# facebookresearch/D3GA

Measured on AMD Instinct MI355X. Metric: fwd+bwd frames/sec @500k Gaussians 1920x1080, higher is better.
Workload: dtype f32

## Files before the change

### d3ga_amd/_lib.py

```python
import ctypes
import os

_HERE = os.path.dirname(os.path.abspath(__file__))
_PATH = os.environ.get("D3GA_LIB_PATH") or os.path.join(_HERE, "libd3ga_hip.so")
_lib = None
ACC_STRIDE = 16
replay_epoch = [0]
ABI_VERSION = 112
KNOBS = ("composite_variant", "merge_slots", "tile_assign", "bwd_split", "sort_merge", "ssim_impl", "wgrad_ws", "chain_abl", "chain_grid")
CAMERA_SLOT_WINDOWED = -1.0
LOSS_PARTIALS = 2048
BLUR_PARTIALS = 6144
CALIB_PARTIALS = 12288
FRAME_GAMMA, FRAME_BG_WHITE, FRAME_ERODE_MASK, FRAME_CLOSE_HOLES, FRAME_IMAGE_U8, FRAME_SEG_F32 = 1, 2, 4, 8, 16, 32
EVAL_BG_WHITE, EVAL_COMPOSED, EVAL_ALPHA3, EVAL_BOUNDARY_F32 = 1, 2, 4, 8
EVAL_MAX_PARTIALS = 2048
MESH_MAX_SIDE = 16384
MESH_CAM_FLOATS = 16
INTERP_MAX_D = 64
KNN_MAX_K = 16
POINTS_MAX_K = 8
LPIPS_PARTIALS = 1024
OPTIM_CHUNK = 8192
OPTIM_ALIGNED16 = 1


class D3GAError(RuntimeError):
    pass


def library_path():
    return _PATH


class RasterParams(ctypes.Structure):
    _fields_ = [("P", ctypes.c_int32), ("M", ctypes.c_int32), ("sh_degree", ctypes.c_int32),
                ("W", ctypes.c_int32), ("H", ctypes.c_int32),
                ("tanfovx", ctypes.c_float), ("tanfovy", ctypes.c_float), ("scale_modifier", ctypes.c_float),
                ("antialiasing", ctypes.c_int32), ("prefiltered", ctypes.c_int32), ("debug", ctypes.c_int32),
                ("opacity_activation", ctypes.c_int32), ("forward_only", ctypes.c_int32),
                ("acc_self_clearing", ctypes.c_int32), ("n_views", ctypes.c_int32), ("per_view_geometry", ctypes.c_int32),
                ("tile_cull", ctypes.c_int32),
                ("factor_rows", ctypes.c_int32), ("per_view_appearance", ctypes.c_int32), ("per_view_background", ctypes.c_int32)]


BODY_MAX_JOINTS = 64
BODY_MAX_SHAPE = 32
BODY_LD_ALIGN = 2048


def body_saved_floats(J):
    return 27 * J + 16


class BodyModel(ctypes.Structure):
    _fields_ = [("V", ctypes.c_int32), ("J", ctypes.c_int32), ("n_shape", ctypes.c_int32), ("n_expr", ctypes.c_int32),
                ("n_hand_pca", ctypes.c_int32), ("ld", ctypes.c_int32), ("n_levels", ctypes.c_int32), ("reserved", ctypes.c_int32)] + \
               [(n, ctypes.c_void_p) for n in ("v_template", "dirs", "w_ptr", "w_joint", "w_val", "wt_ptr", "wt_vert", "wt_val",
                                               "J0", "Jdirs", "parents", "level_ptr", "level_joint", "child_ptr", "child_joint",
                                               "hand_comps", "hand_mean")]


class LbsPoseGrad(ctypes.Structure):
    _fields_ = [("J", ctypes.c_int32), ("n_chunks", ctypes.c_int32), ("n_entries", ctypes.c_int64)] + \
               [(n, ctypes.c_void_p) for n in ("tmpl", "delta", "chunk_ptr", "chunk_range", "entries", "counter", "scratch", "g_joint_mats",
                                               "g_Rh", "g_Th")]


DEFORM_ROUTE_CORNERS, DEFORM_ROUTE_MERGE = 1, 2


class CageDeformIn(ctypes.Structure):
    _fields_ = [(n, ctypes.c_int32) for n in ("P", "V", "flags", "reserved")] + \
               [(n, ctypes.c_void_p) for n in ("tetpoints", "tetras", "tetra_id", "barys", "canon_grad", "scales", "rots", "delta_barys")]


class CageDeformGrads(ctypes.Structure):
    _fields_ = [(n, ctypes.c_void_p) for n in ("g_means", "g_cov6", "g_tetpoints", "g_barys", "g_scales", "g_rots")]


class CageDeformRoute(ctypes.Structure):
    _fields_ = [(n, ctypes.c_int32) for n in ("kind", "n_segments")] + \
               [(n, ctypes.c_void_p) for n in ("item_pos", "seg_begin", "seg_ptr", "vert_start", "vert_items", "records")]


class CageDeformSkin(ctypes.Structure):
    _fields_ = [(n, ctypes.c_int32) for n in ("K", "reserved")] + \
               [(n, ctypes.c_void_p) for n in ("joint_mats", "skin_idx", "skin_w", "Rh", "g_tetpoints_extra", "g_delta")]


SKEL_MAX_JOINTS = 512
SKEL_SAVED_FLOATS = 12


class Skeleton(ctypes.Structure):
    _fields_ = [("J", ctypes.c_int32), ("n_params", ctypes.c_int32), ("n_levels", ctypes.c_int32), ("n_children", ctypes.c_int32)] + \
               [(n, ctypes.c_void_p) for n in ("parents", "level_ptr", "level_joint", "child_ptr", "child_joint", "joint_offset",
                                               "joint_rotation", "transform_offsets", "csr_ptr", "csr_col", "csr_val", "csc_ptr",
                                               "csc_row", "csc_val")]


CODE_MAX_B, CODE_MAX_D = 16, 4096
ROW_CACHE_MAX_PAIRS = 16


class RowPair(ctypes.Structure):
    _fields_ = [("table", ctypes.c_void_p), ("stage", ctypes.c_void_p), ("width", ctypes.c_int32), ("n_rows", ctypes.c_int32)]


SCALE_ACT_NONE, SCALE_ACT_EXP = 0, 1
SCALE_ENERGY_GRID = 1536
OBJ_MAX_FRAMES, OBJ_SLOTS, OBJ_MAX_LEN, OBJ_TERMS = 16, 9, 4096, 9
OBJ_STATUS_NAN_SEEN, OBJ_STATUS_FIRST_BAD, OBJ_STATUS_STEPS, OBJ_STATUS_TERMS, OBJ_STATUS_WORDS = 0, 1, 2, 4, 16


POSE_MAX_D, POSE_FIT_CHUNK = 256, 256
POSE_STAGE_PROJECT, POSE_STAGE_CLIP, POSE_STAGE_RECONSTRUCT = 1, 2, 4


class ObjectiveEntry(ctypes.Structure):
    _fields_ = [("ptr", ctypes.c_void_p), ("len", ctypes.c_int32), ("goff", ctypes.c_int32)]


class ObjectiveDesc(ctypes.Structure):
    _fields_ = [("n_frames", ctypes.c_int32), ("reserved", ctypes.c_int32)] + \
               [(n, ctypes.c_float) for n in ("lambda_dssim", "rgb_weight", "sil_weight", "fme_weight", "blur_weight", "vgg_weight")] + \
               [("entry", ObjectiveEntry * (OBJ_MAX_FRAMES * OBJ_SLOTS))]


_vp, _i, _i64, _f = ctypes.c_void_p, ctypes.c_int, ctypes.c_int64, ctypes.c_float
_prm = ctypes.POINTER(RasterParams)
_bm = ctypes.POINTER(BodyModel)
_lpg = ctypes.POINTER(LbsPoseGrad)
_sk = ctypes.POINTER(Skeleton)

_deform_tail = [ctypes.POINTER(c) for c in (CageDeformIn, CageDeformGrads, CageDeformRoute)]

_SIGNATURES = {
    "d3ga_version": ([], _i),
    "d3ga_status_string": ([_i], ctypes.c_char_p),
    "d3ga_debug_set": ([ctypes.c_int32, ctypes.c_int32], _i),
    "d3ga_debug_defaults": ([ctypes.POINTER(ctypes.c_int32), ctypes.c_int32], _i),
    "d3ga_lbs_cage_fwd": ([_i, _i] + [_vp] * 8 + [_vp], _i),
    "d3ga_lbs_cage_bwd": ([_i, _i] + [_vp] * 6 + [_lpg, _vp], _i),
    "d3ga_lbs_pose_scratch_bytes": ([_i, ctypes.c_int32, ctypes.c_int32, ctypes.POINTER(_i64)], _i),
    "d3ga_cage_deform_fwd": ([ctypes.POINTER(CageDeformIn), _vp, _vp, _vp], _i),
    "d3ga_cage_deform_bwd": ([ctypes.POINTER(c) for c in (CageDeformIn, CageDeformGrads, CageDeformRoute, CageDeformSkin)] + [_lpg, _vp], _i),
    "d3ga_cage_deform_bwd_tail": ([ctypes.POINTER(c) for c in (CageDeformIn, CageDeformGrads, CageDeformRoute, CageDeformSkin)] + [_lpg, _vp], _i),
    "d3ga_fem_energy_fwd": ([_i] + [_vp] * 4 + [_vp], _i),
    "d3ga_fem_energy_bwd": ([_i, _i] + [_vp] * 5 + [_vp], _i),
    "d3ga_bary_interp_fwd": ([ctypes.c_int32] * 3 + [_vp] * 5 + [_vp], _i),
    "d3ga_bary_interp_bwd": ([ctypes.c_int32] * 4 + [_vp] * 9 + [_vp], _i),
    "d3ga_raster_scratch_bytes": ([ctypes.c_int32, ctypes.c_int32, ctypes.c_int32, _i64, ctypes.POINTER(_i64)], _i),
    "d3ga_raster_scratch_bytes_views": ([ctypes.c_int32] * 4 + [_i64, ctypes.c_int32, ctypes.POINTER(_i64)], _i),
    "d3ga_raster_scratch_bytes_window": ([ctypes.c_int32] * 4 + [_i64, ctypes.c_int32, ctypes.POINTER(_i64)], _i),
    "d3ga_raster_binning_layout_window": ([ctypes.c_int32] * 3 + [_i64, ctypes.POINTER(_i64)], _i),
    "d3ga_raster_binning_layout": ([ctypes.c_int32, ctypes.c_int32, _i64, ctypes.POINTER(_i64)], _i),
    "d3ga_raster_img_layout": ([ctypes.c_int32, ctypes.c_int32, ctypes.POINTER(_i64)], _i),
    "d3ga_raster_img_layout_blocks": ([ctypes.c_int32, ctypes.c_int32, ctypes.POINTER(_i64)], _i),
    "d3ga_raster_img_bytes": ([ctypes.c_int32, ctypes.c_int32, _i64, ctypes.c_int32], _i64),
    "d3ga_raster_preprocess": ([_prm] + [_vp] * 12 + [_i64, _vp, _vp], _i),
    "d3ga_raster_bin_sort": ([_prm, _vp, _vp, _i64, _vp], _i),
    "d3ga_raster_composite_fwd": ([_prm, _vp, _vp, _vp, _i64, _vp, _vp, _vp, _vp], _i),
    "d3ga_raster_composite_bwd": ([_prm, _vp, _vp, _vp, _i64, _vp, _vp, _vp, _vp], _i),
    "d3ga_raster_composite_bwd_depth": ([_prm, _vp, _vp, _vp, _i64, _vp, _vp, _vp, _vp, _vp], _i),
    "d3ga_raster_composite_fwd2": ([_prm, _vp, _vp, _vp, _vp, _vp, _i64, _vp, _vp, _vp, _vp, _vp], _i),
    "d3ga_raster_composite_bwd2": ([_prm, _vp, _vp, _vp, _vp, _vp, _i64, _vp, _vp, _vp, _vp, _vp], _i),
    "d3ga_raster_preprocess_bwd": ([_prm] + [_vp] * 18 + [_vp], _i),
    "d3ga_raster_preprocess_bwd_deform": ([_prm] + [_vp] * 18 + _deform_tail + [_vp], _i),
    "d3ga_raster_forward": ([_prm] + [_vp] * 14 + [_i64, _vp, _vp, _vp, _vp], _i),
    "d3ga_raster_backward": ([_prm] + [_vp] * 11 + [_i64] + [_vp] * 11 + [_vp], _i),
    "d3ga_raster_backward_deform": ([_prm] + [_vp] * 11 + [_i64] + [_vp] * 11 + _deform_tail + [_vp], _i),
    "d3ga_raster_composite_fwd_l1": ([_prm, _vp, _vp, _vp, _i64] + [_vp] * 7 + [_vp], _i),
    "d3ga_raster_composite_bwd_l1": ([_prm, _vp, _vp, _vp, _i64] + [_vp] * 7 + [_vp], _i),
    "d3ga_raster_backward_l1": ([_prm] + [_vp] * 11 + [_i64] + [_vp] * 15 + [_vp], _i),
    "d3ga_raster_backward_l1_deform": ([_prm] + [_vp] * 11 + [_i64] + [_vp] * 15 + _deform_tail + [_vp], _i),
    "d3ga_raster_recolor": ([_prm] + [_vp] * 6 + [_vp], _i),
    "d3ga_raster_mark_visible": ([ctypes.c_int32, _vp, _vp, _vp, _vp], _i),
    "d3ga_sh_grad_from_views": ([ctypes.c_int32] * 4 + [_vp, _vp, _i64, _vp, _i64, ctypes.c_float, _vp, _vp], _i),
    "d3ga_compute_bary": ([_i, _i] + [_vp] * 5 + [_vp], _i),
    "d3ga_selftest_row_scan": ([_i, _vp, _vp, _vp], _i),
    "d3ga_selftest_alpha": ([ctypes.c_int32, _vp, _i, _vp, _vp, _vp, _vp, _vp, _vp], _i),
    "d3ga_knn3_mean_dist2": ([_i, _vp, _vp, _vp], _i),
    "d3ga_compute_bary_grid": ([_i] + [_vp] * 9 + [_vp], _i),
    "d3ga_knn3_mean_dist2_grid": ([_i] + [_vp] * 6 + [_vp], _i),
    "d3ga_knn_points": ([_i] * 4 + [_vp] * 4 + [_vp], _i),
    "d3ga_knn_points_grid": ([_i] * 3 + [_vp] * 8 + [_vp], _i),
    "d3ga_interp_face_attrs": ([_i64, _i64, _i] + [_vp] * 4 + [_vp], _i),
    "d3ga_l1_mean_fwd": ([_i64, _vp, _vp, _vp, _vp], _i),
    "d3ga_l1_mean_fwd_ws": ([_i64, _vp, _vp, _vp, _vp, _vp], _i),
    "d3ga_l1_mean_bwd": ([_i64, _vp, _vp, _vp, _vp, _vp], _i),
    "d3ga_l1_mean_fwd_ws_cell": ([_i64, _vp, _vp, _vp, _vp, _vp], _i),
    "d3ga_l1_mean_bwd_cell": ([_i64, _vp, _vp, _vp, _vp, _vp], _i),
    "d3ga_mlp_panel_bytes": ([ctypes.c_int32, ctypes.c_int32], _i64),
    "d3ga_mlp_pack_weights": ([ctypes.c_int32, ctypes.c_int32, _vp, _i64, _i64, _vp, _vp], _i),
# ... 167 lines not shown
```

### d3ga_amd/csrc/build.py

```python
import os
import subprocess
import sys

HERE = os.path.dirname(os.path.abspath(__file__))
SOURCES = ["deform.hip", "raster_pre.hip", "raster_bin.hip", "raster_composite.hip", "raster_composite_scan.hip", "raster_api.hip", "bary.hip", "loss.hip", "image_tail.hip", "calib.hip", "frame_prep.hip", "eval.hip", "mesh_raster.hip", "point_raster.hip", "optim.hip", "mlp.hip", "encoding.hip", "body_model.hip", "skeleton.hip", "perceptual.hip", "lpips.hip", "knn.hip", "bary_interp.hip", "frame_state.hip", "objective.hip", "pose_prior.hip"]
LINK_MAP = os.path.join(HERE, "d3ga.map")
HEADERS = ["d3ga_math.h", "d3ga_internal.h", "raster_pre_body.h", "deform_tail.h", "composite_common.h", "body_model_math.h", "skeleton_math.h", "frame_prep_math.h", "eval_math.h", "mesh_raster_math.h", "point_raster_math.h", "perceptual_math.h", "lpips_math.h", "knn_math.h", "objective_math.h", "pose_prior_math.h", os.path.join("..", "..", "include", "d3ga.h")]
ABL = os.environ.get("D3GA_SCAN_ABL")
VARIANT = os.environ.get("D3GA_VARIANT")
DIAG = os.environ.get("D3GA_DIAG") or (("abl" + ABL) if ABL else None) or (("var" + VARIANT.split(":")[0]) if VARIANT else None)
DIAG_DIR = os.path.abspath(os.path.join(HERE, "..", "..", "tools", "_build"))
_DIAG_TAG = (VARIANT.split(":")[0] if (VARIANT and not os.environ.get("D3GA_DIAG") and not ABL) else
             "diag" if os.environ.get("D3GA_DIAG") in (None, "counters") else os.environ["D3GA_DIAG"])
if VARIANT:
    FLAGS_VARIANT = [f for f in VARIANT.split(":", 1)[1].split(",") if f]
else:
    FLAGS_VARIANT = []
OUT = (os.path.join(DIAG_DIR, f"libd3ga_hip_abl{ABL}.so" if ABL else f"libd3ga_hip_{_DIAG_TAG}.so") if DIAG
       else os.path.join(HERE, "..", "libd3ga_hip.so"))
FLAGS = ["--offload-arch=gfx950", "-O3", "-std=c++17", "-fPIC", "-fvisibility=hidden", "-munsafe-fp-atomics", "-fno-gpu-rdc",
         "-Wall", "-Wno-unused-function"] + FLAGS_VARIANT
EXTRA = {"raster_composite_scan.hip": ["-fno-slp-vectorize"],
         "raster_composite.hip": ["-fno-slp-vectorize"],
         "frame_prep.hip": ["-fhip-fp32-correctly-rounded-divide-sqrt"],
         "eval.hip": ["-fhip-fp32-correctly-rounded-divide-sqrt"]}
EXTRA["mesh_raster.hip"] = ["-fhip-fp32-correctly-rounded-divide-sqrt", "-ffp-contract=off"]
EXTRA["lpips.hip"] = ["-fhip-fp32-correctly-rounded-divide-sqrt"]
EXTRA["point_raster.hip"] = EXTRA["mesh_raster.hip"]
EXTRA["knn.hip"] = ["-ffp-contract=off"]
EXTRA["frame_state.hip"] = ["-fhip-fp32-correctly-rounded-divide-sqrt"]
EXTRA["objective.hip"] = ["-fhip-fp32-correctly-rounded-divide-sqrt", "-ffp-contract=off"]
EXTRA["pose_prior.hip"] = ["-ffp-contract=off"]
if os.environ.get("D3GA_CHAIN_WAVES"):
    FLAGS.append("-DD3GA_CHAIN_WAVES=" + os.environ["D3GA_CHAIN_WAVES"])
if os.environ.get("D3GA_CHAIN_CS"):
    FLAGS.append("-DD3GA_CHAIN_CS=" + os.environ["D3GA_CHAIN_CS"])
if os.environ.get("D3GA_ALL_NOSLP"):
    FLAGS.append("-fno-slp-vectorize")
if ABL:
    FLAGS.append("-DD3GA_SCAN_ABL=" + ABL.split("w")[0].split("p")[0].split("f")[0])
    if "w" in ABL:
        FLAGS.append("-DD3GA_TILE_WAVES=" + ABL.split("w")[1])
    if "f" in ABL:
        FLAGS.append("-DD3GA_FWD_WAVES=" + ABL.split("f")[1])
    if "p" in ABL:
        FLAGS.append("-DD3GA_TILE_PRIO=1")
if os.environ.get("D3GA_DIAG"):
    FLAGS += ["-DD3GA_DIAG", "-DD3GA_DIAG_TIMELINE"]
    if os.environ.get("D3GA_DIAG") == "counters":
        FLAGS.append("-DD3GA_DIAG_COUNTERS")


def _newer(target, deps):
    if not os.path.exists(target):
        return True
    t = os.path.getmtime(target)
    return any(os.path.getmtime(d) > t for d in deps)


def build(force=False, verbose=False):
    hipcc = os.environ.get("HIPCC", "/opt/rocm/bin/hipcc")
    objdir = os.path.join(DIAG_DIR, f"obj_abl{ABL}" if ABL else f"obj_{_DIAG_TAG}") if DIAG else os.path.join(HERE, "build")
    os.makedirs(objdir, exist_ok=True)
    hdrs = [os.path.join(HERE, h) for h in HEADERS]
    objs = []
    for src in SOURCES:
        s = os.path.join(HERE, src)
        o = os.path.join(objdir, src.replace(".hip", ".o"))
        if force or _newer(o, [s] + hdrs):
            cmd = [hipcc] + FLAGS + EXTRA.get(src, []) + ["-c", s, "-o", o]
            if verbose:
                print(" ".join(cmd))
            subprocess.check_call(cmd)
        objs.append(o)
    if force or _newer(OUT, objs + [LINK_MAP]):
        import torch
        tlib = os.path.join(os.path.dirname(torch.__file__), "lib")
        cmd = ["g++", "-shared", "-fPIC"] + objs + ["-L" + tlib, "-lamdhip64", "-Wl,-rpath," + tlib,
                                                    "-Wl,-rpath,/opt/rocm/lib", "-Wl,--version-script=" + LINK_MAP, "-o", OUT]
        if verbose:
            print(" ".join(cmd))
        subprocess.check_call(cmd)
    return os.path.abspath(OUT)


if __name__ == "__main__":
    print(build(force="--force" in sys.argv, verbose=True))
```

### d3ga_amd/csrc/d3ga_internal.h

```cpp
#pragma once
#include <hip/hip_runtime.h>
#include <stdint.h>

#include "../../include/d3ga.h"
#include "d3ga_math.h"

namespace d3ga {

constexpr int kBlock = 256;

int debug_knob(int key);

int deform_tail_check(const d3ga_cage_deform_in *in, const d3ga_cage_deform_grads *gr, const d3ga_cage_deform_route *route);

static inline int64_t align256(int64_t x) { return (x + 255) & ~int64_t(255); }

struct GeomBuf {
    float *depth;
    float4 *conic_o;
    float4 *rgb_invd;
    uint2 *rect;
    uint8_t *clamped;
    float *cov3D;
    float4 *xyh;
    float *dcol;
    int64_t dcol_stride;
};
static inline int64_t geom_bytes(int64_t P) {
    return align256(4 * P) + align256(16 * P) + align256(16 * P) + align256(8 * P) + align256(P) +
           align256(24 * P) + align256(16 * P) + align256(36 * P);
}
static inline GeomBuf carve_geom(void *base, int64_t P) {
    char *p = (char *)base;
    GeomBuf g;
    g.depth = (float *)p;     p += align256(4 * P);
    g.conic_o = (float4 *)p;  p += align256(16 * P);
    g.rgb_invd = (float4 *)p; p += align256(16 * P);
    g.rect = (uint2 *)p;      p += align256(8 * P);
    g.clamped = (uint8_t *)p; p += align256(P);
    g.cov3D = (float *)p;     p += align256(24 * P);
    g.xyh = (float4 *)p;      p += align256(16 * P);
    g.dcol = (float *)p;
    g.dcol_stride = P;
    return g;
}
__host__ __device__ static inline GeomBuf geom_view(const GeomBuf &g, int64_t P, int64_t v) {
    GeomBuf o = g;
    const int64_t d = v * P;
    o.depth += d; o.conic_o += d; o.rgb_invd += d; o.rect += d; o.clamped += d; o.cov3D += 6 * d; o.xyh += d; o.dcol += d;
    return o;
}

struct BinBuf {
    uint32_t *counters;
    uint32_t *tile_count;
    uint32_t *tile_count2;
    uint32_t *vis_part;
    uint32_t *tile_start;
    uint32_t *tile_cursor;
    uint64_t *keys;
    uint32_t *point_list;
    uint32_t *big_tiles;
    uint32_t *huge_tiles;
    uint32_t *mid_tiles;
    uint32_t *tile_order;
};
constexpr int kVisParts = 32, kVisStride = 32;
constexpr int kUnresvWord = 1;
static inline int64_t bin_bytes(int64_t tiles, int64_t dcap) {
    return 256 + 2 * align256(4 * tiles) + 4 * kVisParts * kVisStride + align256(4 * (tiles + 1)) + align256(4 * tiles) + align256(8 * dcap) +
           align256(4 * dcap) + 4 * align256(4 * tiles);
}
static inline BinBuf carve_bin(void *base, int64_t tiles, int64_t dcap) {
    char *p = (char *)base;
    BinBuf b;
    b.counters = (uint32_t *)p;    p += 256;
    b.tile_count = (uint32_t *)p;  p += align256(4 * tiles);
    b.tile_count2 = (uint32_t *)p; p += align256(4 * tiles);
    b.vis_part = (uint32_t *)p;    p += 4 * kVisParts * kVisStride;
    b.tile_start = (uint32_t *)p;  p += align256(4 * (tiles + 1));
    b.tile_cursor = (uint32_t *)p; p += align256(4 * tiles);
    b.keys = (uint64_t *)p;        p += align256(8 * dcap);
    b.point_list = (uint32_t *)p;  p += align256(4 * dcap);
    b.big_tiles = (uint32_t *)p;   p += align256(4 * tiles);
    b.huge_tiles = (uint32_t *)p;  p += align256(4 * tiles);
    b.mid_tiles = (uint32_t *)p;   p += align256(4 * tiles);
    b.tile_order = (uint32_t *)p;
    return b;
}

struct ImgBuf {
    float *final_T;
    uint32_t *n_contrib;
    uint32_t *blk_count;
    uint2 *blk_list;
};
static inline int64_t img_bytes(int64_t W, int64_t H, int64_t tiles, int64_t dcap, int64_t views = 1) {
    return 2 * align256(4 * W * H * views) + align256(64 * tiles) + align256(128 * dcap);
}
static inline ImgBuf carve_img(void *base, int64_t W, int64_t H, int64_t tiles, int64_t views = 1) {
    ImgBuf i;
    char *p = (char *)base;
    i.final_T = (float *)p;        p += align256(4 * W * H * views);
    i.n_contrib = (uint32_t *)p;   p += align256(4 * W * H * views);
    i.blk_count = (uint32_t *)p;   p += align256(64 * tiles);
    i.blk_list = (uint2 *)p;
    return i;
}

constexpr int kResvStride = 512;
constexpr int kResvHdr = 4;
constexpr int kResvTiles = kResvStride - kResvHdr;
constexpr int kResvSlots = (kResvTiles + 63) / 64;
static inline int64_t resv_waves(int64_t P) { return (kBlock / 64) * ((P + kBlock - 1) / kBlock); }
static inline int64_t resv_bytes(int64_t P, int64_t views) { return align256(4 * kResvStride * resv_waves(P) * views); }

struct TileWindow {
    int x0, y0, w, h;
    __device__ __forceinline__ bool empty() const { return w <= 0 || h <= 0; }
    __device__ __forceinline__ bool fits() const { return w <= kResvTiles && h <= kResvTiles && w * h <= kResvTiles; }
    __device__ __forceinline__ int area() const { return w * h; }
    __device__ __forceinline__ int tile_of(int k, int gx, float inv_w) const {
        const int r = (int)(((float)k + 0.5f) * inv_w);
        return (y0 + r) * gx + x0 + (k - r * w);
    }
};

#ifdef __HIPCC__
__device__ __forceinline__ TileWindow wave_tile_window(bool visible, int rx0, int ry0, int rx1, int ry1) {
    int bx0 = visible ? rx0 : 0x7fffffff, by0 = visible ? ry0 : 0x7fffffff, bx1 = visible ? rx1 : 0, by1 = visible ? ry1 : 0;
#pragma unroll
    for (int off = 1; off < 64; off <<= 1) {
        bx0 = min(bx0, __shfl_xor(bx0, off)); by0 = min(by0, __shfl_xor(by0, off));
        bx1 = max(bx1, __shfl_xor(bx1, off)); by1 = max(by1, __shfl_xor(by1, off));
    }
    TileWindow win;
    win.x0 = bx0; win.y0 = by0;
    win.w = bx1 > bx0 ? bx1 - bx0 : 0;
    win.h = by1 > by0 ? by1 - by0 : 0;
    if (win.w == 0 || win.h == 0) { win.x0 = 0; win.y0 = 0; win.w = 0; win.h = 0; }
    return win;
}
#endif

static inline int tiles_x(int W) { return (W + kTile - 1) / kTile; }
static inline int tiles_y(int H) { return (H + kTile - 1) / kTile; }
static inline int n_views_of(const d3ga_raster_params *prm) { return prm->n_views > 1 ? prm->n_views : 1; }
static inline bool is_windowed(const d3ga_raster_params *prm) { return prm->tanfovx == D3GA_CAMERA_SLOT_WINDOWED; }
static inline int grid_x(const d3ga_raster_params *prm) { return tiles_x(prm->W) + (is_windowed(prm) ? 1 : 0); }
static inline int grid_y(const d3ga_raster_params *prm) { return tiles_y(prm->H) + (is_windowed(prm) ? 1 : 0); }
static inline int4 *win_table(void *binning, int64_t tiles, int64_t dcap) { return (int4 *)((char *)binning + bin_bytes(tiles, dcap)); }
static inline int64_t win_table_bytes(int64_t views) { return align256(16 * views); }
static inline uint32_t *resv_records(void *binning, int64_t tiles, int64_t dcap, int64_t views, bool windowed) {
    return (uint32_t *)((char *)binning + bin_bytes(tiles, dcap) + (windowed ? win_table_bytes(views) : 0));
}

static inline int check_launch(hipStream_t s, int debug) {
    hipError_t e = hipGetLastError();
    if (e != hipSuccess) return (int)e;
    if (debug) {
        e = hipStreamSynchronize(s);
        if (e != hipSuccess) return (int)e;
    }
    return 0;
}

#define D3GA_TRY(expr)            \
    do {                          \
        int _st = (expr);         \
        if (_st != 0) return _st; \
    } while (0)
#define D3GA_HIP(expr)                          \
    do {                                        \
        hipError_t _e = (expr);                 \
        if (_e != hipSuccess) return (int)_e;   \
    } while (0)

#ifdef __HIPCC__
static __global__ void zero_words_kernel(uint32_t *__restrict__ p, size_t n) {
    for (size_t i = (size_t)blockIdx.x * blockDim.x + threadIdx.x; i < n; i += (size_t)gridDim.x * blockDim.x) p[i] = 0u;
}
static __global__ void zero_bytes_kernel(unsigned char *__restrict__ p, size_t n) {
    for (size_t i = (size_t)blockIdx.x * blockDim.x + threadIdx.x; i < n; i += (size_t)gridDim.x * blockDim.x) p[i] = 0;
}
static inline hipError_t zero_async(void *ptr, size_t bytes, hipStream_t s) {
    if (bytes == 0) return hipSuccess;
    if ((((uintptr_t)ptr | bytes) & 3) == 0) {
        const size_t n = bytes / 4;
        const size_t blocks = (n + 4 * kBlock - 1) / (4 * kBlock);
        hipLaunchKernelGGL(zero_words_kernel, dim3((unsigned)(blocks < 1 ? 1 : (blocks > 4096 ? 4096 : blocks))), dim3(kBlock), 0, s,
                           reinterpret_cast<uint32_t *>(ptr), n);
    } else {
        const size_t blocks = (bytes + kBlock - 1) / kBlock;
        hipLaunchKernelGGL(zero_bytes_kernel, dim3((unsigned)(blocks > 4096 ? 4096 : blocks)), dim3(kBlock), 0, s,
                           reinterpret_cast<unsigned char *>(ptr), bytes);
    }
    return hipGetLastError();
}
#endif

}
```

### d3ga_amd/csrc/raster_bin.hip

```cpp
#include <atomic>

#include "composite_common.h"

namespace d3ga {

constexpr int kScanBlock = 1024;

__device__ __forceinline__ void tile_scan_body(int tiles, const uint32_t *__restrict__ count, const uint32_t *__restrict__ count2,
                                               const uint32_t *__restrict__ vis_part, uint32_t *__restrict__ start, uint32_t *__restrict__ cursor,
                                               uint32_t *__restrict__ counters, uint64_t dcap,
                                               uint32_t *__restrict__ big_tiles, uint32_t *__restrict__ huge_tiles,
                                               uint32_t *__restrict__ mid_tiles, uint32_t n_small, uint32_t n_mid,
                                               uint32_t n_large) {
    constexpr int kPer = 8, kChunk = kPer * kScanBlock;
    __shared__ uint32_t s_wave[2][kScanBlock / 64];
    __shared__ uint32_t s_max;
    const int tid = threadIdx.x, lane = tid & 63, wave = tid >> 6;
    if (tid == 0) s_max = 0;
    const bool unresv = vis_part[kUnresvWord] != 0u;
    uint32_t visible = wave == 0 && lane < kVisParts ? vis_part[lane * kVisStride] : 0u;
    uint32_t carry = 0, mx = 0;
    int par = 0;
    for (int c0 = 0; c0 < tiles; c0 += kChunk, par ^= 1) {
        const int t0 = c0 + kPer * tid;
        uint32_t c[kPer], u[kPer];
        if (t0 + kPer <= tiles) {
            const uint4 lo = reinterpret_cast<const uint4 *>(count + t0)[0], hi = reinterpret_cast<const uint4 *>(count + t0)[1];
            uint4 lo2 = make_uint4(0u, 0u, 0u, 0u), hi2 = lo2;
            if (unresv) { lo2 = reinterpret_cast<const uint4 *>(count2 + t0)[0]; hi2 = reinterpret_cast<const uint4 *>(count2 + t0)[1]; }
            c[0] = lo.x; c[1] = lo.y; c[2] = lo.z; c[3] = lo.w; c[4] = hi.x; c[5] = hi.y; c[6] = hi.z; c[7] = hi.w;
            u[0] = lo2.x; u[1] = lo2.y; u[2] = lo2.z; u[3] = lo2.w; u[4] = hi2.x; u[5] = hi2.y; u[6] = hi2.z; u[7] = hi2.w;
        } else {
#pragma unroll
            for (int k = 0; k < kPer; ++k) { c[k] = t0 + k < tiles ? count[t0 + k] : 0u; u[k] = unresv && t0 + k < tiles ? count2[t0 + k] : 0u; }
        }
        uint32_t any2 = 0;
#pragma unroll
        for (int k = 0; k < kPer; ++k) { any2 |= u[k]; c[k] += u[k]; }
        uint32_t sum = 0;
#pragma unroll
        for (int k = 0; k < kPer; ++k) { sum += c[k]; mx = max(mx, c[k]); }
        uint32_t incl = sum;
#pragma unroll
        for (int off = 1; off < 64; off <<= 1) {
            const uint32_t v = __shfl_up(incl, off);
            if (lane >= off) incl += v;
        }
        if (lane == 63) s_wave[par][wave] = incl;
        __syncthreads();
        uint32_t wbase = 0, total = 0;
#pragma unroll
        for (int w = 0; w < kScanBlock / 64; ++w) {
            const uint32_t v = s_wave[par][w];
            wbase += w < wave ? v : 0u;
            total += v;
        }
        uint32_t run = carry + wbase + incl - sum;
        uint32_t e[kPer];
        int cls[kPer];
#pragma unroll
        for (int k = 0; k < kPer; ++k) {
            e[k] = run;
            run += c[k];
            cls[k] = c[k] > n_large ? 2 : (c[k] > n_mid ? 1 : (c[k] > n_small ? 0 : -1));
        }
#pragma unroll
        for (int q = 0; q < 3; ++q) {
            uint32_t nq = 0;
#pragma unroll
            for (int k = 0; k < kPer; ++k) nq += cls[k] == q ? 1u : 0u;
            if (__ballot(nq != 0u) == 0ull) continue;
            uint32_t inq = nq;
#pragma unroll
            for (int off = 1; off < 64; off <<= 1) {
                const uint32_t v = __shfl_up(inq, off);
                if (lane >= off) inq += v;
            }
            const uint32_t tot = (uint32_t)__shfl((int)inq, 63);
            uint32_t base = 0;
            if (lane == 0) base = atomicAdd(&counters[q == 0 ? D3GA_CNT_MID : (q == 1 ? D3GA_CNT_BIG : D3GA_CNT_HUGE)], tot);
            uint32_t pos = (uint32_t)__shfl((int)base, 0) + inq - nq;
            uint32_t *list = q == 0 ? mid_tiles : (q == 1 ? big_tiles : huge_tiles);
#pragma unroll
            for (int k = 0; k < kPer; ++k)
                if (cls[k] == q) list[pos++] = (uint32_t)(t0 + k);
        }
        if (t0 + kPer <= tiles) {
            const uint4 lo = make_uint4(e[0], e[1], e[2], e[3]), hi = make_uint4(e[4], e[5], e[6], e[7]);
            reinterpret_cast<uint4 *>(start + t0)[0] = lo; reinterpret_cast<uint4 *>(start + t0)[1] = hi;
        } else {
#pragma unroll
            for (int k = 0; k < kPer; ++k)
                if (t0 + k < tiles) start[t0 + k] = e[k];
        }
        if (any2) {
#pragma unroll
            for (int k = 0; k < kPer; ++k)
                if (t0 + k < tiles && u[k]) cursor[t0 + k] = e[k] + (c[k] - u[k]);
        }
        carry += total;
    }
#pragma unroll
    for (int off = 1; off < 64; off <<= 1) {
        mx = max(mx, (uint32_t)__shfl_xor((int)mx, off));
        visible += (uint32_t)__shfl_xor((int)visible, off);
    }
    if (lane == 0) atomicMax(&s_max, mx);
    __syncthreads();
    if (tid == 0) {
        start[tiles] = carry;
        counters[D3GA_CNT_D] = carry;
        counters[D3GA_CNT_OVERFLOW] = (uint64_t)carry > dcap ? 1u : 0u;
        counters[D3GA_CNT_MAXTILE] = s_max;
        counters[D3GA_CNT_VISIBLE] = visible;
    }
}

__device__ __forceinline__ void tile_order_body(int tiles, const uint32_t *__restrict__ count, const uint32_t *__restrict__ count2,
                                                const uint32_t *__restrict__ vis_part, uint32_t *__restrict__ order, uint32_t *__restrict__ counters) {
    __shared__ uint32_t s_hist[256];
    __shared__ uint32_t s_zero;
    const int tid = threadIdx.x, lane = tid & 63;
    constexpr int kPer = 8;
    const bool unresv = vis_part[kUnresvWord] != 0u;
    if (tid < 256) s_hist[tid] = 0;
    if (tid == 0) s_zero = 0;
    __syncthreads();
    auto bucket = [](uint32_t c) { return 254u - min(c >> 4, 254u); };
    for (int c0 = 0; c0 < tiles; c0 += kPer * kScanBlock) {
        uint32_t c[kPer];
#pragma unroll
        for (int k = 0; k < kPer; ++k) {
            const int t = c0 + k * kScanBlock + tid;
            c[k] = t < tiles ? count[t] + (unresv ? count2[t] : 0u) : 0xffffffffu;
        }
#pragma unroll
        for (int k = 0; k < kPer; ++k) {
            const bool zero = c[k] == 0u;
            const unsigned long long zm = __ballot(zero);
            if (lane == 0 && zm) atomicAdd(&s_zero, (uint32_t)__popcll(zm));
            if (c[k] != 0u && c[k] != 0xffffffffu) atomicAdd(&s_hist[bucket(c[k])], 1u);
        }
        if (c0 + kPer * kScanBlock < tiles) continue;
        __syncthreads();
        if (tid < 64) {
            uint32_t v[4], sum = 0;
#pragma unroll
            for (int k = 0; k < 4; ++k) { v[k] = (4 * tid + k < 255) ? s_hist[4 * tid + k] : 0u; sum += v[k]; }
            uint32_t incl = sum;
#pragma unroll
            for (int off = 1; off < 64; off <<= 1) {
                const uint32_t u = __shfl_up(incl, off);
                if (tid >= off) incl += u;
            }
            uint32_t run = incl - sum;
#pragma unroll
            for (int k = 0; k < 4; ++k) { s_hist[4 * tid + k] = run; run += v[k]; }
        }
        __syncthreads();
        if (tid == 0) {
            s_zero = s_hist[255];
            counters[D3GA_CNT_HEAVY] = s_hist[255] <= 4096u ? (s_hist[255] + 9u) / 10u : 0u;
        }
        __syncthreads();
        for (int c1 = 0; c1 < tiles; c1 += kPer * kScanBlock) {
            if (c0 != 0) {
#pragma unroll
                for (int k = 0; k < kPer; ++k) {
                    const int t = c1 + k * kScanBlock + tid;
                    c[k] = t < tiles ? count[t] + (unresv ? count2[t] : 0u) : 0xffffffffu;
                }
            }
#pragma unroll
            for (int k = 0; k < kPer; ++k) {
                const int t = c1 + k * kScanBlock + tid;
                const bool zero = c[k] == 0u;
                const unsigned long long zm = __ballot(zero);
                uint32_t zbase = 0;
                if (lane == 0 && zm) zbase = atomicAdd(&s_zero, (uint32_t)__popcll(zm));
                zbase = (uint32_t)__shfl((int)zbase, 0);
                if (zero) order[zbase + (uint32_t)__popcll(zm & ((1ull << lane) - 1ull))] = (uint32_t)t;
                if (c[k] != 0u && c[k] != 0xffffffffu) order[atomicAdd(&s_hist[bucket(c[k])], 1u)] = (uint32_t)t;
            }
        }
    }
}

__global__ __launch_bounds__(kScanBlock) void tile_scan_order_kernel(int tiles, const uint32_t *__restrict__ count,
                                                                     const uint32_t *__restrict__ count2,
                                                                     const uint32_t *__restrict__ vis_part,
                                                                     uint32_t *__restrict__ start,
                                                                     uint32_t *__restrict__ cursor,
                                                                     uint32_t *__restrict__ counters, uint64_t dcap,
                                                                     uint32_t *__restrict__ big_tiles,
                                                                     uint32_t *__restrict__ huge_tiles,
                                                                     uint32_t *__restrict__ mid_tiles, uint32_t n_small,
                                                                     uint32_t n_mid, uint32_t n_large,
                                                                     uint32_t *__restrict__ order) {
    if (blockIdx.x == 0) tile_scan_body(tiles, count, count2, vis_part, start, cursor, counters, dcap, big_tiles, huge_tiles, mid_tiles, n_small, n_mid, n_large);
    else tile_order_body(tiles, count, count2, vis_part, order, counters);
}

__global__ __launch_bounds__(kBlock) void tile_scatter_kernel(int P, int gx, const uint2 *__restrict__ rect,
                                                              const float *__restrict__ depth,
                                                              const uint32_t *__restrict__ start,
                                                              const uint32_t *__restrict__ resv,
                                                              uint32_t *__restrict__ cursor, uint64_t *__restrict__ keys,
                                                              uint64_t dcap) {
    __shared__ uint32_t s_cur[kBlock / 64][kResvTiles];
    const int tid = threadIdx.x, lane = tid & 63, wave = tid >> 6;
    const int i = blockIdx.x * kBlock + tid;
    if (i - lane >= P) return;
    const size_t j = (size_t)blockIdx.y * P + i;
    const uint32_t *rec = resv + ((size_t)blockIdx.y * gridDim.x * (kBlock / 64) + blockIdx.x * (kBlock / 64) + wave) * kResvStride;
    const uint2 box = *reinterpret_cast<const uint2 *>(rec);
    uint32_t base[kResvSlots];
    base[0] = rec[kResvHdr + lane];
    int x0 = 0, y0 = 0, x1 = 0, y1 = 0;
    uint64_t key = 0;
    if (i < P) {
        const uint2 rc = rect[j];
        x0 = rc.x & 0xffffu; y0 = rc.x >> 16; x1 = rc.y & 0xffffu; y1 = rc.y >> 16;
        key = ((uint64_t)__float_as_uint(depth[j]) << 32) | (uint32_t)j;
    }
    const bool visible = x1 > x0 && y1 > y0;
    TileWindow win;
    win.x0 = (int)(box.x & 0xffffu); win.y0 = (int)(box.x >> 16); win.w = (int)(box.y & 0xffffu); win.h = (int)(box.y >> 16);
    if (win.empty()) return;
    if (win.fits()) {
        const int area = win.area();
        uint32_t *cur = s_cur[wave];
        const float inv_w = 1.0f / (float)win.w;
#pragma unroll
        for (int q = 1; q < kResvSlots; ++q) base[q] = lane + 64 * q < area ? rec[kResvHdr + lane + 64 * q] : 0u;
#pragma unroll
        for (int q = 0; q < kResvSlots; ++q) {
            const int k = lane + 64 * q;
            if (k < area) cur[k] = start[win.tile_of(k, gx, inv_w)] + base[q];
        }
        __builtin_amdgcn_wave_barrier();
        if (visible)
            for (int ty = y0; ty < y1; ++ty)
                for (int tx = x0; tx < x1; ++tx) {
                    const int l = (ty - win.y0) * win.w + (tx - win.x0);
                    if ((unsigned)l >= (unsigned)area) continue;
                    const uint32_t pos = atomicAdd(&cur[l], 1u);
                    if (pos < dcap) keys[pos] = key;
                }
    } else if (visible) {
        for (int ty = y0; ty < y1; ++ty)
            for (int tx = x0; tx < x1; ++tx) {
                const uint32_t pos = atomicAdd(&cursor[ty * gx + tx], 1u);
                if (pos < dcap) keys[pos] = key;
            }
    }
}

template <typename KeyPtr>
__device__ __forceinline__ void bitonic_sort(KeyPtr k, int n, int tid, int nthreads) {
    int n2 = 1;
    while (n2 < n) n2 <<= 1;
    const int half = n2 >> 1;
    for (int size = 2, lsz = 1; size <= n2; size <<= 1, ++lsz) {
        const int hs = size >> 1;
        for (int i = tid; i < half; i += nthreads) {
            const int blk = i >> (lsz - 1), off = i & (hs - 1);
            const int lo = (blk << lsz) + off, hi = (blk << lsz) + size - 1 - off;
            if (hi < n) {
                const uint64_t a = k[lo], b = k[hi];
                if (b < a) { k[lo] = b; k[hi] = a; }
            }
        }
        __syncthreads();
        for (int j = hs >> 1, lj = lsz - 2; j >= 1; j >>= 1, --lj) {
            for (int i = tid; i < half; i += nthreads) {
                const int blk = i >> lj, off = i & (j - 1);
                const int lo = (blk << (lj + 1)) + off, hi = lo + j;
                if (hi < n) {
                    const uint64_t a = k[lo], b = k[hi];
                    if (b < a) { k[lo] = b; k[hi] = a; }
                }
            }
            __syncthreads();
        }
    }
}

template <int BLOCK, int CAP>
__device__ __forceinline__ void sort_one_tile_bucket(uint64_t *s_key, uint32_t *s_bin, uint32_t *s_red, int tile,
                                                     const uint32_t *__restrict__ start, const uint64_t *__restrict__ keys,
                                                     uint32_t *__restrict__ point_list, uint64_t dcap) {
    static_assert(CAP == 8 * BLOCK, "eight keys / eight counters per thread");
    constexpr int NW = BLOCK / 64;
    const uint64_t b64 = min((uint64_t)start[tile], dcap), e64 = min((uint64_t)start[tile + 1], dcap);
    const int n = min((int)(e64 - b64), CAP);
    const int tid = threadIdx.x, lane = tid & 63, wave = tid >> 6;
    uint64_t r[8];
    uint32_t lo = 0xffffffffu, hi = 0u;
#pragma unroll
    for (int k = 0; k < 8; ++k) {
        const int i = tid + k * BLOCK;
        r[k] = i < n ? keys[b64 + i] : ~0ull;
    }
#pragma unroll
    for (int k = 0; k < 8; ++k) {
        const int i = tid + k * BLOCK;
        if (i < n) { const uint32_t d = (uint32_t)(r[k] >> 32); lo = min(lo, d); hi = max(hi, d); }
    }
#pragma unroll
    for (int off = 1; off < 64; off <<= 1) {
        lo = min(lo, (uint32_t)__shfl_xor((int)lo, off));
        hi = max(hi, (uint32_t)__shfl_xor((int)hi, off));
    }
    if (lane == 0) { s_red[wave] = lo; s_red[NW + wave] = hi; }
#pragma unroll
    for (int k = 0; k < 8; ++k) s_bin[tid + k * BLOCK] = 0u;
    __syncthreads();
#pragma unroll
    for (int w = 0; w < NW; ++w) { lo = min(lo, s_red[w]); hi = max(hi, s_red[NW + w]); }
    const uint32_t range = hi - lo;
    int sh = 32 - __clz((int)(range | 1u)) - (31 - __clz(CAP));
    if (range & 0x80000000u) sh = 32 - (31 - __clz(CAP));
    sh = max(sh, 0);
    uint32_t bucket[8], slot[8];
#pragma unroll
    for (int k = 0; k < 8; ++k) {
        const int i = tid + k * BLOCK;
        bucket[k] = ((uint32_t)(r[k] >> 32) - lo) >> sh;
        slot[k] = 0u;
        if (i < n) slot[k] = atomicAdd(&s_bin[bucket[k]], 1u);
    }
    __syncthreads();
    {
        uint32_t c[8], sum = 0;
#pragma unroll
        for (int k = 0; k < 8; ++k) { c[k] = s_bin[8 * tid + k]; sum += c[k]; }
        uint32_t incl = sum;
#pragma unroll
        for (int off = 1; off < 64; off <<= 1) {
            const uint32_t u = (uint32_t)__shfl_up((int)incl, off);
            if (lane >= off) incl += u;
        }
        if (lane == 63) s_red[wave] = incl;
        __syncthreads();
        uint32_t run = incl - sum;
#pragma unroll
        for (int w = 0; w < NW; ++w) if (w < wave) run += s_red[w];
#pragma unroll
        for (int k = 0; k < 8; ++k) { s_bin[8 * tid + k] = run; run += c[k]; }
        if (tid == BLOCK - 1) s_bin[CAP] = run;
    }
    __syncthreads();
#pragma unroll
    for (int k = 0; k < 8; ++k) {
        const int i = tid + k * BLOCK;
        if (i < n) s_key[s_bin[bucket[k]] + slot[k]] = r[k];
    }
    __syncthreads();
#pragma unroll
    for (int k = 0; k < 8; ++k) {
        const int i = tid + k * BLOCK;
        if (i < n) {
            const uint32_t b0 = s_bin[bucket[k]], b1 = s_bin[bucket[k] + 1];
            uint32_t less = 0;
            for (uint32_t p = b0; p < b1; ++p) less += s_key[p] < r[k] ? 1u : 0u;
            point_list[b64 + b0 + less] = (uint32_t)r[k];
        }
    }
}

template <int BLOCK, int CAP>
__device__ __forceinline__ bool sort_huge_tile_bucket(uint64_t *s_key, uint32_t *s_bin, uint32_t *s_cur, uint32_t *s_red, int tile,
                                                      const uint32_t *__restrict__ start, const uint64_t *__restrict__ keys,
                                                      uint32_t *__restrict__ point_list, uint64_t dcap) {
    static_assert(CAP == 8 * BLOCK, "eight counters per thread");
    constexpr int NW = BLOCK / 64;
    const uint64_t b64 = min((uint64_t)start[tile], dcap), e64 = min((uint64_t)start[tile + 1], dcap);
    const int n = (int)(e64 - b64);
    const int tid = threadIdx.x, lane = tid & 63, wave = tid >> 6;
    uint32_t lo = 0xffffffffu, hi = 0u;
    for (int i = tid; i < n; i += BLOCK) { const uint32_t d = (uint32_t)(keys[b64 + i] >> 32); lo = min(lo, d); hi = max(hi, d); }
#pragma unroll
    for (int off = 1; off < 64; off <<= 1) {
        lo = min(lo, (uint32_t)__shfl_xor((int)lo, off));
        hi = max(hi, (uint32_t)__shfl_xor((int)hi, off));
    }
    __syncthreads();
    if (lane == 0) { s_red[wave] = lo; s_red[NW + wave] = hi; }
#pragma unroll
    for (int k = 0; k < 8; ++k) s_bin[tid + k * BLOCK] = 0u;
    __syncthreads();
#pragma unroll
    for (int w = 0; w < NW; ++w) { lo = min(lo, s_red[w]); hi = max(hi, s_red[NW + w]); }
    const uint32_t range = hi - lo;
    const int sh = max(32 - __clz((int)(range | 1u)) - (31 - __clz(CAP)), 0);
    for (int i = tid; i < n; i += BLOCK) atomicAdd(&s_bin[((uint32_t)(keys[b64 + i] >> 32) - lo) >> sh], 1u);
    __syncthreads();
    uint32_t cmax = 0;
    {
        uint32_t c[8], sum = 0;
#pragma unroll
        for (int k = 0; k < 8; ++k) { c[k] = s_bin[8 * tid + k]; sum += c[k]; cmax = max(cmax, c[k]); }
        uint32_t incl = sum;
#pragma unroll
        for (int off = 1; off < 64; off <<= 1) {
            const uint32_t u = (uint32_t)__shfl_up((int)incl, off);
            if (lane >= off) incl += u;
            cmax = max(cmax, (uint32_t)__shfl_xor((int)cmax, off));
        }
        __syncthreads();
        if (lane == 63) { s_red[wave] = incl; s_red[NW + wave] = cmax; }
        __syncthreads();
        uint32_t run = incl - sum;
#pragma unroll
        for (int w = 0; w < NW; ++w) { if (w < wave) run += s_red[w]; cmax = max(cmax, s_red[NW + w]); }
#pragma unroll
        for (int k = 0; k < 8; ++k) { s_bin[8 * tid + k] = run; run += c[k]; }
        if (tid == BLOCK - 1) s_bin[CAP] = run;
    }
    __syncthreads();
    if (cmax > (uint32_t)CAP) return false;
    for (int segA = 0; segA < CAP;) {
        if (tid == 0) {
            const uint32_t limit = s_bin[segA] + (uint32_t)CAP;
            int a = segA + 1, b = CAP;
            while (a < b) { const int m = (a + b + 1) >> 1; if (s_bin[m] <= limit) a = m; else b = m - 1; }
            s_red[0] = (uint32_t)a;
        }
#pragma unroll
        for (int k = 0; k < 8; ++k) s_cur[tid + k * BLOCK] = 0u;
        __syncthreads();
        const int segB = (int)s_red[0];
        const uint32_t baseA = s_bin[segA], m = s_bin[segB] - baseA;
        if (m) {
            for (int i = tid; i < n; i += BLOCK) {
                const uint64_t key = keys[b64 + i];
                const uint32_t b = ((uint32_t)(key >> 32) - lo) >> sh;
                if (b >= (uint32_t)segA && b < (uint32_t)segB) s_key[s_bin[b] - baseA + atomicAdd(&s_cur[b], 1u)] = key;
            }
            __syncthreads();
            for (uint32_t i = tid; i < m; i += BLOCK) {
                const uint64_t key = s_key[i];
                const uint32_t b = ((uint32_t)(key >> 32) - lo) >> sh;
                const uint32_t b0 = s_bin[b] - baseA, b1 = s_bin[b + 1] - baseA;
                uint32_t less = 0;
                for (uint32_t p = b0; p < b1; ++p) less += s_key[p] < key ? 1u : 0u;
                point_list[b64 + baseA + b0 + less] = (uint32_t)key;
            }
        }
        __syncthreads();
        segA = segB;
    }
    return true;
}

template <int BLOCK, int CAP>
__global__ __launch_bounds__(BLOCK) void tile_sort_lds_kernel(const uint32_t *__restrict__ start,
                                                              const uint64_t *__restrict__ keys,
                                                              uint32_t *__restrict__ point_list, uint64_t dcap,
                                                              const uint32_t *__restrict__ order, int tiles) {
    __shared__ uint64_t s_key[CAP];
    __shared__ __attribute__((aligned(8))) uint32_t s_bin[CAP + 1];
    __shared__ uint32_t s_red[2 * (BLOCK / 64)];
    for (int rank = blockIdx.x; rank < tiles; rank += gridDim.x) {
        const int tile = (int)order[rank];
        const uint32_t n = start[tile + 1] - start[tile];
        if (n == 0) return;
        if (n <= (uint32_t)CAP) sort_one_tile_bucket<BLOCK, CAP>(s_key, s_bin, s_red, tile, start, keys, point_list, dcap);
        __syncthreads();
    }
}

template <int BLOCK, int CAP>
__global__ __launch_bounds__(BLOCK) void tile_sort_lds_list_kernel(const uint32_t *__restrict__ start,
                                                                   const uint64_t *__restrict__ keys,
                                                                   uint32_t *__restrict__ point_list, uint64_t dcap,
                                                                   const uint32_t *__restrict__ list,
                                                                   const uint32_t *__restrict__ list_count,
                                                                   uint64_t *__restrict__ keys_rw,
                                                                   const uint32_t *__restrict__ huge_list,
                                                                   const uint32_t *__restrict__ huge_count,
                                                                   const uint32_t *__restrict__ list2,
                                                                   const uint32_t *__restrict__ list2_count) {
    extern __shared__ __attribute__((aligned(16))) uint64_t s_key_dyn[];
    uint32_t *s_bin = reinterpret_cast<uint32_t *>(s_key_dyn + CAP);
    uint32_t *s_red = s_bin + CAP + 1;
    uint32_t *s_cur = s_red + 2 * (BLOCK / 64) + 2;
    const uint32_t count = *list_count;
    for (uint32_t v = blockIdx.x; v < count; v += gridDim.x) {
        __syncthreads();
        sort_one_tile_bucket<BLOCK, CAP>(s_key_dyn, s_bin, s_red, (int)list[v], start, keys, point_list, dcap);
    }
    if (list2) {
        const uint32_t count2 = *list2_count;
        for (uint32_t v = gridDim.x - 1u - blockIdx.x; v < count2; v += gridDim.x) {
            __syncthreads();
            sort_one_tile_bucket<BLOCK, CAP>(s_key_dyn, s_bin, s_red, (int)list2[v], start, keys, point_list, dcap);
        }
    }
    if (huge_list) {
        const uint32_t hcount = *huge_count;
        const int tid = threadIdx.x;
        for (uint32_t k = blockIdx.x; k < hcount; k += gridDim.x) {
            const int tile = (int)huge_list[k];
            const uint64_t b64 = min((uint64_t)start[tile], dcap), e64 = min((uint64_t)start[tile + 1], dcap);
            const int n = (int)(e64 - b64);
            __syncthreads();
            if (!sort_huge_tile_bucket<BLOCK, CAP>(s_key_dyn, s_bin, s_cur, s_red, tile, start, keys, point_list, dcap)) {
                bitonic_sort(keys_rw + b64, n, tid, BLOCK);
                for (int i = tid; i < n; i += BLOCK) point_list[b64 + i] = (uint32_t)keys_rw[b64 + i];
            }
        }
    }
}

}

using namespace d3ga;

constexpr int kSortSmall = 2048;
constexpr int kSortMid = 4096;
constexpr int kSortLarge = 8192;
static inline size_t sort_lds_bytes(int cap, int block, bool huge = false) {
    return (size_t)cap * 8 + ((size_t)cap + 1 + 2 * (block / 64) + 2 + (huge ? cap : 0)) * 4 + 16;
}


extern "C" int d3ga_raster_bin_sort(const d3ga_raster_params *prm, void *geom, void *binning, int64_t d_capacity,
                                    d3ga_stream_t stream) {
    if (!prm || !geom || !binning) return D3GA_E_NULL;
    if (prm->P < 0 || prm->W <= 0 || prm->H <= 0 || d_capacity < 0) return D3GA_E_SIZE;
    hipStream_t s = (hipStream_t)stream;
    const int views = n_views_of(prm);
    const int gx = grid_x(prm);
    const int tiles = gx * grid_y(prm) * views;
    const int64_t P = (int64_t)prm->P * views;
    BinBuf bin = carve_bin(binning, tiles, d_capacity);
    GeomBuf g = carve_geom(geom, P);
    hipLaunchKernelGGL(tile_scan_order_kernel, dim3(2), dim3(kScanBlock), 0, s, tiles, bin.tile_count, bin.tile_count2, bin.vis_part, bin.tile_start,
                       bin.tile_cursor, bin.counters, (uint64_t)d_capacity, bin.big_tiles, bin.huge_tiles, bin.mid_tiles,
                       (uint32_t)kSortSmall, (uint32_t)kSortMid, (uint32_t)kSortLarge, bin.tile_order);
    D3GA_TRY(check_launch(s, prm->debug));
    if (P == 0 || d_capacity == 0) return D3GA_OK;
    hipLaunchKernelGGL(tile_scatter_kernel, dim3((unsigned)((prm->P + kBlock - 1) / kBlock), (unsigned)views), dim3(kBlock), 0, s, prm->P,
                       gx, g.rect, g.depth, bin.tile_start, resv_records(binning, tiles, d_capacity, views, is_windowed(prm)),
                       bin.tile_cursor, bin.keys, (uint64_t)d_capacity);
    D3GA_TRY(check_launch(s, prm->debug));
    {
        static std::atomic<int> resident[64] = {};
        int dev = 0;
        D3GA_HIP(hipGetDevice(&dev));
        int want = (dev >= 0 && dev < 64) ? resident[dev].load(std::memory_order_relaxed) : 0;
        if (want == 0) {
            int per_cu = 0, cus = 0;
            if (hipOccupancyMaxActiveBlocksPerMultiprocessor(&per_cu, (const void *)tile_sort_lds_kernel<256, kSortSmall>, 256, 0) != hipSuccess || per_cu < 1) per_cu = 4;
            if (hipDeviceGetAttribute(&cus, hipDeviceAttributeMultiprocessorCount, dev) != hipSuccess || cus < 1) cus = 256;
            want = per_cu * cus;
            if (dev >= 0 && dev < 64) resident[dev].store(want, std::memory_order_relaxed);
        }
        hipLaunchKernelGGL((tile_sort_lds_kernel<256, kSortSmall>), dim3(tiles < want ? tiles : want), dim3(256), 0, s, bin.tile_start,
                           bin.keys, bin.point_list, (uint64_t)d_capacity, (const uint32_t *)bin.tile_order, tiles);
    }
    D3GA_TRY(check_launch(s, prm->debug));
    {
        static std::atomic<bool> attr_set[64] = {};
        int dev = 0;
        D3GA_HIP(hipGetDevice(&dev));
        if (dev >= 0 && dev < 64 && !attr_set[dev].load(std::memory_order_relaxed)) {
            D3GA_HIP(hipFuncSetAttribute((const void *)tile_sort_lds_list_kernel<1024, kSortLarge>,
                                         hipFuncAttributeMaxDynamicSharedMemorySize, (int)sort_lds_bytes(kSortLarge, 1024, true)));
            attr_set[dev].store(true, std::memory_order_relaxed);
        }
    }
    const int lgrid = tiles < 256 ? tiles : 256, mgrid = tiles < 768 ? tiles : 768;
    const int merge_knob = debug_knob(D3GA_KNOB_SORT_MERGE);
    const bool merged = merge_knob >= 0 ? merge_knob != 0 : d_capacity / (tiles > 0 ? tiles : 1) < 320;
#define D3GA_LAUNCH_LIST_SORT(BLOCKV, CAPV, GRID, HUGE, LIST, CNT, KEYS_RW, HLIST, HCNT, LIST2, CNT2)                              \
    hipLaunchKernelGGL((tile_sort_lds_list_kernel<BLOCKV, CAPV>), dim3(GRID), dim3(BLOCKV), sort_lds_bytes(CAPV, BLOCKV, HUGE), s, \
                       bin.tile_start, bin.keys, bin.point_list, (uint64_t)d_capacity, LIST, CNT, KEYS_RW, HLIST, HCNT, LIST2, CNT2)
    const uint32_t *const nil = nullptr;
    if (!merged) {
        D3GA_LAUNCH_LIST_SORT(512, kSortMid, mgrid, false, bin.mid_tiles, bin.counters + D3GA_CNT_MID, (uint64_t *)nullptr, nil, nil, nil, nil);
        D3GA_TRY(check_launch(s, prm->debug));
    }
    const uint32_t *l2 = merged ? (const uint32_t *)bin.mid_tiles : nil, *c2 = merged ? (const uint32_t *)(bin.counters + D3GA_CNT_MID) : nil;
    D3GA_LAUNCH_LIST_SORT(1024, kSortLarge, lgrid, true, bin.big_tiles, bin.counters + D3GA_CNT_BIG, bin.keys,
                          (const uint32_t *)bin.huge_tiles, (const uint32_t *)(bin.counters + D3GA_CNT_HUGE), l2, c2);
#undef D3GA_LAUNCH_LIST_SORT
    return check_launch(s, prm->debug);
}
```

### d3ga_amd/csrc/raster_pre.hip

```cpp
#include <type_traits>

#include "composite_common.h"
#include "raster_pre_body.h"
#include "deform_tail.h"

namespace d3ga {

constexpr int kShRow = 52;
constexpr int kShSlab = 64 * kShRow;
constexpr size_t kShLdsBytes = (size_t)(kBlock / 64) * kShSlab * sizeof(float);

__host__ __device__ __forceinline__ bool sh_staged(int M) { return M > 0 && (3 * M) % 4 == 0 && 3 * M <= 48; }

__device__ __forceinline__ void sh_slab_load(float *slab, const float *__restrict__ src, int rows, int M3, int lane) {
    const int nvec = rows * M3 / 4;
    for (int v = lane; v < nvec; v += 64) {
        const float4 x = reinterpret_cast<const float4 *>(src)[v];
        const int e = 4 * v, r = e / M3, c = e - r * M3;
        *reinterpret_cast<float4 *>(slab + r * kShRow + c) = x;
    }
}
__device__ __forceinline__ void sh_slab_store(const float *slab, float *__restrict__ dst, int rows, int M3, int lane) {
    const int nvec = rows * M3 / 4;
    for (int v = lane; v < nvec; v += 64) {
// ... 69 lines not shown
    float *slab = s_sh + wave * kShHalfSlab;
    const int row0 = blockIdx.x * kBlock + wave * 64;
    const int rows = min(64, prm.P - row0);
    const int nb = (prm.sh_degree + 1) * (prm.sh_degree + 1);
    float B[16];
    float dx = 0.f, dy = 0.f, dz = 1.f;
    auto eval = [&](const float *row) __attribute__((always_inline)) {
        if (WANT_J) cj = sh_accumulate_jacobian(B, dx, dy, dz, row, nb, cj);
        else sh_accumulate(B, row, 0, 16, nb, acc);
    };
    if (M3 == 48 && rows == 64) {
        if (WANT_J) {
            sh_two_pass48(slab, shs + (size_t)48 * row0, lane, [&]() __attribute__((always_inline)) {
                sh_view_dir(mean, campos, dx, dy, dz);
                sh_basis(prm.sh_degree, dx, dy, dz, B);
            }, eval);
            return;
        }
        const float *src = shs + (size_t)48 * row0;
        const ShRegs<kShPassRows> h0 = sh_rows48_load<kShPassRows>(src, lane);
        const ShRegs<kShPassRows> h1 = sh_rows48_load<kShPassRows>(src + 48 * kShPassRows, lane);
        sh_view_basis(prm, mean, campos, B);
        __builtin_amdgcn_wave_barrier();
        sh_rows48_to_slab<kShPassRows>(slab, h0, lane);
        __builtin_amdgcn_wave_barrier();
        if (lane / kShPassRows == 0) eval(slab + (lane % kShPassRows) * kShRow);
        __builtin_amdgcn_wave_barrier();
        sh_rows48_to_slab<kShPassRows>(slab, h1, lane);
        __builtin_amdgcn_wave_barrier();
        if (lane / kShPassRows == 1) eval(slab + (lane % kShPassRows) * kShRow);
        return;
    }
    if (WANT_J && i < prm.P) sh_view_dir(mean, campos, dx, dy, dz);
    if (i < prm.P) sh_view_basis(prm, mean, campos, B);
    for (int h = 0; h < 2; ++h) {
        const int r = min(kShPassRows, rows - kShPassRows * h);
        __builtin_amdgcn_wave_barrier();
        if (r > 0) sh_slab_load(slab, shs + (size_t)M3 * (row0 + kShPassRows * h), r, M3, lane);
        __builtin_amdgcn_wave_barrier();
        if (i < prm.P && lane / kShPassRows == h) eval(slab + (lane % kShPassRows) * kShRow);
    }
}

struct TileRect { bool visible; int r0, r1, r2, r3; };
__device__ __forceinline__ TileRect view_tile_rect(const PreOut &o, int tile_row0) {
    const Splat &sp = o.sp;
    return TileRect{sp.visible, sp.rect[0], sp.rect[1] + tile_row0, sp.rect[2], sp.rect[3] + tile_row0};
}
__device__ __forceinline__ void tile_tighten(PreOut &o) {
    Splat &sp = o.sp;
    if (!sp.visible) return;
    const SplatCull sc = splat_cull(sp.conic[0], sp.conic[1], sp.conic[2], o.opacity);
    tile_rect_tight(sp.rect, sp.px, sp.py, sc.hx, sc.hy, sp.rect);
}
__device__ __forceinline__ float write_geom_records_splat(const GeomBuf &geom, int i, const PreOut &o, bool keep_cov, int tile_row0,
                                                          int32_t *__restrict__ radii) {
    const Splat &sp = o.sp;
    if (keep_cov) {
#pragma unroll
        for (int k = 0; k < 6; ++k) geom.cov3D[6 * (size_t)i + k] = o.c6[k];
    }
    radii[i] = sp.radius;
    geom.depth[i] = sp.depth;
    geom.rect[i] = sp.visible ? make_uint2((uint32_t)sp.rect[0] | ((uint32_t)(sp.rect[1] + tile_row0) << 16),
                                           (uint32_t)sp.rect[2] | ((uint32_t)(sp.rect[3] + tile_row0) << 16))
                              : make_uint2(0u, 0u);
    geom.conic_o[i] = make_float4(sp.conic[0], sp.conic[1], sp.conic[2], o.opacity);
    {
        const SplatCull sc = splat_cull(sp.conic[0], sp.conic[1], sp.conic[2], o.opacity);
        geom.xyh[i] = make_float4(sp.px, sp.py, sp.visible ? sc.hx : -1.0f, sc.hy);
    }
    return sp.visible ? 1.0f / sp.depth : 0.f;
}
__device__ __forceinline__ void write_geom_records_colour(const GeomBuf &geom, int i, float r, float g, float b, float invd,
                                                           uint8_t clampmask, bool want_j, const ShColJ &cj) {
    geom.rgb_invd[i] = make_float4(r, g, b, invd);
    geom.clamped[i] = clampmask;
    if (want_j) dcol_store(geom.dcol, geom.dcol_stride, i, cj);
}
__device__ __forceinline__ void write_geom_records(const GeomBuf &geom, int i, const PreOut &o, bool keep_cov, int tile_row0,
                                                   int32_t *__restrict__ radii, bool want_j, const ShColJ &cj) {
    const float invd = write_geom_records_splat(geom, i, o, keep_cov, tile_row0, radii);
    write_geom_records_colour(geom, i, o.rgb[0], o.rgb[1], o.rgb[2], invd, o.clampmask, want_j, cj);
}

__device__ __forceinline__ PreOut window_clip(PreOut o, int x0, int y0, int gx, int gy) {
    Splat &sp = o.sp;
    const int r0 = max(sp.rect[0], x0) - x0, r1 = max(sp.rect[1], y0) - y0;
    const int r2 = min(sp.rect[2], x0 + gx) - x0, r3 = min(sp.rect[3], y0 + gy) - y0;
    if (sp.visible && r2 > r0 && r3 > r1) { sp.rect[0] = r0; sp.rect[1] = r1; sp.rect[2] = r2; sp.rect[3] = r3; }
    else { sp.visible = false; sp.rect[0] = sp.rect[1] = sp.rect[2] = sp.rect[3] = 0; }
    return o;
}
__global__ void window_table_kernel(d3ga_raster_params prm, const float *__restrict__ campos, int views, int4 *__restrict__ table) {
    const int v = blockIdx.x * blockDim.x + threadIdx.x;
    if (v >= views) return;
    const ViewCam c = view_cam(prm, nullptr, nullptr, campos + (size_t)D3GA_CAMERA_SLOT_WINDOWED_FLOATS * v, true);
    table[v] = make_int4(c.ox, c.oy, c.W, c.H);
}

struct TileResv { TileWindow win; uint32_t base[kResvSlots]; };
template <bool SCALAR_WIN = false >
__device__ __forceinline__ TileResv tile_reserve_issue(uint32_t *s_win, const TileRect &t, int gx, uint32_t *__restrict__ tile_count,
                                                       uint32_t *__restrict__ tile_count2, uint32_t *__restrict__ vis_part) {
    const int lane = threadIdx.x & 63;
    TileResv r;
    r.win = wave_tile_window(t.visible, t.r0, t.r1, t.r2, t.r3);
    if constexpr (SCALAR_WIN) {
    r.win.x0 = __builtin_amdgcn_readfirstlane(r.win.x0); r.win.y0 = __builtin_amdgcn_readfirstlane(r.win.y0);
    r.win.w = __builtin_amdgcn_readfirstlane(r.win.w); r.win.h = __builtin_amdgcn_readfirstlane(r.win.h);
    }
#pragma unroll
    for (int j = 0; j < kResvSlots; ++j) r.base[j] = 0u;
    const unsigned long long vis = __ballot(t.visible);
    if (lane == 0 && vis) atomicAdd(&vis_part[((blockIdx.x * (kBlock / 64) + (threadIdx.x >> 6)) % kVisParts) * kVisStride], (uint32_t)__popcll(vis));
    if (r.win.empty()) return r;
    if (r.win.fits()) {
        const int area = r.win.area();
        __builtin_amdgcn_wave_barrier();
#pragma unroll
        for (int j = 0; j < kResvSlots; ++j)
            if (lane + 64 * j < area) s_win[lane + 64 * j] = 0u;
        __builtin_amdgcn_wave_barrier();
        if (t.visible)
            for (int ty = t.r1; ty < t.r3; ++ty)
                for (int tx = t.r0; tx < t.r2; ++tx) atomicAdd(&s_win[(ty - r.win.y0) * r.win.w + (tx - r.win.x0)], 1u);
        __builtin_amdgcn_wave_barrier();
        const float inv_w = 1.0f / (float)r.win.w;
#pragma unroll
        for (int j = 0; j < kResvSlots; ++j) {
            const int k = lane + 64 * j;
            const uint32_t c = k < area ? s_win[k] : 0u;
            if (c) r.base[j] = atomicAdd(&tile_count[r.win.tile_of(k, gx, inv_w)], c);
        }
    } else {
        if (lane == 0) atomicOr(&vis_part[kUnresvWord], 1u);
        if (t.visible)
            for (int ty = t.r1; ty < t.r3; ++ty)
                for (int tx = t.r0; tx < t.r2; ++tx) atomicAdd(&tile_count2[ty * gx + tx], 1u);
    }
    return r;
}
__device__ __forceinline__ void tile_reserve_store(const TileResv &r, uint32_t *__restrict__ rec) {
    const int lane = threadIdx.x & 63;
    if (lane == 0)
        *reinterpret_cast<uint4 *>(rec) = make_uint4((uint32_t)r.win.x0 | ((uint32_t)r.win.y0 << 16), (uint32_t)r.win.w | ((uint32_t)r.win.h << 16), 0u, 0u);
    if (r.win.empty() || !r.win.fits()) return;
    const int area = r.win.area();
#pragma unroll
    for (int j = 0; j < kResvSlots; ++j)
        if (lane + 64 * j < area) rec[kResvHdr + lane + 64 * j] = r.base[j];
}

template <bool WIN, bool TC = false>
__device__ __forceinline__ PreOut preprocess_view(const d3ga_raster_params &prm, const ViewCam &cam, int i, V3 mean,
                                                    const float *sh_row, bool staged, const ShColJ &cj, bool pre, const float (&pc6)[6],
                                                    float pop, const float *colors_precomp, const float *opacities, const float *scales,
                                                    const float *rotations, const float *cov3D_precomp, int gx, int gy) {
    PreLoaded pl;
    pl.has_sh = staged; pl.has_c6 = pre;
    pl.sh[0] = cj.a0; pl.sh[1] = cj.a1; pl.sh[2] = cj.a2;
#pragma unroll
    for (int k = 0; k < 6; ++k) pl.c6[k] = pc6[k];
    pl.op = pop;
    pl.has_mean = true; pl.mean = mean;
    PreOut o = preprocess_one(prm, cam, i, nullptr, sh_row, colors_precomp, opacities, scales, rotations, cov3D_precomp, pl);
    if constexpr (TC) tile_tighten(o);
    if constexpr (WIN) o = window_clip(o, cam.ox / kTile, cam.oy / kTile, gx, gy);
    return o;
}

template <bool WIN, bool TC = false>
__device__ __forceinline__ void preprocess_full_wavefront(
    const d3ga_raster_params &prm, const ViewCam &cam, const float *__restrict__ means3D, const float *__restrict__ shs,
    const float *__restrict__ opacities, const float *__restrict__ cov3D_precomp, const float *__restrict__ campos, const GeomBuf &geom,
    uint32_t *__restrict__ tile_count,
    uint32_t *__restrict__ tile_count2, uint32_t *__restrict__ vis_part, uint32_t *__restrict__ rec, int32_t *__restrict__ radii,
    int tile_row0, int gx, int gy, float *slab) {
    const int tid = threadIdx.x, lane = tid & 63;
    const int i = blockIdx.x * kBlock + tid;
    const int row0 = i - lane;
    PreLoaded pl;
    pl.has_sh = true; pl.has_c6 = true; pl.has_mean = true;
    pl.mean = ld3(means3D, i);
    pl.op = opacities[i];
#pragma unroll
    for (int k = 0; k < 6; ++k) pl.c6[k] = cov3D_precomp[6 * (size_t)i + k];
    const int nb = (prm.sh_degree + 1) * (prm.sh_degree + 1);
    float B[16];
    float dx, dy, dz, invd;
    bool visible = false;
    TileResv rs;
    ShColJ cj = {0.f, 0.f, 0.f, 0.f, 0.f, 0.f, 0.f, 0.f, 0.f, 0.f, 0.f, 0.f};
    sh_two_pass48(slab, shs + (size_t)48 * row0, lane, [&]() __attribute__((always_inline)) {
        PreOut o = preprocess_geom(prm, cam, i, pl.mean, opacities, nullptr, nullptr, cov3D_precomp, pl);
        if constexpr (WIN) visible = o.sp.visible;
        if constexpr (TC) tile_tighten(o);
        if constexpr (WIN) o = window_clip(o, cam.ox / kTile, cam.oy / kTile, gx, gy);
        rs = tile_reserve_issue<true>(reinterpret_cast<uint32_t *>(slab), view_tile_rect(o, tile_row0), gx, tile_count, tile_count2, vis_part);
        invd = write_geom_records_splat(geom, i, o, false, tile_row0, radii);
        sh_view_dir(pl.mean, campos, dx, dy, dz);
        sh_basis(prm.sh_degree, dx, dy, dz, B);
    }, [&](const float *row) __attribute__((always_inline)) {
        cj = sh_accumulate_jacobian(B, dx, dy, dz, row, nb, cj);
    });
    pl.sh[0] = cj.a0; pl.sh[1] = cj.a1; pl.sh[2] = cj.a2;
    float rgb[3] = {0.f, 0.f, 0.f};
    uint8_t clampmask = 0;
    if constexpr (!WIN) visible = invd != 0.f;
    preprocess_colour(prm, cam, i, pl.mean, nullptr, nullptr, pl, visible, rgb, clampmask);
    write_geom_records_colour(geom, i, rgb[0], rgb[1], rgb[2], invd, clampmask, true, cj);
    tile_reserve_store(rs, rec);
}

template <bool WANT_J, bool WIN, bool TC = false>
__global__ __launch_bounds__(kBlock) void preprocess_kernel(
    d3ga_raster_params prm, const float *__restrict__ means3D, const float *__restrict__ shs,
    const float *__restrict__ colors_precomp, const float *__restrict__ opacities, const float *__restrict__ scales,
    const float *__restrict__ rotations, const float *__restrict__ cov3D_precomp, const float *__restrict__ viewmatrix,
    const float *__restrict__ projmatrix, const float *__restrict__ campos, GeomBuf geom,
    uint32_t *__restrict__ tile_count, uint32_t *__restrict__ tile_count2, uint32_t *__restrict__ vis_part,
    uint32_t *__restrict__ resv , int32_t *__restrict__ radii,
    int tile_row0 ) {
    const ViewCam cam = view_cam(prm, viewmatrix, projmatrix, campos, WIN);
    const int gx = (prm.W + kTile - 1) / kTile + (WIN ? 1 : 0), gy = (prm.H + kTile - 1) / kTile + 1;
    extern __shared__ __attribute__((aligned(16))) char smem[];
    float *s_sh = reinterpret_cast<float *>(smem);
    const int tid = threadIdx.x, wave = tid >> 6;
    const int i = blockIdx.x * kBlock + tid;
    const int M3 = 3 * prm.M;
    const bool staged = shs != nullptr && sh_staged(prm.M);
    uint32_t *s_win = reinterpret_cast<uint32_t *>(smem) + wave * (staged ? kShHalfSlab : kResvStride);
    uint32_t *const rec = resv + (size_t)(blockIdx.x * (kBlock / 64) + wave) * kResvStride;
    const int row0 = blockIdx.x * kBlock + wave * 64;
    if (WANT_J && staged && cov3D_precomp && M3 == 48 && prm.P - row0 >= 64) {
        preprocess_full_wavefront<WIN, TC>(prm, cam, means3D, shs, opacities, cov3D_precomp, campos, geom, tile_count, tile_count2, vis_part, rec,
                                           radii, tile_row0, gx, gy, s_sh + wave * kShHalfSlab);
        return;
    }
    V3 mean = v3(0.f, 0.f, 0.f);
    float pc6[6] = {0.f, 0.f, 0.f, 0.f, 0.f, 0.f}, pop = 0.f;
    const bool pre = staged && cov3D_precomp != nullptr;
    if (i < prm.P) {
        mean = ld3(means3D, i);
        if (pre) {
#pragma unroll
            for (int k = 0; k < 6; ++k) pc6[k] = cov3D_precomp[6 * (size_t)i + k];
            pop = opacities[i];
        }
    }
    ShColJ cj = {0.f, 0.f, 0.f, 0.f, 0.f, 0.f, 0.f, 0.f, 0.f, 0.f, 0.f, 0.f};
    float acc[3] = {0.f, 0.f, 0.f};
    if (staged) {
        staged_sh_colour<WANT_J>(prm, mean, shs, campos, s_sh, acc, cj);
        if (!WANT_J) { cj.a0 = acc[0]; cj.a1 = acc[1]; cj.a2 = acc[2]; }
    }
    TileRect tr = {false, 0, 0, 0, 0};
    PreOut o = {};
    if (i < prm.P) {
        o = staged ? preprocess_view<WIN, TC>(prm, cam, i, mean, nullptr, true, cj, pre, pc6, pop, colors_precomp, opacities, scales,
                                              rotations, cov3D_precomp, gx, gy)
                   : preprocess_view<WIN, TC>(prm, cam, i, mean, shs ? shs + (size_t)M3 * i : nullptr, false, cj, false, pc6, pop,
                                              colors_precomp, opacities, scales, rotations, cov3D_precomp, gx, gy);
        tr = view_tile_rect(o, tile_row0);
    }
    const TileResv rs = tile_reserve_issue(s_win, tr, gx, tile_count, tile_count2, vis_part);
    if (i < prm.P) write_geom_records(geom, i, o, !cov3D_precomp, tile_row0, radii, WANT_J, cj);
    tile_reserve_store(rs, rec);
}

template <bool WANT_J, int KV>
__device__ __forceinline__ void staged_sh_colour_views(const d3ga_raster_params &prm, const float *__restrict__ means3D, size_t pv,
                                                       const float *__restrict__ shs, const ViewCams<KV> &cams, float *s_sh,
                                                       ShColJ (&cj)[KV]) {
    const int tid = threadIdx.x, lane = tid & 63, wave = tid >> 6;
    const int i = blockIdx.x * kBlock + tid;
    const int M3 = 3 * prm.M;
    float *slab = s_sh + wave * kShHalfSlab;
    const int row0 = blockIdx.x * kBlock + wave * 64;
    const int rows = min(64, prm.P - row0);
    const int nb = (prm.sh_degree + 1) * (prm.sh_degree + 1);
    auto eval = [&](const float *row) __attribute__((always_inline)) {
#pragma unroll
        for (int v = 0; v < KV; ++v) {
            float B[16];
            const float *mv = means3D + 3 * pv * v;
            if (WANT_J) {
                float dx, dy, dz;
                sh_view_dir(mv, i, cams.cp[v], dx, dy, dz);
                sh_basis(prm.sh_degree, dx, dy, dz, B);
                cj[v] = sh_accumulate_jacobian(B, dx, dy, dz, row, nb, cj[v]);
            } else {
                sh_view_basis(prm, mv, i, cams.cp[v], B);
                float acc[3] = {cj[v].a0, cj[v].a1, cj[v].a2};
                sh_accumulate(B, row, 0, 16, nb, acc);
                cj[v].a0 = acc[0]; cj[v].a1 = acc[1]; cj[v].a2 = acc[2];
            }
        }
    };
    if (M3 == 48 && rows == 64) {
        const float *src = shs + (size_t)48 * row0;
        const ShRegs<kShPassRows> h0 = sh_rows48_load<kShPassRows>(src, lane);
        const ShRegs<kShPassRows> h1 = sh_rows48_load<kShPassRows>(src + 48 * kShPassRows, lane);
        __builtin_amdgcn_wave_barrier();
        sh_rows48_to_slab<kShPassRows>(slab, h0, lane);
        __builtin_amdgcn_wave_barrier();
        if (lane / kShPassRows == 0) eval(slab + (lane % kShPassRows) * kShRow);
        __builtin_amdgcn_wave_barrier();
        sh_rows48_to_slab<kShPassRows>(slab, h1, lane);
        __builtin_amdgcn_wave_barrier();
        if (lane / kShPassRows == 1) eval(slab + (lane % kShPassRows) * kShRow);
        return;
    }
    for (int h = 0; h < 2; ++h) {
        const int r = min(kShPassRows, rows - kShPassRows * h);
        __builtin_amdgcn_wave_barrier();
        if (r > 0) sh_slab_load(slab, shs + (size_t)M3 * (row0 + kShPassRows * h), r, M3, lane);
        __builtin_amdgcn_wave_barrier();
        if (i < prm.P && lane / kShPassRows == h) eval(slab + (lane % kShPassRows) * kShRow);
    }
}

template <bool WANT_J, int KV, bool TC = false>
__global__ __launch_bounds__(kBlock) void preprocess_views_kernel(
    d3ga_raster_params prm, const float *__restrict__ means3D, const float *__restrict__ shs,
    const float *__restrict__ colors_precomp, const float *__restrict__ opacities, const float *__restrict__ scales,
    const float *__restrict__ rotations, const float *__restrict__ cov3D_precomp, ViewCams<KV> cams, GeomBuf geom ,
    uint32_t *__restrict__ tile_count, uint32_t *__restrict__ tile_count2, uint32_t *__restrict__ vis_part,
    uint32_t *__restrict__ resv , int32_t *__restrict__ radii ,
    int tile_row0, int gyv, size_t pv ) {
    extern __shared__ __attribute__((aligned(16))) char smem[];
    float *s_sh = reinterpret_cast<float *>(smem);
    const int tid = threadIdx.x, wave = tid >> 6;
    const int i = blockIdx.x * kBlock + tid;
    uint32_t *s_win = reinterpret_cast<uint32_t *>(smem) + wave * kShHalfSlab;
    const size_t wpv = (size_t)gridDim.x * (kBlock / 64);
    float pc6[6] = {0.f, 0.f, 0.f, 0.f, 0.f, 0.f}, pop = 0.f;
    const bool pre = cov3D_precomp != nullptr && pv == 0;
    if (pre && i < prm.P) {
#pragma unroll
        for (int k = 0; k < 6; ++k) pc6[k] = cov3D_precomp[6 * (size_t)i + k];
        pop = opacities[i];
    }
    ShColJ cj[KV];
#pragma unroll
    for (int v = 0; v < KV; ++v) cj[v] = ShColJ{0.f, 0.f, 0.f, 0.f, 0.f, 0.f, 0.f, 0.f, 0.f, 0.f, 0.f, 0.f};
    staged_sh_colour_views<WANT_J, KV>(prm, means3D, pv, shs, cams, s_sh, cj);
    const int gx = (prm.W + kTile - 1) / kTile;
#pragma unroll
    for (int v = 0; v < KV; ++v) {
        TileRect tr = {false, 0, 0, 0, 0};
        PreOut o = {};
        if (i < prm.P) {
            const size_t og = pv * v;
            o = preprocess_view<false, TC>(prm, view_cam(prm, cams.vm[v], cams.pm[v], cams.cp[v], false), i, ld3(means3D + 3 * og, i), nullptr, true,
                                           cj[v], pre, pc6, pop, colors_precomp, opacities, scales ? scales + 3 * og : nullptr,
                                           rotations ? rotations + 4 * og : nullptr, cov3D_precomp ? cov3D_precomp + 6 * og : nullptr, gx, 0);
            tr = view_tile_rect(o, tile_row0 + v * gyv);
        }
        const TileResv rs = tile_reserve_issue(s_win, tr, gx, tile_count, tile_count2, vis_part);
        if (i < prm.P)
            write_geom_records(geom_view(geom, prm.P, v), i, o, !cov3D_precomp, tile_row0 + v * gyv, radii + (size_t)prm.P * v, WANT_J, cj[v]);
        tile_reserve_store(rs, resv + (wpv * v + blockIdx.x * (kBlock / 64) + wave) * kResvStride);
    }
}

template <bool WANT_J>
__global__ __launch_bounds__(kBlock) void recolor_kernel(d3ga_raster_params prm, const float *__restrict__ means3D,
                                                         const float *__restrict__ shs,
                                                         const float *__restrict__ colors_precomp,
                                                         const float *__restrict__ campos, GeomBuf src, GeomBuf dst) {
    extern __shared__ __attribute__((aligned(16))) char smem[];
    float *s_sh = reinterpret_cast<float *>(smem);
    const int i = blockIdx.x * kBlock + threadIdx.x;
    const int M3 = 3 * prm.M;
    const bool staged = shs != nullptr && sh_staged(prm.M);
    ShColJ cj = {0.f, 0.f, 0.f, 0.f, 0.f, 0.f, 0.f, 0.f, 0.f, 0.f, 0.f, 0.f};
    float acc[3] = {0.f, 0.f, 0.f};
    if (staged) staged_sh_colour<WANT_J>(prm, i < prm.P ? ld3(means3D, i) : v3(0.f, 0.f, 0.f), shs, campos, s_sh, acc, cj);
    if (i >= prm.P) return;
    if (WANT_J) {
        acc[0] = cj.a0; acc[1] = cj.a1; acc[2] = cj.a2;
        dcol_store(dst.dcol, dst.dcol_stride, i, cj);
    }
    const uint2 rc = src.rect[i];
    const bool visible = rect_visible(rc.x, rc.y);
    const float depth = src.depth[i];
    dst.depth[i] = depth;
    dst.conic_o[i] = src.conic_o[i];
    dst.xyh[i] = src.xyh[i];
    dst.rect[i] = rc;
#pragma unroll
    for (int k = 0; k < 6; ++k) dst.cov3D[6 * (size_t)i + k] = src.cov3D[6 * (size_t)i + k];
    float rgb[3] = {0.f, 0.f, 0.f};
    uint8_t mask = 0;
    if (visible) {
        if (colors_precomp) {
            rgb[0] = colors_precomp[3 * (size_t)i]; rgb[1] = colors_precomp[3 * (size_t)i + 1];
            rgb[2] = colors_precomp[3 * (size_t)i + 2];
        } else {
            if (!staged) {
                float B[16];
                sh_view_basis(prm, means3D, i, campos, B);
                sh_accumulate(B, shs + (size_t)M3 * i, 0, 16, (prm.sh_degree + 1) * (prm.sh_degree + 1), acc);
            }
#pragma unroll
            for (int c = 0; c < 3; ++c) {
                const float v = acc[c] + 0.5f;
                if (v < 0.f) mask |= (uint8_t)(1u << c);
                rgb[c] = fmaxf(v, 0.f);
            }
        }
    }
    dst.rgb_invd[i] = make_float4(rgb[0], rgb[1], rgb[2], visible ? 1.0f / depth : 0.f);
    dst.clamped[i] = mask;
}

__device__ __forceinline__ ViewRecs view_recs(const GeomBuf &g, const float *acc) {
    return ViewRecs{reinterpret_cast<const uint32_t *>(g.rect), acc, g.clamped, reinterpret_cast<const float *>(g.conic_o), g.dcol,
                    g.dcol_stride};
}
// ... 89 lines not shown
                for (int k = 0; k < 3; ++k) g9[k] = dL_dmeans3D[3 * (size_t)i + k];
#pragma unroll
                for (int k = 0; k < 6; ++k) g9[3 + k] = dL_dcov3D[6 * (size_t)i + k];
            } else {
                const size_t u = (size_t)i;
                float *const m2d = dL_dmeans2D ? dL_dmeans2D + 3 * u : nullptr, *const dop = dL_dopacity ? dL_dopacity + u : nullptr;
                float *const dcl = dL_dcolors ? dL_dcolors + 3 * u : nullptr;
                if (staged)
                    preprocess_bwd_one(prm, cam, 0, visible, means3D + 3 * u, slab + lane * kShRow, nullptr, nullptr, c6, clampmask, ar.a,
                                       g9, m2d, dop, dL_dsh ? slab + lane * kShRow : nullptr, dcl, g9 + 3, nullptr, nullptr, act_opacity,
                                       have_j, jd, 0);
                else
                    preprocess_bwd_one(prm, cam, 0, visible, means3D + 3 * u, shs ? shs + (size_t)M3 * i : nullptr, nullptr, nullptr, c6,
                                       clampmask, ar.a, g9, m2d, dop, dL_dsh ? dL_dsh + (size_t)M3 * i : nullptr, dcl, g9 + 3, nullptr,
                                       nullptr, act_opacity, false, ShColJ(), 0);
            }
        } else if (staged)
            preprocess_bwd_one(prm, cam, i, visible, means3D, slab + lane * kShRow, scales, rotations, c6, clampmask, ar.a, dL_dmeans3D,
                               dL_dmeans2D, dL_dopacity, dL_dsh ? slab + lane * kShRow : nullptr, dL_dcolors, dL_dcov3D, dL_dscales,
                               dL_drots, act_opacity, have_j, jd, accum);
        else
            preprocess_bwd_one(prm, cam, i, visible, means3D, shs ? shs + (size_t)M3 * i : nullptr, scales, rotations, c6, clampmask,
                               ar.a, dL_dmeans3D, dL_dmeans2D, dL_dopacity, dL_dsh ? dL_dsh + (size_t)M3 * i : nullptr, dL_dcolors,
                               dL_dcov3D, dL_dscales, dL_drots, act_opacity, false, ShColJ(), accum);
    }
    if (staged && dL_dsh) {
        __builtin_amdgcn_wave_barrier();
        if (full48) sh_rows48_store<64>(slab, dL_dsh + (size_t)48 * row0, lane);
        else if (rows > 0) sh_slab_store(slab, dL_dsh + (size_t)M3 * row0, rows, M3, lane);
    }
    if constexpr (DEFORM) {
        const auto &dt = first_of(tail...);
        DeformGrad o;
        if (i < prm.P) {
            load_deform_streams(i, tet, dt.barys, dt.canon_grad, dt.scales, dt.rots, dt.delta_barys, dt.flags, din);
            deform_bwd(din, g9, g9 + 3, o);
            store_deform_grads(i, dt.flags, din, o, dt.g_barys, dt.g_scales, dt.g_rots);
        }
        if (dt.mg.item_pos) {
            __syncthreads();
            deform_merge_epilogue(*reinterpret_cast<float (*)[3][kMergeItems]>(smem), dt.mg, prm.P, i, i < prm.P, o);
        } else if (dt.corner_grads && i < prm.P) {
            store_corner_records(dt.corner_grads, i, o);
        }
    }
}

constexpr int kMaxGroup = 8;
template <bool WIN>
__global__ __launch_bounds__(kBlock) void preprocess_bwd_views_kernel(
    d3ga_raster_params prm, int kv, const float *__restrict__ means3D, bool sh_path, const float *__restrict__ scales,
    const float *__restrict__ rotations, const float *__restrict__ cov3D_precomp, ViewCams<kMaxGroup> cams, GeomBuf geom ,
    const float *__restrict__ acc , float *__restrict__ dL_dmeans3D, float *__restrict__ dL_dmeans2D ,
    float *__restrict__ dL_dopacity, float *__restrict__ dL_dsh, float *__restrict__ dL_dcolors, float *__restrict__ dL_dcov3D,
    float *__restrict__ dL_dscales, float *__restrict__ dL_drots, bool accum,
    size_t pv ,
    bool pva ) {
    extern __shared__ __attribute__((aligned(16))) char smem[];
    float *s_sh = reinterpret_cast<float *>(smem);
    const int tid = threadIdx.x, lane = tid & 63, wave = tid >> 6;
    const int i = blockIdx.x * kBlock + tid;
    const int M3 = 3 * prm.M;
    const int row0 = blockIdx.x * kBlock + wave * 64;
    const int rows = min(64, prm.P - row0);
    float *slab = s_sh + wave * kShSlab;
    if (i < prm.P)
        preprocess_bwd_views_one(prm, i, kv, WIN, cams, view_recs(geom, acc), means3D, cov3D_precomp ? cov3D_precomp : geom.cov3D,
                                 scales, rotations, sh_path, pv, pva, accum, dL_dmeans3D, dL_dmeans2D, dL_dopacity, dL_dcolors,
                                 dL_dcov3D, dL_dscales, dL_drots, sh_path && dL_dsh ? slab + lane * kShRow : nullptr);
    if (sh_path && dL_dsh) {
        __builtin_amdgcn_wave_barrier();
        if (accum) {
            const int nvec = rows > 0 ? rows * M3 / 4 : 0;
            float4 *dst = reinterpret_cast<float4 *>(dL_dsh + (size_t)M3 * row0);
            for (int v = lane; v < nvec; v += 64) {
                const int e = 4 * v, r = e / M3, c = e - r * M3;
                const float4 x = *reinterpret_cast<const float4 *>(slab + r * kShRow + c);
                float4 y = dst[v];
                y.x += x.x; y.y += x.y; y.z += x.z; y.w += x.w;
                dst[v] = y;
            }
        } else if (M3 == 48 && rows == 64) sh_rows48_store<64>(slab, dL_dsh + (size_t)48 * row0, lane);
        else if (rows > 0) sh_slab_store(slab, dL_dsh + (size_t)M3 * row0, rows, M3, lane);
    }
}

__global__ __launch_bounds__(kBlock) void sh_grad_from_views_kernel(
    int P, int M, int sh_degree, int n_views, const float *__restrict__ means3D, int64_t means_stride ,
    const float *__restrict__ g_views, int64_t g_stride, const float *__restrict__ campos_views, int64_t campos_stride, float scale,
    float *__restrict__ dL_dsh) {
    extern __shared__ __attribute__((aligned(16))) char smem[];
    float *s_sh = reinterpret_cast<float *>(smem);
    const int tid = threadIdx.x, lane = tid & 63, wave = tid >> 6;
    const int i = blockIdx.x * kBlock + tid;
    const int M3 = 3 * M;
    const bool staged = sh_staged(M);
    const int row0 = blockIdx.x * kBlock + wave * 64;
    const int rows = min(64, P - row0);
    float *slab = s_sh + wave * kShSlab;
    if (i < P) {
        float out[48];
#pragma unroll
        for (int k = 0; k < 48; ++k) out[k] = 0.f;
        const int nb = (sh_degree + 1) * (sh_degree + 1);
        for (int v = 0; v < n_views; ++v) {
            const float *g = g_views + v * g_stride + 3 * (size_t)i;
            const float g0 = g[0], g1 = g[1], g2 = g[2];
            if (g0 == 0.f && g1 == 0.f && g2 == 0.f) continue;
            const V3 mean = ld3(means3D + v * means_stride, i);
            const float *cp = campos_views + v * campos_stride;
            const V3 d0 = mean - v3(cp[0], cp[1], cp[2]);
            const float inv = 1.0f / sqrtf(dot(d0, d0));
            float B[16];
            sh_basis(sh_degree, d0.x * inv, d0.y * inv, d0.z * inv, B);
#pragma unroll
            for (int k = 0; k < 16; ++k)
                if (k < nb) {
                    out[3 * k] += B[k] * g0; out[3 * k + 1] += B[k] * g1; out[3 * k + 2] += B[k] * g2;
                }
        }
        float *row = staged ? slab + lane * kShRow : nullptr;
#pragma unroll
        for (int k = 0; k < 48; ++k)
            if (k < M3) {
                if (staged) row[k] = out[k] * scale;
                else dL_dsh[(size_t)M3 * i + k] = out[k] * scale;
            }
    }
    if (staged) {
        __syncthreads();
        if (rows > 0) sh_slab_store(slab, dL_dsh + (size_t)M3 * row0, rows, M3, lane);
    }
}

__global__ __launch_bounds__(kBlock) void mark_visible_kernel(int P, const float *__restrict__ means3D,
                                                              const float *__restrict__ viewmatrix,
                                                              uint8_t *__restrict__ visible) {
    const int i = blockIdx.x * kBlock + threadIdx.x;
    if (i >= P) return;
    visible[i] = xform_point(viewmatrix, ld3(means3D, i)).z > kNear ? 1 : 0;
}

}

using namespace d3ga;

static int validate(const d3ga_raster_params *prm) {
    if (!prm) return D3GA_E_NULL;
    if (prm->P < 0 || prm->W <= 0 || prm->H <= 0 || prm->M < 0 || prm->M > 16) return D3GA_E_SIZE;
    if (prm->sh_degree < 0 || prm->sh_degree > 3) return D3GA_E_CONFIG;
    if (prm->n_views < 0) return D3GA_E_SIZE;
    if (grid_x(prm) > 65535 || (int64_t)grid_y(prm) * n_views_of(prm) > 65535) return D3GA_E_SIZE;
    if ((int64_t)prm->P * n_views_of(prm) >= (1ll << 31)) return D3GA_E_SIZE;
    return D3GA_OK;
}

static bool staged(const d3ga_raster_params *prm, const float *shs) { return shs != nullptr && sh_staged(prm->M); }
static bool leaves_dcol(const d3ga_raster_params *prm, const float *shs) { return staged(prm, shs) && !prm->forward_only; }
static size_t lds_bytes(bool staged, size_t slabs, size_t floor = 0) { return staged && slabs > floor ? slabs : floor; }
static int cam_stride(const d3ga_raster_params *prm) {
    return prm->tanfovx > 0.f ? 3 : (is_windowed(prm) ? D3GA_CAMERA_SLOT_WINDOWED_FLOATS : 5);
}
template <int K>
static ViewCams<K> view_cams(const float *vm, const float *pm, const float *cp, int stride, int v0, int kv) {
    ViewCams<K> c;
    for (int q = 0; q < K; ++q) {
        const int v = v0 + (q < kv ? q : 0);
        c.vm[q] = vm + 16 * (size_t)v; c.pm[q] = pm + 16 * (size_t)v; c.cp[q] = cp + (size_t)stride * v;
    }
    return c;
}
template <class T>
static T *at(T *p, size_t n, size_t r) { return p ? p + n * r : nullptr; }

extern "C" int d3ga_raster_preprocess(const d3ga_raster_params *prm, const float *means3D, const float *shs,
                                      const float *colors_precomp, const float *opacities, const float *scales,
                                      const float *rotations, const float *cov3D_precomp, const float *viewmatrix,
                                      const float *projmatrix, const float *campos, void *geom, void *binning,
                                      int64_t d_capacity, int32_t *radii, d3ga_stream_t stream) {
    D3GA_TRY(validate(prm));
    if (!geom || !binning || !viewmatrix || !projmatrix || !campos) return D3GA_E_NULL;
    if (d_capacity < 0) return D3GA_E_SIZE;
    hipStream_t s = (hipStream_t)stream;
    const int views = n_views_of(prm), gyv = grid_y(prm);
    const int64_t tiles = (int64_t)grid_x(prm) * gyv * views;
    const bool wnd = is_windowed(prm);
    BinBuf bin = carve_bin(binning, tiles, d_capacity);
    D3GA_HIP(zero_async(bin.counters, 256 + 2 * align256(4 * tiles) + 4 * kVisParts * kVisStride, s));
    if (wnd) hipLaunchKernelGGL(window_table_kernel, dim3((views + 63) / 64), dim3(64), 0, s, *prm, campos, views, win_table(binning, tiles, d_capacity));
    if (prm->P == 0) return D3GA_OK;
    if ((shs != nullptr) == (colors_precomp != nullptr)) return D3GA_E_CONFIG;
    const bool pva = views > 1 && prm->per_view_appearance;
    if (pva && shs) return D3GA_E_CONFIG;
    const bool sr = scales != nullptr && rotations != nullptr;
    if (sr == (cov3D_precomp != nullptr)) return D3GA_E_CONFIG;
    if (shs && (prm->sh_degree + 1) * (prm->sh_degree + 1) > prm->M) return D3GA_E_CONFIG;
    if (!means3D || !opacities || !radii) return D3GA_E_NULL;
    const GeomBuf g = carve_geom(geom, (int64_t)prm->P * views);
    const size_t lds = lds_bytes(staged(prm, shs), kShHalfLdsBytes, (size_t)(kBlock / 64) * kResvStride * 4);
    uint32_t *const resv = resv_records(binning, tiles, d_capacity, views, wnd);
    const size_t resv_view = (size_t)resv_waves(prm->P) * kResvStride;
    const bool want_j = leaves_dcol(prm, shs);
    const bool tc = prm->tile_cull != 0;
    const int cs = cam_stride(prm);
    const size_t pv = (views > 1 && prm->per_view_geometry) ? (size_t)prm->P : 0;
    const size_t pa = pva ? (size_t)prm->P : 0;
    const dim3 grid((prm->P + kBlock - 1) / kBlock), block(kBlock);
    int v0 = 0;
    const bool grouped = views > 1 && !pva && !wnd && staged(prm, shs);
    auto launch_group = [&](auto kv) {
        constexpr int KV = decltype(kv)::value;
        const size_t og = pv * v0;
        const auto kernel = tc ? (want_j ? preprocess_views_kernel<true, KV, true> : preprocess_views_kernel<false, KV, true>)
                               : (want_j ? preprocess_views_kernel<true, KV> : preprocess_views_kernel<false, KV>);
        hipLaunchKernelGGL(kernel, grid, block, lds, s, *prm,
                           at(means3D, 3, og), shs, colors_precomp, opacities, at(scales, 3, og), at(rotations, 4, og),
                           at(cov3D_precomp, 6, og), view_cams<KV>(viewmatrix, projmatrix, campos, cs, v0, KV), geom_view(g, prm->P, v0),
                           bin.tile_count, bin.tile_count2, bin.vis_part, resv + resv_view * v0, radii + (size_t)prm->P * v0, v0 * gyv,
                           gyv, pv);
        v0 += KV;
    };
    while (grouped && views - v0 >= 2) {
        const int left = views - v0;
        if (left >= 4 && left != 5) launch_group(std::integral_constant<int, 4>());
        else if (left == 3 || left == 5) launch_group(std::integral_constant<int, 3>());
        else launch_group(std::integral_constant<int, 2>());
    }
    const auto kernel = tc ? (want_j ? (wnd ? preprocess_kernel<true, true, true> : preprocess_kernel<true, false, true>)
                                      : (wnd ? preprocess_kernel<false, true, true> : preprocess_kernel<false, false, true>))
                            : (want_j ? (wnd ? preprocess_kernel<true, true> : preprocess_kernel<true, false>)
                                      : (wnd ? preprocess_kernel<false, true> : preprocess_kernel<false, false>));
    for (int v = v0; v < views; ++v) {
        const ViewCams<1> c = view_cams<1>(viewmatrix, projmatrix, campos, cs, v, 1);
        const size_t og = pv * v, oa = pa * v;
        hipLaunchKernelGGL(kernel, grid, block, lds, s, *prm, at(means3D, 3, og), shs, at(colors_precomp, 3, oa), opacities + oa,
                           at(scales, 3, og), at(rotations, 4, og), at(cov3D_precomp, 6, og), c.vm[0], c.pm[0], c.cp[0],
                           geom_view(g, prm->P, v), bin.tile_count, bin.tile_count2, bin.vis_part, resv + resv_view * v,
                           radii + (size_t)prm->P * v, v * gyv);
    }
    return check_launch(s, prm->debug & 0xff);
}

extern "C" int d3ga_raster_recolor(const d3ga_raster_params *prm, const float *means3D, const float *shs,
                                   const float *colors_precomp, const float *campos, const void *geom_src,
                                   void *geom_dst, d3ga_stream_t stream) {
    D3GA_TRY(validate(prm));
    if (n_views_of(prm) > 1 || is_windowed(prm)) return D3GA_E_CONFIG;
    if (prm->P == 0) return D3GA_OK;
    if (!geom_src || !geom_dst || geom_src == geom_dst) return D3GA_E_NULL;
    if ((shs != nullptr) == (colors_precomp != nullptr)) return D3GA_E_CONFIG;
    if (shs && (!means3D || !campos)) return D3GA_E_NULL;
    if (shs && (prm->sh_degree + 1) * (prm->sh_degree + 1) > prm->M) return D3GA_E_CONFIG;
    hipStream_t s = (hipStream_t)stream;
    const GeomBuf src = carve_geom(const_cast<void *>(geom_src), prm->P), dst = carve_geom(geom_dst, prm->P);
    hipLaunchKernelGGL(leaves_dcol(prm, shs) ? recolor_kernel<true> : recolor_kernel<false>, dim3((prm->P + kBlock - 1) / kBlock),
                       dim3(kBlock), lds_bytes(staged(prm, shs), kShHalfLdsBytes), s, *prm, means3D, shs, colors_precomp, campos, src, dst);
    return check_launch(s, prm->debug & 0xff);
}

extern "C" int d3ga_raster_preprocess_bwd_deform(const d3ga_raster_params *prm, const float *means3D, const float *shs,
                                                 const float *scales, const float *rotations, const float *cov3D_precomp,
                                                 const float *viewmatrix, const float *projmatrix, const float *campos,
                                                 const void *geom, const float *acc, float *dL_dmeans3D, float *dL_dmeans2D,
                                                 float *dL_dopacity, float *dL_dsh, float *dL_dcolors, float *dL_dcov3D,
                                                 float *dL_dscales, float *dL_drots, const d3ga_cage_deform_in *din,
                                                 const d3ga_cage_deform_grads *dgr, const d3ga_cage_deform_route *route,
                                                 d3ga_stream_t stream) {
    D3GA_TRY(validate(prm));
    D3GA_TRY(deform_tail_check(din, dgr, route));
    if (n_views_of(prm) > 1 || is_windowed(prm) || scales || rotations || dL_dscales || dL_drots || din->P != prm->P) return D3GA_E_CONFIG;
    if ((dL_dmeans3D != nullptr) != (dL_dcov3D != nullptr)) return D3GA_E_CONFIG;
    if (prm->P == 0) return D3GA_OK;
    if (!means3D || !viewmatrix || !projmatrix || !campos || !geom || !acc || !cov3D_precomp) return D3GA_E_NULL;
    if (dL_dsh && !shs) return D3GA_E_NULL;
    if (shs && !dL_dsh && !dL_dcolors) return D3GA_E_NULL;
    hipStream_t s = (hipStream_t)stream;
    const GeomBuf g = carve_geom(const_cast<void *>(geom), prm->P);
    const bool merge = route && route->kind == D3GA_DEFORM_ROUTE_MERGE;
    const size_t lds = lds_bytes(staged(prm, shs), kShLdsBytes, merge ? sizeof(float) * 3 * kMergeItems : 0);
    const ViewCams<1> c = view_cams<1>(viewmatrix, projmatrix, campos, cam_stride(prm), 0, 1);
    auto launch = [&](auto dt) {
        using Tail = decltype(dt);
        dt = Tail{din->tetpoints, din->tetras, din->tetra_id, din->barys, din->canon_grad, din->scales, din->rots, din->delta_barys,
                  (int)din->flags, dgr->g_barys, dgr->g_scales, dgr->g_rots, (route && !merge) ? route->records : nullptr,
                  merge ? DeformMerge{route->item_pos, route->seg_ptr, route->seg_begin, route->records}
                        : DeformMerge{nullptr, nullptr, nullptr, nullptr}};
        hipLaunchKernelGGL((preprocess_bwd_kernel<false, true, Tail>), dim3((prm->P + kBlock - 1) / kBlock), dim3(kBlock), lds, s, *prm,
                           means3D, shs, (const float *)nullptr, (const float *)nullptr, c.vm[0], c.pm[0], c.cp[0], g, acc, dL_dmeans3D,
                           dL_dmeans2D, dL_dopacity, dL_dsh, dL_dcolors, dL_dcov3D, (float *)nullptr, (float *)nullptr, cov3D_precomp, 0, dt);
    };
    if (dL_dmeans3D) launch(DeformTailGeo{});
    else launch(DeformTail{});
    return check_launch(s, prm->debug);
}

extern "C" int d3ga_raster_preprocess_bwd(const d3ga_raster_params *prm, const float *means3D, const float *shs,
                                          const float *scales, const float *rotations, const float *cov3D_precomp,
                                          const float *viewmatrix, const float *projmatrix, const float *campos,
                                          const void *geom, const float *acc, float *dL_dmeans3D, float *dL_dmeans2D,
                                          float *dL_dopacity, float *dL_dsh, float *dL_dcolors, float *dL_dcov3D,
                                          float *dL_dscales, float *dL_drots, d3ga_stream_t stream) {
    D3GA_TRY(validate(prm));
    if (prm->P == 0) return D3GA_OK;
    if (!means3D || !viewmatrix || !projmatrix || !campos || !geom || !acc || !dL_dmeans3D) return D3GA_E_NULL;
    if (dL_dsh && !shs) return D3GA_E_NULL;
    if (shs && !dL_dsh && !dL_dcolors) return D3GA_E_NULL;
    if ((dL_dscales != nullptr) != (dL_drots != nullptr)) return D3GA_E_CONFIG;
    if (dL_dscales && (!scales || !rotations)) return D3GA_E_NULL;
    if (!cov3D_precomp && !(scales && rotations)) return D3GA_E_NULL;
    hipStream_t s = (hipStream_t)stream;
    const int views = n_views_of(prm);
    const bool pva = views > 1 && prm->per_view_appearance;
    if (pva && shs) return D3GA_E_CONFIG;
    const GeomBuf g = carve_geom(const_cast<void *>(geom), (int64_t)prm->P * views);
    const size_t lds = lds_bytes(staged(prm, shs), kShLdsBytes);
    const bool win = is_windowed(prm);
    const int cs = cam_stride(prm);
    const dim3 grid((prm->P + kBlock - 1) / kBlock), block(kBlock);
    const size_t pv = prm->per_view_geometry ? (size_t)prm->P : 0;
    auto launch_view = [&](int v, float *dsh, float *dcol, int accum) {
        const ViewCams<1> c = view_cams<1>(viewmatrix, projmatrix, campos, cs, v, 1);
        const size_t o = (size_t)prm->P * v, og = pv * v;
        hipLaunchKernelGGL(win ? preprocess_bwd_kernel<true> : preprocess_bwd_kernel<false>, grid, block, lds, s, *prm, at(means3D, 3, og),
                           shs, at(scales, 3, og), at(rotations, 4, og), c.vm[0], c.pm[0], c.cp[0], geom_view(g, prm->P, v),
                           acc + D3GA_ACC_STRIDE * o, dL_dmeans3D + 3 * og, at(dL_dmeans2D, 3, o), dL_dopacity, dsh, dcol,
                           at(dL_dcov3D, 6, og), at(dL_dscales, 3, og), at(dL_drots, 4, og), at(cov3D_precomp, 6, og), accum);
    };
    if (views == 1) {
        launch_view(0, dL_dsh, dL_dcolors, 0);
        return check_launch(s, prm->debug);
    }
    if (shs ? (dL_dsh != nullptr && leaves_dcol(prm, shs)) : true) {
        for (int v0 = 0; v0 < views; v0 += kMaxGroup) {
            const int kv = views - v0 < kMaxGroup ? views - v0 : kMaxGroup;
            const size_t o = (size_t)prm->P * v0, og = pv * v0, oa = pva ? o : 0;
            hipLaunchKernelGGL(win ? preprocess_bwd_views_kernel<true> : preprocess_bwd_views_kernel<false>, grid, block, lds, s, *prm, kv,
                               at(means3D, 3, og), shs != nullptr, at(scales, 3, og), at(rotations, 4, og), at(cov3D_precomp, 6, og),
                               view_cams<kMaxGroup>(viewmatrix, projmatrix, campos, cs, v0, kv), geom_view(g, prm->P, v0),
                               acc + D3GA_ACC_STRIDE * o, dL_dmeans3D + 3 * og, at(dL_dmeans2D, 3, o), at(dL_dopacity, 1, oa), dL_dsh,
                               at(dL_dcolors, 3, oa), at(dL_dcov3D, 6, og), at(dL_dscales, 3, og), at(dL_drots, 4, og), v0 > 0, pv, pva);
        }
        return check_launch(s, prm->debug);
    }
    if (pva) return D3GA_E_CONFIG;
    if (shs && !dL_dcolors) return D3GA_E_NULL;
    if (prm->factor_rows != 0 && prm->factor_rows < prm->P) return D3GA_E_SIZE;
    const size_t fr = prm->factor_rows > 0 ? (size_t)prm->factor_rows : (size_t)prm->P;
    for (int v = 0; v < views; ++v) launch_view(v, nullptr, shs ? dL_dcolors + 3 * fr * v : dL_dcolors, v > 0 ? (pv ? 1 : 3) : 0);
    D3GA_TRY(check_launch(s, prm->debug));
    if (shs && dL_dsh) {
        hipLaunchKernelGGL(sh_grad_from_views_kernel, grid, block, lds_bytes(sh_staged(prm->M), kShLdsBytes), s, prm->P, prm->M,
                           prm->sh_degree, views, means3D, (int64_t)(3 * pv), dL_dcolors, (int64_t)(3 * fr), campos, (int64_t)cs, 1.0f, dL_dsh);
        return check_launch(s, prm->debug);
    }
    return D3GA_OK;
}

extern "C" int d3ga_sh_grad_from_views(int32_t P, int32_t M, int32_t sh_degree, int32_t n_views, const float *means3D,
                                       const float *g_views, int64_t g_stride, const float *campos_views,
                                       int64_t campos_stride, float scale, float *dL_dsh, d3ga_stream_t stream) {
    if (P < 0 || M < 1 || M > 16 || n_views < 0) return D3GA_E_SIZE;
    if (sh_degree < 0 || sh_degree > 3 || (sh_degree + 1) * (sh_degree + 1) > M) return D3GA_E_CONFIG;
    if (P == 0) return D3GA_OK;
    if (!means3D || !dL_dsh || (n_views > 0 && (!g_views || !campos_views))) return D3GA_E_NULL;
    hipStream_t s = (hipStream_t)stream;
    hipLaunchKernelGGL(sh_grad_from_views_kernel, dim3((P + kBlock - 1) / kBlock), dim3(kBlock), lds_bytes(sh_staged(M), kShLdsBytes), s, P, M, sh_degree,
                       n_views, means3D, (int64_t)0, g_views, g_stride, campos_views, campos_stride, scale, dL_dsh);
    return check_launch(s, 0);
}

extern "C" int d3ga_raster_mark_visible(int32_t P, const float *means3D, const float *viewmatrix, uint8_t *visible,
                                        d3ga_stream_t stream) {
    if (P < 0) return D3GA_E_SIZE;
    if (P == 0) return D3GA_OK;
    if (!means3D || !viewmatrix || !visible) return D3GA_E_NULL;
    hipLaunchKernelGGL(mark_visible_kernel, dim3((P + kBlock - 1) / kBlock), dim3(kBlock), 0, (hipStream_t)stream, P,
                       means3D, viewmatrix, visible);
    return check_launch((hipStream_t)stream, 0);
}
```

### d3ga_amd/rasterizer.py

```python
import ctypes
import os
from typing import NamedTuple, Optional

import torch
from torch import nn

from . import _lib
from ._lib import RasterParams, check, dptr, require_cuda, stream_handle


class GaussianRasterizationSettings(NamedTuple):
    image_height: int
    image_width: int
    tanfovx: float
    tanfovy: float
    bg: torch.Tensor
    scale_modifier: float
    viewmatrix: torch.Tensor
    projmatrix: torch.Tensor
    sh_degree: int
    campos: torch.Tensor
    prefiltered: bool
    debug: bool
    antialiasing: bool = False
    tile_cull: bool = False


_policy = {"mode": "auto", "static": 0}
_hwm = {}
_last = {}
_last_img = {}
_capture_log = None


def set_capacity_policy(mode, capacity=0):
    if mode not in ("auto", "static"):
        raise ValueError(mode)
    _policy["mode"] = mode
    _policy["static"] = int(capacity)


def _record_forward(dev, binning, cap):
    _last[dev.index] = (binning, cap)
    if _capture_log is not None:
        _capture_log.append((binning, cap))


def _forward_with_capacity(P, k, dev, launch):
    static = _policy["mode"] == "static"
    cap = _policy["static"] if static else k * max(_hwm.get(dev.index, 0), 4 * P + 1024)
    while True:
        geom, binning, img = launch(cap)
        _record_forward(dev, binning, cap)
        if static:
            break
        cnt = binning[:32].view(torch.int32)[:2].cpu().tolist()
        D = cnt[0] & 0xFFFFFFFF
        _hwm[dev.index] = max(_hwm.get(dev.index, 0), int(D * 1.25 / k) + 1024)
        if not cnt[1]:
            break
        cap = k * _hwm[dev.index]
    return cap, geom, binning, img


_acc_policy = {"persistent": False}
_acc_cache = {}


def set_accumulator_policy(mode):
    if mode not in ("fresh", "persistent"):
        raise ValueError(mode)
    _acc_policy["persistent"] = mode == "persistent"
    if mode == "fresh":
        _acc_cache.clear()


_tile_cull = {"override": None}


def set_tile_cull(mode):
    if mode not in (None, True, False):
        raise ValueError(mode)
    _tile_cull["override"] = mode


def _tile_cull_of(requested):
    o = _tile_cull["override"]
    return bool(requested) if o is None else o


_l1_policy = {"fused_value": os.environ.get("D3GA_L1_VALUE", "fused") != "separate"}


def l1_mean_forward(image, target, cell, out, dev):
    L = _lib.lib()
    ws = torch.empty(_lib.LOSS_PARTIALS, dtype=torch.float32, device=dev)
    if cell is None:
        check(L.d3ga_l1_mean_fwd_ws(image.numel(), dptr(image), dptr(target), dptr(out), dptr(ws), stream_handle()), "d3ga_l1_mean_fwd_ws")
    else:
        check(L.d3ga_l1_mean_fwd_ws_cell(image.numel(), dptr(image), dptr(cell), dptr(out), dptr(ws), stream_handle()),
              "d3ga_l1_mean_fwd_ws_cell")


def _accumulator(P, dev):
    if not _acc_policy["persistent"] or P == 0:
        return torch.empty((P, _lib.ACC_STRIDE), dtype=torch.float32, device=dev), False
    key = (dev.index, P)
    buf = _acc_cache.get(key)
    if buf is None:
        if len(_acc_cache) > 8:
            _acc_cache.clear()
        buf = _acc_cache[key] = torch.zeros((P, _lib.ACC_STRIDE), dtype=torch.float32, device=dev)
    return buf, True


def last_counters(device=None):
    dev = torch.cuda.current_device() if device is None else torch.device(device).index
    c = _last[dev][0][:32].view(torch.int32)[:4].cpu().tolist()
    return {"D": c[0] & 0xFFFFFFFF, "overflow": bool(c[1]), "max_tile": c[2] & 0xFFFFFFFF, "visible": c[3]}


class StageTimer:

    def __init__(self):
        self.enabled = False
        self.records = []
        self.burst = {}

    def reset(self):
        self.records = []

    def stage(self, name, fn):
        if not self.enabled:
            return fn()
        reps = int(self.burst.get(name, 1))
        a, b = torch.cuda.Event(enable_timing=True), torch.cuda.Event(enable_timing=True)
        a.record()
        r = fn()
        for _ in range(reps - 1):
            fn()
        b.record()
        self.records.append((name, a, b, reps))
        return r

    def summary(self):
        per = {}
        for name, a, b, reps in self.records:
            per.setdefault(name, []).append((a.elapsed_time(b) / reps, reps))
        out = {}
        for name, ts in per.items():
            med = sorted(t for t, _ in ts)[len(ts) // 2]
            kept = [(t, r) for t, r in ts if t <= 5.0 * med] or ts
            out[name] = (sum(r for _, r in kept), sum(t for t, _ in kept) / len(kept))
        return out


stage_timer = StageTimer()


_scratch_sizes = {}
_prm_cache = {}


def _scratch(P, W, H, k, cap, device, forward_only, windowed, binning=True):
    key = (P, W, H, k, cap, bool(forward_only), bool(windowed))
    sz = _scratch_sizes.get(key)
    if sz is None:
        sizes = (ctypes.c_int64 * 3)()
        name = "d3ga_raster_scratch_bytes_window" if windowed else "d3ga_raster_scratch_bytes_views"
        check(getattr(_lib.lib(), name)(P, W, H, k, cap, int(bool(forward_only)), sizes), name)
        if len(_scratch_sizes) > 64:
            _scratch_sizes.clear()
        sz = _scratch_sizes[key] = tuple(int(n) for n in sizes)
    new = lambda n: torch.empty(n, dtype=torch.uint8, device=device)
    return [new(sz[0]), new(sz[1]) if binning else None, new(sz[2])]


def _params(P, M, sh_degree, W, H, tanfovx, tanfovy, scale_modifier, antialiasing, prefiltered, debug, opacity_activation,
            forward_only, n_views=0, per_view_geometry=False, per_view_appearance=False, per_view_background=False, tile_cull=False):
    key = (P, M, sh_degree, W, H, tanfovx, tanfovy, scale_modifier, antialiasing, prefiltered, debug, opacity_activation,
           forward_only, n_views, per_view_geometry, per_view_appearance, per_view_background, tile_cull)
    prm = _prm_cache.get(key)
    if prm is None:
        if len(_prm_cache) > 64:
            _prm_cache.clear()
        prm = _prm_cache[key] = RasterParams(
            P=P, M=M, sh_degree=sh_degree, W=W, H=H, tanfovx=tanfovx, tanfovy=tanfovy, scale_modifier=scale_modifier,
            antialiasing=int(antialiasing), prefiltered=int(prefiltered), debug=int(debug),
            opacity_activation=_ACTIVATIONS[opacity_activation], forward_only=int(forward_only), n_views=n_views,
            per_view_geometry=int(per_view_geometry), per_view_appearance=int(per_view_appearance),
            per_view_background=int(per_view_background), tile_cull=int(tile_cull))
        prm.cache_key = key
    return prm


def _prm_variant(prm, **fields):
    key = (prm.cache_key, tuple(fields.items()))
    p2 = _prm_cache.get(key)
    if p2 is None:
        if len(_prm_cache) > 64:
            _prm_cache.clear()
        p2 = _prm_cache[key] = RasterParams(**{f: getattr(prm, f) for f, _ in RasterParams._fields_})
        for f, value in fields.items():
            setattr(p2, f, value)
        p2.cache_key = key
    return p2


def _f32(t, device):
    if t is None:
        return None
    if t.dtype != torch.float32 or t.device != device:
        t = t.to(device=device, dtype=torch.float32)
    return t if t.is_contiguous() else t.contiguous()


def _views_of(prm):
    return max(prm.n_views, 1)


def _composite_forward(prm, cap, windowed, bg, geom, binning, img, color, invdepth, pair, l1):
    L, st, pp = _lib.lib(), stream_handle(), ctypes.byref(prm)
    if pair is not None:
        colors2, bg2, color2 = pair
        stage_timer.stage("composite_fwd", lambda: check(L.d3ga_raster_composite_fwd2(
            pp, dptr(bg), dptr(bg2), dptr(geom), dptr(colors2), dptr(binning), cap, dptr(img), dptr(color), dptr(color2),
            dptr(invdepth), st), "d3ga_raster_composite_fwd2"))
    elif l1 is not None:
        target, cell, loss = l1
        ws = torch.empty(4 * _views_of(prm) * ((prm.W + 15) // 16 + windowed) * ((prm.H + 15) // 16 + windowed),
                         dtype=torch.float32, device=color.device)
        stage_timer.stage("composite_fwd", lambda: check(L.d3ga_raster_composite_fwd_l1(
            pp, dptr(bg), dptr(geom), dptr(binning), cap, dptr(img), dptr(color), dptr(invdepth),
            dptr(None if cell is not None else target), dptr(cell), dptr(loss), dptr(ws), st), "d3ga_raster_composite_fwd_l1"))
    else:
        stage_timer.stage("composite_fwd", lambda: check(L.d3ga_raster_composite_fwd(
            pp, dptr(bg), dptr(geom), dptr(binning), cap, dptr(img), dptr(color), dptr(invdepth), st), "d3ga_raster_composite_fwd"))


def _launch_forward(prm, cap, windowed, gauss, cam, bg, color, radii, invdepth, pair=None, l1=None):
    means3D, sh, colors_precomp, opacities, scales, rotations, cov3Ds_precomp = gauss
    view, proj, campos = cam
    k = _views_of(prm)
    geom, binning, img = _scratch(prm.P, prm.W, prm.H, k, cap, color.device, prm.forward_only, windowed)
    L = _lib.lib()
    if stage_timer.enabled or k > 1 or pair is not None or l1 is not None:
        st, pp = stream_handle(), ctypes.byref(prm)
        stage_timer.stage("preprocess", lambda: check(L.d3ga_raster_preprocess(
            pp, dptr(means3D), dptr(sh), dptr(colors_precomp), dptr(opacities), dptr(scales), dptr(rotations),
            dptr(cov3Ds_precomp), dptr(view), dptr(proj), dptr(campos), dptr(geom), dptr(binning), cap,
            dptr(radii), st), "d3ga_raster_preprocess"))
        stage_timer.stage("bin_sort", lambda: check(L.d3ga_raster_bin_sort(
            pp, dptr(geom), dptr(binning), cap, st), "d3ga_raster_bin_sort"))
        _composite_forward(prm, cap, windowed, bg, geom, binning, img, color, invdepth, pair, l1)
    else:
        check(L.d3ga_raster_forward(ctypes.byref(prm), dptr(means3D), dptr(sh), dptr(colors_precomp),
                                    dptr(opacities), dptr(scales), dptr(rotations), dptr(cov3Ds_precomp),
                                    dptr(view), dptr(proj), dptr(campos), dptr(bg), dptr(geom), dptr(binning),
                                    dptr(img), cap, dptr(color), dptr(radii), dptr(invdepth), stream_handle()),
              "d3ga_raster_forward")
    return geom, binning, img


def _grad_buffers(prm, has_sh, from_sr, dev, exchanged, geo, opac, col, lead, geometry=True):
    new = lambda *shape: torch.empty(shape, dtype=torch.float32, device=dev)
    P, cut = prm.P, None
    if not exchanged:
        g_means3D, g_opac = new(*geo, 3) if geometry else None, new(*opac)
        g_sh = new(P, prm.M, 3) if has_sh else None
        g_col = None if col is None else new(*col)
        g_cov = None if (from_sr or not geometry) else new(*geo, 6)
        g_scales = new(*geo, 3) if from_sr else None
        g_rots = new(*geo, 4) if from_sr else None
    else:
        widths = [3, 1] + ([3, 4] if from_sr else [6]) + ([] if has_sh else [3])
        flat = new(P * sum(widths))
        parts, off = [], 0
        for w in widths:
            parts.append(flat[off:off + P * w].view(P, w))
            off += P * w
        g_means3D, g_opac = parts[0], parts[1]
        g_scales, g_rots = (parts[2], parts[3]) if from_sr else (None, None)
        g_cov = None if from_sr else parts[2]
        g_sh = factor = None
        by_name = {"means3D": g_means3D, "opacities": g_opac}
        by_name.update({"scales": g_scales, "rotations": g_rots} if from_sr else {"cov3D_precomp": g_cov})
        if not has_sh:
            g_col = by_name["colors_precomp"] = parts[-1]
        else:
            g_col = factor = new(*lead, P + 1, 3)
            if _views_of(prm) > 1:
                prm = _prm_variant(prm, factor_rows=P + 1)
        cut = (flat, factor, by_name)
    return g_means3D, g_opac, g_sh, g_col, g_cov, g_scales, g_rots, cut, prm


def _launch_backward(prm, cap, gauss, cam, bg, geom, binning, img, grad_color, grads, pair=None, g_invd=None, l1=None, deform=None):
    means3D, sh, scales, rotations, cov3Ds_precomp = gauss
    view, proj, campos = cam
    g_means3D, g_means2D, g_opac, g_sh, g_col, g_cov, g_scales, g_rots = grads
    k = _views_of(prm)
    acc, self_clearing = _accumulator(k * prm.P, means3D.device)
    if self_clearing != bool(prm.acc_self_clearing):
        prm = _prm_variant(prm, acc_self_clearing=int(self_clearing))
    L = _lib.lib()
    tail = () if deform is None else tuple(None if x is None else ctypes.byref(x) for x in deform)
    sfx = "" if deform is None else "_deform"
    if stage_timer.enabled or k > 1 or pair is not None or g_invd is not None:
        st, pp = stream_handle(), ctypes.byref(prm)
        if not self_clearing:
            acc.zero_()
        if pair is not None:
            colors2, bg2, grad_color2 = pair
            stage_timer.stage("composite_bwd", lambda: check(L.d3ga_raster_composite_bwd2(
                pp, dptr(bg), dptr(bg2), dptr(geom), dptr(colors2), dptr(binning), cap, dptr(img), dptr(grad_color),
                dptr(grad_color2), dptr(acc), st), "d3ga_raster_composite_bwd2"))
        elif g_invd is not None:
            stage_timer.stage("composite_bwd", lambda: check(L.d3ga_raster_composite_bwd_depth(
                pp, dptr(bg), dptr(geom), dptr(binning), cap, dptr(img), dptr(grad_color), dptr(g_invd), dptr(acc), st),
                "d3ga_raster_composite_bwd_depth"))
        elif l1 is not None:
            image, target, cell, g_loss = l1
            stage_timer.stage("composite_bwd", lambda: check(L.d3ga_raster_composite_bwd_l1(
                pp, dptr(bg), dptr(geom), dptr(binning), cap, dptr(img), dptr(image), dptr(target), dptr(cell),
                dptr(g_loss), dptr(grad_color), dptr(acc), st), "d3ga_raster_composite_bwd_l1"))
        else:
            stage_timer.stage("composite_bwd", lambda: check(L.d3ga_raster_composite_bwd(
                pp, dptr(bg), dptr(geom), dptr(binning), cap, dptr(img), dptr(grad_color), dptr(acc), st),
                "d3ga_raster_composite_bwd"))
        stage_timer.stage("preprocess_bwd", lambda: check(getattr(L, "d3ga_raster_preprocess_bwd" + sfx)(
            pp, dptr(means3D), dptr(sh), dptr(scales), dptr(rotations), dptr(cov3Ds_precomp), dptr(view), dptr(proj),
            dptr(campos), dptr(geom), dptr(acc), dptr(g_means3D), dptr(g_means2D), dptr(g_opac), dptr(g_sh),
            dptr(g_col), dptr(g_cov), dptr(g_scales), dptr(g_rots), *tail, st), "d3ga_raster_preprocess_bwd" + sfx))
    elif l1 is not None:
        image, target, cell, g_loss = l1
        check(getattr(L, "d3ga_raster_backward_l1" + sfx)(
            ctypes.byref(prm), dptr(means3D), dptr(sh), dptr(scales), dptr(rotations), dptr(cov3Ds_precomp),
            dptr(view), dptr(proj), dptr(campos), dptr(bg), dptr(geom), dptr(binning), cap, dptr(img),
            dptr(image), dptr(target), dptr(cell), dptr(g_loss), dptr(grad_color), dptr(acc), dptr(g_means3D),
            dptr(g_means2D), dptr(g_opac), dptr(g_sh), dptr(g_col), dptr(g_cov), dptr(g_scales), dptr(g_rots), *tail,
            stream_handle()), "d3ga_raster_backward_l1" + sfx)
    else:
        check(getattr(L, "d3ga_raster_backward" + sfx)(
            ctypes.byref(prm), dptr(means3D), dptr(sh), dptr(scales), dptr(rotations), dptr(cov3Ds_precomp),
            dptr(view), dptr(proj), dptr(campos), dptr(bg), dptr(geom), dptr(binning), cap, dptr(img),
            dptr(grad_color), dptr(acc), dptr(g_means3D), dptr(g_means2D), dptr(g_opac), dptr(g_sh), dptr(g_col),
            dptr(g_cov), dptr(g_scales), dptr(g_rots), *tail, stream_handle()), "d3ga_raster_backward" + sfx)


def _sh_grad_from_factors(gathered, P, M, sh_degree, means3D, scale):
    g_sh = torch.empty((P, M, 3), dtype=torch.float32, device=means3D.device)
    g = gathered.view(-1, P + 1, 3)
    check(_lib.lib().d3ga_sh_grad_from_views(P, M, sh_degree, g.shape[0], dptr(means3D), dptr(g), 3 * (P + 1), dptr(g[0, P]),
                                             3 * (P + 1), scale, dptr(g_sh), stream_handle()), "d3ga_sh_grad_from_views")
    return g_sh


def _exchange_gradients(sync, prm, cut, campos, means3D):
    P = prm.P
    flat, factor, by_name = cut
    if factor is not None:
        factor.view(-1, P + 1, 3)[:, P].copy_(campos.reshape(_views_of(prm), -1)[:, :3])
    if getattr(sync, "deferred", False):
        sync.park(flat, factor, by_name,
                  None if factor is None else {"P": P, "M": prm.M, "sh_degree": prm.sh_degree, "means3D": means3D})
        return True, None
    gathered = sync.exchange(flat, factor)
    return False, None if factor is None else _sh_grad_from_factors(gathered, P, prm.M, prm.sh_degree, means3D, sync.scale)


_reuse = {"enabled": False}
_geom_cache = {}


def set_geometry_reuse(enabled):
    _reuse["enabled"] = bool(enabled)
    if not enabled:
        _geom_cache.clear()


def clear_geometry_cache():
    _geom_cache.clear()


class geometry_reuse:

    def __enter__(self):
        self._was = _reuse["enabled"]
        _reuse["enabled"] = True
        return self

    def __exit__(self, *exc):
        _reuse["enabled"] = self._was
        _geom_cache.clear()
        return False


def _tkey(t):
    return None if t is None else (t.data_ptr(), t._version, tuple(t.shape))


def _geometry_key(prm, cap_mode, tensors):
    return (prm.P, prm.W, prm.H, prm.tanfovx, prm.tanfovy, prm.scale_modifier, prm.prefiltered, prm.opacity_activation, prm.antialiasing, prm.tile_cull, cap_mode) + tuple(
        _tkey(t) for t in tensors)


def _empty_to_none(t):
    return None if (t is None or t.numel() == 0) else t


def _check_exactly_one(shs, colors_precomp, scales, rotations, cov3D_precomp):
    if (shs is None) == (colors_precomp is None):
        raise Exception("Please provide excatly one of either SHs or precomputed colors!")
    if ((scales is None or rotations is None) and cov3D_precomp is None) or (
            (scales is not None or rotations is not None) and cov3D_precomp is not None):
        raise Exception("Please provide exactly one of either scale/rotation pair or precomputed 3D covariance!")


def _admit_grad_sync(grad_sync, P):
    if grad_sync is None or P == 0 or not (grad_sync.world > 1 or getattr(grad_sync, "always", False)):
        return None
    return grad_sync


def _verify_sync_inputs(sync, means3D, opacities, colors_precomp, sh, cov3Ds_precomp, scales, rotations):
    if sync is not None and hasattr(sync, "verify_inputs"):
        sync.verify_inputs({"means3D": means3D, "opacities": opacities, "colors_precomp": colors_precomp,
                            "shs": sh, "cov3D_precomp": cov3Ds_precomp, "scales": scales, "rotations": rotations})


class _RasterizeGaussians(torch.autograd.Function):
    @staticmethod
    def forward(ctx, means3D, means2D, sh, colors_precomp, opacities, scales, rotations, cov3Ds_precomp,
                raster_settings, grad_sync=None, colors2=None, bg2=None, opacity_activation=None, l1_target=None,
                want_invdepth=True, deform_node=None):
        s = raster_settings
        require_cuda(means3D)
        dev = means3D.device
        if means3D.shape[0] > 0:
            sh, colors_precomp, scales, rotations, cov3Ds_precomp = map(
                _empty_to_none, (sh, colors_precomp, scales, rotations, cov3Ds_precomp))
        means3D, sh, colors_precomp, opacities, scales, rotations, cov3Ds_precomp = (
            _f32(t, dev) for t in (means3D, sh, colors_precomp, opacities, scales, rotations, cov3Ds_precomp))
        view, proj, campos, bg = (_f32(t, dev) for t in (s.viewmatrix, s.projmatrix, s.campos, s.bg))
        P = means3D.shape[0]
        dual = colors2 is not None and P > 0
        empty_pair = colors2 is not None and P == 0
        if colors2 is not None:
            colors2, bg2 = _f32(colors2.detach(), dev), _f32(bg2, dev)
        H, W = int(s.image_height), int(s.image_width)
        M = sh.shape[1] if sh is not None else 0
        tfx, tfy = float(s.tanfovx), float(s.tanfovy)
        windowed = tfx == _lib.CAMERA_SLOT_WINDOWED and tfy == _lib.CAMERA_SLOT_WINDOWED and campos.numel() >= 9
        if not (tfx > 0.0 and tfy > 0.0) and not windowed:
            if not (tfx == 0.0 and tfy == 0.0 and campos.numel() >= 5):
                raise ValueError(f"GaussianRasterizationSettings: tanfovx / tanfovy must be positive (got {tfx}, {tfy}); only a "
                                 "camera slot (tanfovx = tanfovy = 0 with a 5-float campos: cameras.CameraSlot) reads them from the device")
        fwd_only = not any(ctx.needs_input_grad[:8])
        prm = _params(P, M, int(s.sh_degree), W, H, tfx, tfy, float(s.scale_modifier), bool(s.antialiasing), bool(s.prefiltered),
                      bool(s.debug), opacity_activation, fwd_only, tile_cull=_tile_cull_of(getattr(s, "tile_cull", False)))
        color = torch.empty((3, H, W), dtype=torch.float32, device=dev)
        l1_t = l1_cell = loss = None
        if l1_target is not None:
            from .graph import TensorSlot
            l1_t = l1_target.current if isinstance(l1_target, TensorSlot) else _f32(l1_target, dev)
            l1_cell = l1_target.cell if isinstance(l1_target, TensorSlot) else None
            if tuple(l1_t.shape) != (3, H, W):
                raise ValueError(f"rasterize_gaussians_l1: the target must be (3, {H}, {W}), got {tuple(l1_t.shape)}")
            loss = torch.empty((), dtype=torch.float32, device=dev)
        l1 = (l1_t, l1_cell, loss) if (l1_target is not None and P > 0 and colors2 is None and _l1_policy["fused_value"]) else None
        invdepth = torch.empty((1, H, W), dtype=torch.float32, device=dev) if want_invdepth else None
        radii = torch.empty((P,), dtype=torch.int32, device=dev)
        gauss = (means3D, sh, colors_precomp, opacities, scales, rotations, cov3Ds_precomp)
        cam = (view, proj, campos)
        geo_inputs = (means3D, opacities, scales, rotations, cov3Ds_precomp, view, proj)
        color2 = torch.empty((3, H, W), dtype=torch.float32, device=dev) if dual else None
        pair = (colors2, bg2, color2) if dual else None
        use_cache = _reuse["enabled"] and P > 0 and not dual and not windowed and not torch.cuda.is_current_stream_capturing()
        key = hit = None
        if use_cache:
            key = _geometry_key(prm, ("static", _policy["static"]) if _policy["mode"] == "static" else "auto", geo_inputs)
            hit = _geom_cache.get(dev.index)
        if hit is not None and hit["key"] == key:
            cap, binning, radii = hit["cap"], hit["binning"], hit["radii"]
            geom, _unused, img = _scratch(P, W, H, 1, cap, dev, fwd_only, False, binning=False)
            L, st, pp = _lib.lib(), stream_handle(), ctypes.byref(prm)
            stage_timer.stage("recolor", lambda: check(L.d3ga_raster_recolor(
                pp, dptr(means3D), dptr(sh), dptr(colors_precomp), dptr(campos), dptr(hit["geom"]), dptr(geom), st),
                "d3ga_raster_recolor"))
            _composite_forward(prm, cap, windowed, bg, geom, binning, img, color, invdepth, None, l1)
            _record_forward(dev, binning, cap)
        else:
            cap, geom, binning, img = _forward_with_capacity(P, 1, dev, lambda cap: _launch_forward(
                prm, cap, windowed, gauss, cam, bg, color, radii, invdepth, pair, l1))
            if use_cache:
                _geom_cache[dev.index] = {"key": key, "geom": geom, "binning": binning, "cap": cap, "radii": radii,
                                          "pins": tuple(None if t is None else t.detach() for t in geo_inputs)}
        ctx.prm = prm
        ctx.cap = cap
        ctx.has_means2D = means2D is not None
        ctx.grad_sync = _admit_grad_sync(grad_sync, P)
        _verify_sync_inputs(ctx.grad_sync, means3D, opacities, colors_precomp, sh, cov3Ds_precomp, scales, rotations)
        ctx.dual = dual
        ctx.l1 = l1_target is not None and P > 0 and not dual
        if deform_node is not None and (windowed or ctx.grad_sync is not None or P == 0 or cov3Ds_precomp is None or fwd_only):
            from .cage_deform import release_claim
            release_claim(*deform_node)
            deform_node = None
        ctx.deform_node = deform_node
        if l1_target is not None and l1 is None:
            l1_mean_forward(color, l1_t, l1_cell, loss, dev)
        _last_img[dev.index] = (img, W, H, geom, P)
        ctx.save_for_backward(means3D, sh, scales, rotations, cov3Ds_precomp, view, proj, campos, bg, geom, binning, img,
                              colors2, bg2, color if ctx.l1 else None, l1_t if ctx.l1 else None, l1_cell if ctx.l1 else None)
        ctx.mark_non_differentiable(radii)
        ctx.set_materialize_grads(False)
        if l1_target is not None:
            return color, radii, invdepth, loss
        if dual:
            return color, radii, invdepth, color2
        if empty_pair:
            return color, radii, invdepth, bg2.reshape(3, 1, 1).expand(3, H, W).contiguous()
        return color, radii, invdepth

    @staticmethod
    def backward(ctx, grad_color, _grad_radii, _grad_invdepth, grad_color2=None):
        (means3D, sh, scales, rotations, cov3Ds_precomp, view, proj, campos, bg, geom, binning, img, colors2,
         bg2, image, l1_t, l1_cell) = ctx.saved_tensors
        prm, dev, P = ctx.prm, means3D.device, means3D.shape[0]
        dual = ctx.dual
        g_loss = None
        if ctx.l1:
            g_loss, grad_color2 = grad_color2, None
            if g_loss is not None:
                g_loss = _f32(g_loss, dev).reshape(1)
        g_invd = None
        if _grad_invdepth is not None:
            if dual or ctx.l1:
                raise NotImplementedError("a gradient of the inverse-depth image is implemented for the single-image rasterizer call only "
                                          "(not for rasterize_gaussians_pair / rasterize_gaussians_l1)")
            g_invd = _f32(_grad_invdepth, dev).reshape(prm.H, prm.W)
        if grad_color is None and g_loss is None and g_invd is None:
            grad_color = torch.zeros((3, prm.H, prm.W), dtype=torch.float32, device=dev)
        grad_color = _f32(grad_color, dev)
        if dual:
            grad_color2 = (torch.zeros_like(grad_color) if grad_color2 is None else _f32(grad_color2, dev))
        has_sh, from_sr, sync = sh is not None, cov3Ds_precomp is None, ctx.grad_sync
        deform = deposit = node = None
        if ctx.deform_node is not None:
            from .cage_deform import deposit_on, fused_tail_structs, holds_claim
            node = ctx.deform_node[0] if holds_claim(*ctx.deform_node) else None
        g_means3D, g_opac, g_sh, g_col, g_cov, g_scales, g_rots, cut, prm = _grad_buffers(
            prm, has_sh, from_sr, dev, exchanged=sync is not None, geo=(P,), opac=(P, 1), col=None if has_sh else (P, 3), lead=(),
            geometry=node is None)
        g_means2D = torch.empty((P, 3), dtype=torch.float32, device=dev)
        if node is not None:
            *deform, deposit = fused_tail_structs(node)
        _launch_backward(prm, ctx.cap, (means3D, sh, scales, rotations, cov3Ds_precomp), (view, proj, campos), bg, geom, binning, img,
                         grad_color, (g_means3D, g_means2D, g_opac, g_sh, g_col, g_cov, g_scales, g_rots),
                         (colors2, bg2, grad_color2) if dual else None, g_invd,
                         (image, l1_t, l1_cell, g_loss) if g_loss is not None else None, deform)
        if deposit is not None:
            deposit_on(node, deposit)
        if sync is not None:
            parked, g_sh = _exchange_gradients(sync, prm, cut, campos, means3D)
            if parked:
                return (None, g_means2D if ctx.has_means2D else None) + (None,) * 14
            if has_sh:
                g_col = None
        return (g_means3D, g_means2D if ctx.has_means2D else None, g_sh, g_col, g_opac, g_scales, g_rots, g_cov, None,
                None, None, None, None, None, None, None)


_ACTIVATIONS = {None: 0, "none": 0, "sigmoid": 1}


def rasterize_gaussians(means3D, means2D, sh, colors_precomp, opacities, scales, rotations, cov3Ds_precomp,
                        raster_settings, grad_sync=None, opacity_activation=None, want_invdepth=True, deform_node=None):
    return _RasterizeGaussians.apply(means3D, means2D, sh, colors_precomp, opacities, scales, rotations,
                                     cov3Ds_precomp, raster_settings, grad_sync, None, None, opacity_activation, None, want_invdepth,
                                     deform_node)


def rasterize_gaussians_l1(means3D, means2D, sh, colors_precomp, opacities, scales, rotations, cov3Ds_precomp,
                           raster_settings, target, grad_sync=None, opacity_activation=None, want_invdepth=True, deform_node=None):
    return _RasterizeGaussians.apply(means3D, means2D, sh, colors_precomp, opacities, scales, rotations,
                                     cov3Ds_precomp, raster_settings, grad_sync, None, None, opacity_activation, target, want_invdepth,
                                     deform_node)


def rasterize_gaussians_pair(means3D, means2D, sh, colors_precomp, opacities, scales, rotations, cov3Ds_precomp,
                             raster_settings, colors2, bg2, grad_sync=None, opacity_activation=None, want_invdepth=True,
                             deform_node=None):
    return _RasterizeGaussians.apply(means3D, means2D, sh, colors_precomp, opacities, scales, rotations,
                                     cov3Ds_precomp, raster_settings, grad_sync, colors2, bg2, opacity_activation, None, want_invdepth,
                                     deform_node)


class GaussianRasterizer(nn.Module):

    def __init__(self, raster_settings, grad_sync=None, opacity_activation=None):
        super().__init__()
        self.raster_settings = raster_settings
        self.grad_sync = grad_sync
        self.opacity_activation = opacity_activation
        self.want_invdepth = True

    def markVisible(self, positions):
        require_cuda(positions)
        with torch.no_grad():
            p = _f32(positions, positions.device)
            view = _f32(self.raster_settings.viewmatrix, positions.device)
            vis = torch.empty((p.shape[0],), dtype=torch.uint8, device=p.device)
            check(_lib.lib().d3ga_raster_mark_visible(p.shape[0], dptr(p), dptr(view), dptr(vis), stream_handle()),
                  "d3ga_raster_mark_visible")
        return vis.bool()

    def forward(self, means3D, means2D, opacities, shs: Optional[torch.Tensor] = None,
                colors_precomp: Optional[torch.Tensor] = None, scales: Optional[torch.Tensor] = None,
                rotations: Optional[torch.Tensor] = None, cov3D_precomp: Optional[torch.Tensor] = None):
        _check_exactly_one(shs, colors_precomp, scales, rotations, cov3D_precomp)
        return rasterize_gaussians(means3D, means2D, shs, colors_precomp, opacities, scales, rotations, cov3D_precomp,
                                   self.raster_settings, self.grad_sync, self.opacity_activation, self.want_invdepth)


def last_tile_lists(W, H, device=None):
    dev = torch.cuda.current_device() if device is None else torch.device(device).index
    binning, cap = _last[dev]
    return tile_lists(binning, W, H, cap)


def last_termination(device=None):
    dev = torch.cuda.current_device() if device is None else torch.device(device).index
    img, W, H = _last_img[dev][:3]
    off = (ctypes.c_int64 * 2)()
    check(_lib.lib().d3ga_raster_img_layout(W, H, off), "d3ga_raster_img_layout")
    n = 4 * W * H
    return (img[off[0]:off[0] + n].view(torch.float32).view(H, W), img[off[1]:off[1] + n].view(torch.int32).view(H, W))


def last_block_lists(device=None):
    dev = torch.cuda.current_device() if device is None else torch.device(device).index
    img, W, H = _last_img[dev][:3]
    off = (ctypes.c_int64 * 2)()
    check(_lib.lib().d3ga_raster_img_layout_blocks(W, H, off), "d3ga_raster_img_layout_blocks")
    tiles = ((W + 15) // 16) * ((H + 15) // 16)
    if img.numel() <= off[1]:
        raise RuntimeError("the last forward was a forward_only render: it has no block lists")
    cnt = img[off[0]:off[0] + 64 * tiles].view(torch.int32).view(tiles, 16).long()
    n = (img.numel() - off[1]) // 8
# ... 27 lines not shown
```

### d3ga_amd/renderer.py

```python
import torch

from .cameras import CAMERA_SLOT_WINDOWED, batch_to_camera, crop_window, is_cropped, window_camera
from .rasterizer import GaussianRasterizationSettings, rasterize_gaussians, rasterize_gaussians_l1, rasterize_gaussians_pair

bg_colors = {"white": (1.0, 1.0, 1.0), "black": (0.0, 0.0, 0.0)}


_zeros = {}


def _zero_leaf(like):
    key = (like.device, tuple(like.shape))
    z = _zeros.get(key)
    if z is None:
        if len(_zeros) > 16:
            _zeros.clear()
        z = _zeros[key] = torch.zeros(like.shape, dtype=torch.float32, device=like.device)
    return z.detach().requires_grad_(True)


def paste(img, crop):
    left_w, right_w, top_h, bottom_h, W, H = crop[0], crop[1], crop[2], crop[3], int(crop[4]), int(crop[5])
    if W < img.shape[2]:
        img = img[:, :, :W] if left_w > right_w else img[:, :, -W:]
    if H < img.shape[1]:
        img = img[:, :H, :] if top_h > bottom_h else img[:, -H:, :]
    return img


def render_pair(batch, pkg, bg_color, colors2, bg_color2, grad_sync=None, crop_window=False):
    out = render(batch, pkg, bg_color, grad_sync=grad_sync, _pair=(colors2, bg_color2), crop_window=crop_window)
    return out


def render_l1(batch, pkg, bg_color, target, grad_sync=None, crop_window=False):
    windowed = crop_window or _windowed_slot(batch)
    if is_cropped(batch) and not windowed:
        from .losses import l1_loss
        img = render(batch, pkg, bg_color, grad_sync=grad_sync)["render"]
        return {"render": img, "l1": l1_loss(img, target)}
    return render(batch, pkg, bg_color, grad_sync=grad_sync, _l1=target, crop_window=crop_window)


def _windowed_slot(batch):
    slot = batch.get("camera_slot")
    return slot is not None and getattr(slot, "windowed", False)


def render_views(batches, pkg, bg_color, targets=None, cameras=None, colors2=None, bg_color2=None, grad_sync=None, tile_cull=False):
    from .raster_views import CameraBatch, rasterize_gaussians_views
    frames = pkg if isinstance(pkg, (list, tuple)) else None
    if frames is not None:
        first = frames[0]
        for f in frames[1:]:
            if f.get("shs") is not first.get("shs"):
                raise ValueError("render_views: the frames of a batch share their SH coefficients; `shs` differs between the packages")
            if f.get("sh_degree", 0) != first.get("sh_degree", 0):
                raise ValueError(f"render_views: `sh_degree` differs between the packages ({first.get('sh_degree', 0)} and {f.get('sh_degree', 0)})")
            for key in ("opacities", "opacity_logits", "rgb"):
                if (f.get(key) is None) != (first.get(key) is None):
                    raise ValueError(f"render_views: `{key}` is given in some packages of the batch and not in others")
        stack = lambda key: None if first.get(key) is None else torch.stack([f[key] for f in frames])
        same = lambda key: all(f.get(key) is first.get(key) for f in frames)
        look = {key: first.get(key) if same(key) else stack(key) for key in ("opacities", "opacity_logits", "rgb")}
        pkg = dict(first, means3D=stack("means3D"), cov3D_precomp=stack("cov3D_precomp"), scales=stack("scales"), rotations=stack("rotations"),
                   **look)
    means3D = pkg["means3D"]
    if cameras is None:
        sizes = {(int(b["width"]), int(b["height"])) for b in batches}
        if len(sizes) == 1 and not any(is_cropped(b) for b in batches):
            cameras = CameraBatch(len(batches), int(batches[0]["width"]), int(batches[0]["height"]), device=means3D.device).set(batches)
        else:
            W, H = crop_window(batches[0])[4:]
            for v, b in enumerate(batches):
                if crop_window(b)[4:] != (W, H):
                    raise ValueError(f"render_views: view {v}'s crop pastes to {crop_window(b)[4]}x{crop_window(b)[5]}, view 0's to {W}x{H} "
                                     "-- the views of a batch share one pasted image size")
            cameras = CameraBatch(len(batches), W, H, device=means3D.device, windowed=True).set(batches)
    opacities, act = pkg.get("opacities"), None
    if opacities is None and pkg.get("opacity_logits") is not None:
        opacities, act = pkg["opacity_logits"], "sigmoid"
    shs = pkg["shs"]
    out = rasterize_gaussians_views(means3D, shs, None if shs is not None else pkg["rgb"], opacities, pkg.get("scales"),
                                    pkg.get("rotations"), pkg.get("cov3D_precomp"), cameras, bg_color,
                                    sh_degree=pkg["sh_degree"] if "sh_degree" in pkg else 0, opacity_activation=act, l1_targets=targets,
                                    colors2=colors2, bg2=bg_color2, grad_sync=grad_sync, tile_cull=tile_cull)
    if colors2 is not None:
        return {"render": out[0], "render2": out[2]}
    return {"render": out[0], "l1": out[2]} if targets is not None else {"render": out[0]}


def render(batch, pkg, bg_color, colors_precomp=None, measure_time=False, solid_bg=True, fast=False, detach=[],
           grad_sync=None, _pair=None, _l1=None, crop_window=False):
    means3D = pkg["means3D"]
    slot = batch.get("camera_slot")
    crop = batch["crop"]
    windowed = (slot is not None and getattr(slot, "windowed", False)) or (crop_window and slot is None and is_cropped(batch))
    if windowed and grad_sync is not None:
        raise ValueError("render: grad_sync is not available with crop-window rendering")
    if windowed and slot is None:
        W, H = int(crop[4]), int(crop[5])
        mats, row = window_camera(batch, device=means3D.device)
        view, full, campos, tfx = mats[0:16].view(4, 4), mats[32:48].view(4, 4), row, CAMERA_SLOT_WINDOWED
    else:
        cam = slot or batch_to_camera(batch, device=means3D.device)
        W, H = (slot.image_width, slot.image_height) if windowed else (int(batch["width"]), int(batch["height"]))
        view, full, campos, tfx = cam.world_view_transform, cam.full_proj_transform, cam.camera_center, cam.tanfovx
    if windowed:
        crop = None

    settings = GaussianRasterizationSettings(
        image_height=H,
        image_width=W,
        tanfovx=tfx,
        tanfovy=tfx if windowed else cam.tanfovy,
        bg=bg_color,
        scale_modifier=1.0,
        viewmatrix=view,
        projmatrix=full,
        sh_degree=pkg["sh_degree"] if "sh_degree" in pkg else 0,
        campos=campos,
        prefiltered=False,
        debug=False,
        antialiasing=False,
        tile_cull=True,
    )

    geo = {k: pkg.get(k) for k in ("cov3D_precomp", "scales", "rotations", "opacities")}
    act = None
    if geo["opacities"] is None and pkg.get("opacity_logits") is not None:
        geo["opacities"], act = pkg["opacity_logits"], "sigmoid"
    cut = {"position": "means3D", "covariance": "cov3D_precomp", "opacity": "opacities"}
    geo["means3D"] = means3D
    for name in detach:
        if name in cut:
            geo[cut[name]] = geo[cut[name]].detach()
    means3D, cov3D_precomp, scales, rotations, opacities = (geo[k] for k in ("means3D", "cov3D_precomp", "scales", "rotations", "opacities"))
    shs = pkg["shs"] if colors_precomp is None else None
    if colors_precomp is None and shs is None:
        colors_precomp = pkg["rgb"]

    means2D = _zero_leaf(means3D)
    node = None
    if grad_sync is None and not windowed and scales is None and rotations is None:
        from .cage_deform import claim_for_render
        node = claim_for_render(means3D, cov3D_precomp)
        node = node if node[0] is not None else None
    try:
        means2D.retain_grad()
    except Exception:
        pass

    if _pair is not None:
        img, _radii, _invd, img2 = rasterize_gaussians_pair(means3D, means2D, shs, colors_precomp, opacities, scales, rotations,
                                                            cov3D_precomp, settings, _pair[0], _pair[1], grad_sync, act,
                                                            want_invdepth=False, deform_node=node)
        if crop is None:
            return {"render": img, "render2": img2}
        return {"render": paste(img, crop), "render2": paste(img2, crop)}
    if _l1 is not None:
        img, _radii, _invd, loss = rasterize_gaussians_l1(means3D, means2D, shs, colors_precomp, opacities, scales, rotations,
                                                          cov3D_precomp, settings, _l1, grad_sync, act, want_invdepth=False,
                                                          deform_node=node)
        return {"render": img, "l1": loss}
    if measure_time:
        torch.cuda.synchronize()
    rendered = rasterize_gaussians(means3D, means2D, shs, colors_precomp, opacities, scales, rotations, cov3D_precomp, settings,
                                   grad_sync, act, want_invdepth=False, deform_node=node)[0]
    if measure_time:
        torch.cuda.synchronize()
    return {"render": rendered if crop is None else paste(rendered, crop)}
```

### include/d3ga.h

```cpp
#ifndef D3GA_H
#define D3GA_H

#include <stddef.h>
#include <stdint.h>

#ifdef __cplusplus
extern "C" {
#endif

#if defined(__GNUC__)
#pragma GCC visibility push(default)
#endif

#define D3GA_VERSION 112

#define D3GA_OK 0
#define D3GA_E_NULL (-1)
#define D3GA_E_SIZE (-2)
#define D3GA_E_CONFIG (-3)
#define D3GA_E_CAPACITY (-4)

typedef void *d3ga_stream_t;

int d3ga_version(void);
const char *d3ga_status_string(int status);
#define D3GA_KNOB_COMPOSITE_VARIANT 0
#define D3GA_KNOB_MERGE_SLOTS 1
#define D3GA_KNOB_TILE_ASSIGN 2
#define D3GA_KNOB_BWD_SPLIT 3
#define D3GA_KNOB_SORT_MERGE 4
#define D3GA_KNOB_SSIM_IMPL 5
#define D3GA_KNOB_WGRAD_WS 6
#define D3GA_KNOB_CHAIN_ABL 7
#define D3GA_KNOB_CHAIN_GRID 8
#define D3GA_KNOB_COUNT 9
#define D3GA_KNOB_DEFAULT (-2147483647 - 1)
int d3ga_debug_set(int32_t key, int32_t value);
int d3ga_debug_defaults(int32_t *out, int32_t n);

typedef struct d3ga_lbs_pose_grad {
    int32_t J;
    int32_t n_chunks;
    int64_t n_entries;
    const float *tmpl;
    const float *delta;
    const int32_t *chunk_ptr;
    const int32_t *chunk_range;
    const int32_t *entries;
    uint32_t *counter;
    void *scratch;
    float *g_joint_mats;
    float *g_Rh;
    float *g_Th;
} d3ga_lbs_pose_grad;
int d3ga_lbs_pose_scratch_bytes(int V, int32_t n_chunks, int32_t fused, int64_t *bytes);
int d3ga_lbs_cage_fwd(int V, int K, const float *tmpl, const float *delta, const float *joint_mats,
                      const int32_t *skin_idx, const float *skin_w, const float *Rh, const float *Th, float *out,
                      d3ga_stream_t stream);
int d3ga_lbs_cage_bwd(int V, int K, const float *joint_mats, const int32_t *skin_idx, const float *skin_w,
                      const float *Rh, const float *grad_out, float *grad_delta, const d3ga_lbs_pose_grad *pose,
                      d3ga_stream_t stream);

#define D3GA_DEFORM_LOG_SCALES 1
#define D3GA_DEFORM_GRAD_PER_TET 2
typedef struct d3ga_cage_deform_in {
    int32_t P, V, flags, reserved;
    const float *tetpoints;
    const int32_t *tetras, *tetra_id;
    const float *barys, *canon_grad, *scales, *rots, *delta_barys;
} d3ga_cage_deform_in;
typedef struct d3ga_cage_deform_grads {
    const float *g_means, *g_cov6;
    float *g_tetpoints, *g_barys, *g_scales, *g_rots;
} d3ga_cage_deform_grads;
#define D3GA_DEFORM_ROUTE_CORNERS 1
#define D3GA_DEFORM_ROUTE_MERGE 2
typedef struct d3ga_cage_deform_route {
    int32_t kind, n_segments;
    const uint16_t *item_pos, *seg_begin;
    const int32_t *seg_ptr, *vert_start, *vert_items;
    float *records;
} d3ga_cage_deform_route;
typedef struct d3ga_cage_deform_skin {
    int32_t K, reserved;
    const float *joint_mats;
    const int32_t *skin_idx;
    const float *skin_w, *Rh, *g_tetpoints_extra;
    float *g_delta;
} d3ga_cage_deform_skin;
int d3ga_cage_deform_fwd(const d3ga_cage_deform_in *in, float *means3D, float *cov6, d3ga_stream_t stream);
int d3ga_cage_deform_bwd(const d3ga_cage_deform_in *in, const d3ga_cage_deform_grads *grads, const d3ga_cage_deform_route *route,
                         const d3ga_cage_deform_skin *skin, const d3ga_lbs_pose_grad *pose, d3ga_stream_t stream);
int d3ga_cage_deform_bwd_tail(const d3ga_cage_deform_in *in, const d3ga_cage_deform_grads *grads, const d3ga_cage_deform_route *route,
                              const d3ga_cage_deform_skin *skin, const d3ga_lbs_pose_grad *pose, d3ga_stream_t stream);

int d3ga_fem_energy_fwd(int T, const float *tetpoints, const int32_t *tetras, const float *Dn_inv, float *energy,
                        d3ga_stream_t stream);
int d3ga_fem_energy_bwd(int T, int V, const float *tetpoints, const int32_t *tetras, const float *Dn_inv,
                        const float *g_energy, float *g_tetpoints, d3ga_stream_t stream);

int d3ga_bary_interp_fwd(int32_t P, int32_t K, int32_t C, const float *attr, const int32_t *rows, const float *barys,
                         const float *delta_barys, float *out, d3ga_stream_t stream);
int d3ga_bary_interp_bwd(int32_t P, int32_t V, int32_t K, int32_t C, const float *attr, const int32_t *rows, const float *barys,
                         const float *delta_barys, const float *g_out, const int32_t *vert_start, const int32_t *vert_items,
                         float *g_attr, float *g_barys, d3ga_stream_t stream);

#define D3GA_BODY_MAX_JOINTS 64
#define D3GA_BODY_MAX_SHAPE 32
#define D3GA_BODY_LD_ALIGN 2048
#define D3GA_BODY_SAVED_FLOATS(J) (27 * (J) + 16)
typedef struct d3ga_body_model {
    int32_t V, J;
    int32_t n_shape, n_expr;
    int32_t n_hand_pca;
    int32_t ld;
    int32_t n_levels;
    int32_t reserved;
    const float *v_template;
    const float *dirs;
    const int32_t *w_ptr, *w_joint;
    const float *w_val;
    const int32_t *wt_ptr, *wt_vert;
    const float *wt_val;
    const float *J0;
    const float *Jdirs;
    const int32_t *parents, *level_ptr, *level_joint, *child_ptr, *child_joint;
    const float *hand_comps, *hand_mean;
} d3ga_body_model;
int d3ga_body_model_scratch_bytes(const d3ga_body_model *model, int32_t B, int64_t *fwd_bytes, int64_t *bwd_bytes);
int d3ga_body_model_fwd(const d3ga_body_model *model, int32_t B, int32_t pose_width, const float *poses, const float *shapes,
                        const float *expr, const float *Rh, const float *Th, float *verts, float *T, float *A, float *bs,
                        float *saved, void *scratch, int64_t scratch_bytes, d3ga_stream_t stream);
int d3ga_body_model_bwd(const d3ga_body_model *model, int32_t B, int32_t pose_width, const float *saved, const float *T,
                        const float *bs, const float *g_verts, const float *g_T, const float *g_A, const float *g_bs,
                        float *g_poses, float *g_shapes, float *g_expr, float *g_Rh, float *g_Th, void *scratch,
                        int64_t scratch_bytes, d3ga_stream_t stream);

typedef struct d3ga_raster_params {
    int32_t P;
    int32_t M;
    int32_t sh_degree;
    int32_t W, H;
    float tanfovx, tanfovy;
    float scale_modifier;
    int32_t antialiasing;
    int32_t prefiltered;
    int32_t debug;
    int32_t opacity_activation;
    int32_t forward_only;
    int32_t acc_self_clearing;
    int32_t n_views;
    int32_t per_view_geometry;
    int32_t tile_cull;
    int32_t factor_rows;
    int32_t per_view_appearance;
    int32_t per_view_background;
} d3ga_raster_params;
#define D3GA_OPACITY_SIGMOID 1

#define D3GA_CAMERA_SLOT_WINDOWED (-1.0f)
#define D3GA_CAMERA_SLOT_WINDOWED_FLOATS 9

int d3ga_raster_scratch_bytes(int32_t P, int32_t W, int32_t H, int64_t d_capacity, int64_t sizes[3]);
int64_t d3ga_raster_img_bytes(int32_t W, int32_t H, int64_t d_capacity, int32_t forward_only);
int d3ga_raster_scratch_bytes_views(int32_t P, int32_t W, int32_t H, int32_t n_views, int64_t d_capacity, int32_t forward_only,
                                    int64_t sizes[3]);

int d3ga_raster_scratch_bytes_window(int32_t P, int32_t W, int32_t H, int32_t n_views, int64_t d_capacity, int32_t forward_only,
                                     int64_t sizes[3]);
int d3ga_raster_binning_layout_window(int32_t W, int32_t H, int32_t n_views, int64_t d_capacity, int64_t offsets[7]);

int d3ga_raster_binning_layout(int32_t W, int32_t H, int64_t d_capacity, int64_t offsets[6]);
int d3ga_raster_img_layout(int32_t W, int32_t H, int64_t offsets[2]);
int d3ga_raster_img_layout_blocks(int32_t W, int32_t H, int64_t offsets[2]);

#define D3GA_CNT_D 0
#define D3GA_CNT_OVERFLOW 1
#define D3GA_CNT_MAXTILE 2
#define D3GA_CNT_VISIBLE 3
#define D3GA_CNT_BIG 4
#define D3GA_CNT_HUGE 5
#define D3GA_CNT_MID 6
#define D3GA_CNT_HEAVY 7

int d3ga_raster_preprocess(const d3ga_raster_params *prm, const float *means3D, const float *shs,
                           const float *colors_precomp, const float *opacities, const float *scales,
                           const float *rotations, const float *cov3D_precomp, const float *viewmatrix,
                           const float *projmatrix, const float *campos, void *geom, void *binning,
                           int64_t d_capacity, int32_t *radii, d3ga_stream_t stream);
int d3ga_raster_bin_sort(const d3ga_raster_params *prm, void *geom, void *binning, int64_t d_capacity,
                         d3ga_stream_t stream);
int d3ga_raster_composite_fwd(const d3ga_raster_params *prm, const float *bg, const void *geom, const void *binning,
                              int64_t d_capacity, void *img, float *out_color, float *out_invdepth,
                              d3ga_stream_t stream);
#define D3GA_ACC_STRIDE 16
int d3ga_raster_composite_bwd(const d3ga_raster_params *prm, const float *bg, const void *geom, const void *binning,
                              int64_t d_capacity, const void *img, const float *dL_dpix, float *acc,
                              d3ga_stream_t stream);
int d3ga_raster_composite_bwd_depth(const d3ga_raster_params *prm, const float *bg, const void *geom, const void *binning,
                                    int64_t d_capacity, const void *img, const float *dL_dpix, const float *dL_dinvdepth,
                                    float *acc, d3ga_stream_t stream);

int d3ga_raster_composite_fwd2(const d3ga_raster_params *prm, const float *bg, const float *bg2, const void *geom,
                               const float *colors2, const void *binning, int64_t d_capacity, void *img, float *out_color,
                               float *out_color2, float *out_invdepth, d3ga_stream_t stream);
int d3ga_raster_composite_bwd2(const d3ga_raster_params *prm, const float *bg, const float *bg2, const void *geom,
                               const float *colors2, const void *binning, int64_t d_capacity, const void *img,
                               const float *dL_dpix, const float *dL_dpix2, float *acc, d3ga_stream_t stream);

int d3ga_raster_composite_fwd_l1(const d3ga_raster_params *prm, const float *bg, const void *geom, const void *binning,
                                 int64_t d_capacity, void *img, float *out_color, float *out_invdepth, const float *target,
                                 const void *target_cell, float *loss, float *partials, d3ga_stream_t stream);
int d3ga_raster_composite_bwd_l1(const d3ga_raster_params *prm, const float *bg, const void *geom, const void *binning,
                                 int64_t d_capacity, const void *img, const float *image, const float *target,
                                 const void *target_cell, const float *g_loss, const float *dL_dpix, float *acc,
                                 d3ga_stream_t stream);
int d3ga_raster_backward_l1(const d3ga_raster_params *prm, const float *means3D, const float *shs, const float *scales,
                            const float *rotations, const float *cov3D_precomp, const float *viewmatrix,
                            const float *projmatrix, const float *campos, const float *bg, const void *geom,
                            const void *binning, int64_t d_capacity, const void *img, const float *image,
                            const float *target, const void *target_cell, const float *g_loss, const float *dL_dpix,
                            float *acc, float *dL_dmeans3D, float *dL_dmeans2D, float *dL_dopacity, float *dL_dsh,
                            float *dL_dcolors, float *dL_dcov3D, float *dL_dscales, float *dL_drots, d3ga_stream_t stream);
int d3ga_raster_recolor(const d3ga_raster_params *prm, const float *means3D, const float *shs,
                        const float *colors_precomp, const float *campos, const void *geom_src, void *geom_dst,
                        d3ga_stream_t stream);

int d3ga_raster_preprocess_bwd(const d3ga_raster_params *prm, const float *means3D, const float *shs,
                               const float *scales, const float *rotations, const float *cov3D_precomp,
                               const float *viewmatrix, const float *projmatrix, const float *campos,
                               const void *geom, const float *acc, float *dL_dmeans3D, float *dL_dmeans2D,
                               float *dL_dopacity, float *dL_dsh, float *dL_dcolors, float *dL_dcov3D,
                               float *dL_dscales, float *dL_drots, d3ga_stream_t stream);

int d3ga_raster_forward(const d3ga_raster_params *prm, const float *means3D, const float *shs,
                        const float *colors_precomp, const float *opacities, const float *scales,
                        const float *rotations, const float *cov3D_precomp, const float *viewmatrix,
                        const float *projmatrix, const float *campos, const float *bg, void *geom, void *binning,
                        void *img, int64_t d_capacity, float *out_color, int32_t *radii, float *out_invdepth,
                        d3ga_stream_t stream);
int d3ga_raster_backward(const d3ga_raster_params *prm, const float *means3D, const float *shs, const float *scales,
                         const float *rotations, const float *cov3D_precomp, const float *viewmatrix,
                         const float *projmatrix, const float *campos, const float *bg, const void *geom,
                         const void *binning, int64_t d_capacity, const void *img, const float *dL_dpix, float *acc,
                         float *dL_dmeans3D, float *dL_dmeans2D, float *dL_dopacity, float *dL_dsh,
                         float *dL_dcolors, float *dL_dcov3D, float *dL_dscales, float *dL_drots,
                         d3ga_stream_t stream);

int d3ga_raster_preprocess_bwd_deform(const d3ga_raster_params *prm, const float *means3D, const float *shs,
                                      const float *scales, const float *rotations, const float *cov3D_precomp,
                                      const float *viewmatrix, const float *projmatrix, const float *campos,
                                      const void *geom, const float *acc, float *dL_dmeans3D, float *dL_dmeans2D,
                                      float *dL_dopacity, float *dL_dsh, float *dL_dcolors, float *dL_dcov3D,
                                      float *dL_dscales, float *dL_drots, const d3ga_cage_deform_in *deform,
                                      const d3ga_cage_deform_grads *dgrads, const d3ga_cage_deform_route *route,
                                      d3ga_stream_t stream);
int d3ga_raster_backward_deform(const d3ga_raster_params *prm, const float *means3D, const float *shs, const float *scales,
                                const float *rotations, const float *cov3D_precomp, const float *viewmatrix,
                                const float *projmatrix, const float *campos, const float *bg, const void *geom,
                                const void *binning, int64_t d_capacity, const void *img, const float *dL_dpix, float *acc,
                                float *dL_dmeans3D, float *dL_dmeans2D, float *dL_dopacity, float *dL_dsh,
                                float *dL_dcolors, float *dL_dcov3D, float *dL_dscales, float *dL_drots,
                                const d3ga_cage_deform_in *deform, const d3ga_cage_deform_grads *dgrads,
                                const d3ga_cage_deform_route *route, d3ga_stream_t stream);
int d3ga_raster_backward_l1_deform(const d3ga_raster_params *prm, const float *means3D, const float *shs, const float *scales,
                                   const float *rotations, const float *cov3D_precomp, const float *viewmatrix,
                                   const float *projmatrix, const float *campos, const float *bg, const void *geom,
                                   const void *binning, int64_t d_capacity, const void *img, const float *image,
                                   const float *target, const void *target_cell, const float *g_loss, const float *dL_dpix,
                                   float *acc, float *dL_dmeans3D, float *dL_dmeans2D, float *dL_dopacity, float *dL_dsh,
                                   float *dL_dcolors, float *dL_dcov3D, float *dL_dscales, float *dL_drots,
                                   const d3ga_cage_deform_in *deform, const d3ga_cage_deform_grads *dgrads,
                                   const d3ga_cage_deform_route *route, d3ga_stream_t stream);

int d3ga_sh_grad_from_views(int32_t P, int32_t M, int32_t sh_degree, int32_t n_views, const float *means3D,
                            const float *g_views, int64_t g_stride, const float *campos_views, int64_t campos_stride,
                            float scale, float *dL_dsh, d3ga_stream_t stream);

int d3ga_raster_mark_visible(int32_t P, const float *means3D, const float *viewmatrix, uint8_t *visible,
                             d3ga_stream_t stream);

int d3ga_l1_mean_fwd(int64_t n, const float *a, const float *b, float *out, d3ga_stream_t stream);
#define D3GA_LOSS_PARTIALS 2048
int d3ga_l1_mean_fwd_ws(int64_t n, const float *a, const float *b, float *out, float *partials, d3ga_stream_t stream);
int d3ga_l1_mean_bwd(int64_t n, const float *a, const float *b, const float *g, float *grad_a, d3ga_stream_t stream);
int d3ga_l1_mean_fwd_ws_cell(int64_t n, const float *a, const float *const *b_cell, float *out, float *partials,
                             d3ga_stream_t stream);
int d3ga_l1_mean_bwd_cell(int64_t n, const float *a, const float *const *b_cell, const float *g, float *grad_a,
                          d3ga_stream_t stream);

int d3ga_ssim_fwd(int32_t C, int32_t H, int32_t W, const float *img1, const float *img2, float *out, float *Dm,
                  float *Dq1, float *Dq12, d3ga_stream_t stream);
int d3ga_ssim_bwd(int32_t C, int32_t H, int32_t W, const float *img1, const float *img2, const float *Dm,
                  const float *Dq1, const float *Dq12, const float *g, float *grad_img1, d3ga_stream_t stream);
int d3ga_ssim_l1_fwd(int32_t C, int32_t H, int32_t W, const float *img1, const float *img2, float *out, float *Dm,
                     float *Dq1, float *Dq12, float *out_l1, d3ga_stream_t stream);
int d3ga_ssim_l1_bwd(int32_t C, int32_t H, int32_t W, const float *img1, const float *img2, const float *Dm,
                     const float *Dq1, const float *Dq12, const float *g, const float *g_l1, float *grad_img1,
                     d3ga_stream_t stream);

#define D3GA_BLUR_PARTIALS 6144
int d3ga_blur_mix_fwd(int32_t C, int32_t H, int32_t W, int32_t n_cameras, const float *img, const float *weights_raw,
                      const int32_t *cam_idx, float *out, d3ga_stream_t stream);
int d3ga_blur_mix_bwd(int32_t C, int32_t H, int32_t W, int32_t n_cameras, const float *img, const float *weights_raw,
                      const int32_t *cam_idx, const float *grad_out, float *grad_img, float *grad_weights_raw,
                      float *partials, d3ga_stream_t stream);
// ... 258 lines not shown
```

Measured before the change: 2935.

## Write tile sort keys directly into fixed-capacity per-tile strips during preprocessing

Adds an optional key-strip path: preprocessing writes each Gaussian's depth/index key straight into a per-tile fixed-capacity strip buffer, so the separate tile scatter pass can exit early and the per-tile sort reads keys from the strip. Overflow or unreserved-tile flags fall back to the original scatter into the contiguous key array. The renderer enables it by default for single-view renders. It costs a large extra buffer (tiles × 4096 × 8 bytes), extra preprocess kernel variants and overflow bookkeeping.

```diff
diff --git a/d3ga_amd/_lib.py b/d3ga_amd/_lib.py
--- a/d3ga_amd/_lib.py
+++ b/d3ga_amd/_lib.py
@@ -41,6 +41,7 @@
                 ("opacity_activation", ctypes.c_int32), ("forward_only", ctypes.c_int32),
                 ("acc_self_clearing", ctypes.c_int32), ("n_views", ctypes.c_int32), ("per_view_geometry", ctypes.c_int32),
                 ("tile_cull", ctypes.c_int32),
+                ("key_strips", ctypes.c_int32), ("key_strips_lo", ctypes.c_int32), ("key_strips_hi", ctypes.c_int32),
                 ("factor_rows", ctypes.c_int32), ("per_view_appearance", ctypes.c_int32), ("per_view_background", ctypes.c_int32)]
 
 
diff --git a/d3ga_amd/csrc/build.py b/d3ga_amd/csrc/build.py
--- a/d3ga_amd/csrc/build.py
+++ b/d3ga_amd/csrc/build.py
@@ -5,7 +5,7 @@
 HERE = os.path.dirname(os.path.abspath(__file__))
 SOURCES = ["deform.hip", "raster_pre.hip", "raster_bin.hip", "raster_composite.hip", "raster_composite_scan.hip", "raster_api.hip", "bary.hip", "loss.hip", "image_tail.hip", "calib.hip", "frame_prep.hip", "eval.hip", "mesh_raster.hip", "point_raster.hip", "optim.hip", "mlp.hip", "encoding.hip", "body_model.hip", "skeleton.hip", "perceptual.hip", "lpips.hip", "knn.hip", "bary_interp.hip", "frame_state.hip", "objective.hip", "pose_prior.hip"]
 LINK_MAP = os.path.join(HERE, "d3ga.map")
-HEADERS = ["d3ga_math.h", "d3ga_internal.h", "raster_pre_body.h", "deform_tail.h", "composite_common.h", "body_model_math.h", "skeleton_math.h", "frame_prep_math.h", "eval_math.h", "mesh_raster_math.h", "point_raster_math.h", "perceptual_math.h", "lpips_math.h", "knn_math.h", "objective_math.h", "pose_prior_math.h", os.path.join("..", "..", "include", "d3ga.h")]
+HEADERS = ["d3ga_math.h", "d3ga_internal.h", "key_strips.h", "raster_pre_body.h", "deform_tail.h", "composite_common.h", "body_model_math.h", "skeleton_math.h", "frame_prep_math.h", "eval_math.h", "mesh_raster_math.h", "point_raster_math.h", "perceptual_math.h", "lpips_math.h", "knn_math.h", "objective_math.h", "pose_prior_math.h", os.path.join("..", "..", "include", "d3ga.h")]
 ABL = os.environ.get("D3GA_SCAN_ABL")
 VARIANT = os.environ.get("D3GA_VARIANT")
 DIAG = os.environ.get("D3GA_DIAG") or (("abl" + ABL) if ABL else None) or (("var" + VARIANT.split(":")[0]) if VARIANT else None)
diff --git a/d3ga_amd/csrc/d3ga_internal.h b/d3ga_amd/csrc/d3ga_internal.h
--- a/d3ga_amd/csrc/d3ga_internal.h
+++ b/d3ga_amd/csrc/d3ga_internal.h
@@ -4,6 +4,7 @@
 
 #include "../../include/d3ga.h"
 #include "d3ga_math.h"
+#include "key_strips.h"
 
 namespace d3ga {
 
@@ -67,6 +68,18 @@
 };
 constexpr int kVisParts = 32, kVisStride = 32;
 constexpr int kUnresvWord = 1;
+constexpr int kStripOvfWord = 2;
+struct KeyStrips { uint64_t *keys; uint32_t cap; };
+static inline bool key_strips_on(const d3ga_raster_params *prm) { return prm->key_strips > 0 && prm->n_views <= 1; }
+static inline KeyStrips key_strips_of(const d3ga_raster_params *prm) {
+    if (!key_strips_on(prm)) return KeyStrips{nullptr, 0u};
+    return KeyStrips{(uint64_t *)(uintptr_t)((uint64_t)(uint32_t)prm->key_strips_lo | ((uint64_t)(uint32_t)prm->key_strips_hi << 32)), (uint32_t)prm->key_strips};
+}
+#ifdef __HIPCC__
+__device__ __forceinline__ bool strips_route(const uint32_t *__restrict__ vis_part) {
+    return (vis_part[kUnresvWord] | vis_part[kStripOvfWord]) == 0u;
+}
+#endif
 static inline int64_t bin_bytes(int64_t tiles, int64_t dcap) {
     return 256 + 2 * align256(4 * tiles) + 4 * kVisParts * kVisStride + align256(4 * (tiles + 1)) + align256(4 * tiles) + align256(8 * dcap) +
            align256(4 * dcap) + 4 * align256(4 * tiles);
diff --git a/d3ga_amd/csrc/key_strips.h b/d3ga_amd/csrc/key_strips.h
--- /dev/null
+++ b/d3ga_amd/csrc/key_strips.h
@@ -0,0 +1,21 @@
+#pragma once
+#include <stdint.h>
+
+#ifndef D3GA_HD
+#ifdef __HIPCC__
+#define D3GA_HD __host__ __device__ __forceinline__
+#else
+#define D3GA_HD static inline
+#endif
+#endif
+
+namespace d3ga {
+
+D3GA_HD bool strip_cap_valid(int64_t cap) { return cap >= 1 && cap <= (int64_t(1) << 20) && (cap & (cap - 1)) == 0; }
+D3GA_HD int64_t strip_bytes(int64_t tiles, int64_t cap) { return 8 * tiles * cap; }
+D3GA_HD uint64_t strip_index(uint32_t tile, uint32_t slot, uint32_t cap) { return (uint64_t)tile * cap + slot; }
+D3GA_HD bool strip_slot_fits(uint32_t slot, uint32_t cap) { return slot < cap; }
+D3GA_HD bool strip_range_overflows(uint32_t base, uint32_t c, uint32_t cap) { return (uint64_t)base + c > (uint64_t)cap; }
+D3GA_HD uint64_t strip_key(uint32_t depth_bits, uint32_t j) { return ((uint64_t)depth_bits << 32) | j; }
+
+}
diff --git a/d3ga_amd/csrc/raster_bin.hip b/d3ga_amd/csrc/raster_bin.hip
--- a/d3ga_amd/csrc/raster_bin.hip
+++ b/d3ga_amd/csrc/raster_bin.hip
@@ -1,3 +1,4 @@
+#include <algorithm>
 #include <atomic>
 
 #include "composite_common.h"
@@ -201,60 +202,77 @@
     else tile_order_body(tiles, count, count2, vis_part, order, counters);
 }
 
+struct StripSrc { uint64_t *keys; uint32_t cap; const uint32_t *vis_part; };
+template <class T>
+__device__ __forceinline__ const T &first_of(const T &t) { return t; }
+#define D3GA_SCATTER_BLOCK(BX, NBX, LEAVE) \
+    const int tid = threadIdx.x, lane = tid & 63, wave = tid >> 6; \
+    const int i = (BX) * kBlock + tid; \
+    if (i - lane >= P) LEAVE; \
+    const size_t j = (size_t)blockIdx.y * P + i; \
+    const uint32_t *rec = resv + ((size_t)blockIdx.y * (NBX) * (kBlock / 64) + (BX) * (kBlock / 64) + wave) * kResvStride; \
+    const uint2 box = *reinterpret_cast<const uint2 *>(rec); \
+    uint32_t base[kResvSlots]; \
+    base[0] = rec[kResvHdr + lane]; \
+    int x0 = 0, y0 = 0, x1 = 0, y1 = 0; \
+    uint64_t key = 0; \
+    if (i < P) { \
+        const uint2 rc = rect[j]; \
+        x0 = rc.x & 0xffffu; y0 = rc.x >> 16; x1 = rc.y & 0xffffu; y1 = rc.y >> 16; \
+        key = ((uint64_t)__float_as_uint(depth[j]) << 32) | (uint32_t)j; \
+    } \
+    const bool visible = x1 > x0 && y1 > y0; \
+    TileWindow win; \
+    win.x0 = (int)(box.x & 0xffffu); win.y0 = (int)(box.x >> 16); win.w = (int)(box.y & 0xffffu); win.h = (int)(box.y >> 16); \
+    if (win.empty()) LEAVE; \
+    if (win.fits()) { \
+        const int area = win.area(); \
+        uint32_t *cur = s_cur[wave]; \
+        const float inv_w = 1.0f / (float)win.w; \
+    _Pragma("unroll") \
+        for (int q = 1; q < kResvSlots; ++q) base[q] = lane + 64 * q < area ? rec[kResvHdr + lane + 64 * q] : 0u; \
+    _Pragma("unroll") \
+        for (int q = 0; q < kResvSlots; ++q) { \
+            const int k = lane + 64 * q; \
+            if (k < area) cur[k] = start[win.tile_of(k, gx, inv_w)] + base[q]; \
+        } \
+        __builtin_amdgcn_wave_barrier(); \
+        if (visible) \
+            for (int ty = y0; ty < y1; ++ty) \
+                for (int tx = x0; tx < x1; ++tx) { \
+                    const int l = (ty - win.y0) * win.w + (tx - win.x0); \
+                    if ((unsigned)l >= (unsigned)area) continue; \
+                    const uint32_t pos = atomicAdd(&cur[l], 1u); \
+                    if (pos < dcap) keys[pos] = key; \
+                } \
+    } else if (visible) { \
+        for (int ty = y0; ty < y1; ++ty) \
+            for (int tx = x0; tx < x1; ++tx) { \
+                const uint32_t pos = atomicAdd(&cursor[ty * gx + tx], 1u); \
+                if (pos < dcap) keys[pos] = key; \
+            } \
+    }
+template <class... TAIL>
 __global__ __launch_bounds__(kBlock) void tile_scatter_kernel(int P, int gx, const uint2 *__restrict__ rect,
                                                               const float *__restrict__ depth,
                                                               const uint32_t *__restrict__ start,
                                                               const uint32_t *__restrict__ resv,
                                                               uint32_t *__restrict__ cursor, uint64_t *__restrict__ keys,
-                                                              uint64_t dcap) {
+                                                              uint64_t dcap, TAIL... tail) {
     __shared__ uint32_t s_cur[kBlock / 64][kResvTiles];
-    const int tid = threadIdx.x, lane = tid & 63, wave = tid >> 6;
-    const int i = blockIdx.x * kBlock + tid;
-    if (i - lane >= P) return;
-    const size_t j = (size_t)blockIdx.y * P + i;
-    const uint32_t *rec = resv + ((size_t)blockIdx.y * gridDim.x * (kBlock / 64) + blockIdx.x * (kBlock / 64) + wave) * kResvStride;
-    const uint2 box = *reinterpret_cast<const uint2 *>(rec);
-    uint32_t base[kResvSlots];
-    base[0] = rec[kResvHdr + lane];
-    int x0 = 0, y0 = 0, x1 = 0, y1 = 0;
-    uint64_t key = 0;
-    if (i < P) {
-        const uint2 rc = rect[j];
-        x0 = rc.x & 0xffffu; y0 = rc.x >> 16; x1 = rc.y & 0xffffu; y1 = rc.y >> 16;
-        key = ((uint64_t)__float_as_uint(depth[j]) << 32) | (uint32_t)j;
-    }
-    const bool visible = x1 > x0 && y1 > y0;
-    TileWindow win;
-    win.x0 = (int)(box.x & 0xffffu); win.y0 = (int)(box.x >> 16); win.w = (int)(box.y & 0xffffu); win.h = (int)(box.y >> 16);
-    if (win.empty()) return;
-    if (win.fits()) {
-        const int area = win.area();
-        uint32_t *cur = s_cur[wave];
-        const float inv_w = 1.0f / (float)win.w;
-#pragma unroll
-        for (int q = 1; q < kResvSlots; ++q) base[q] = lane + 64 * q < area ? rec[kResvHdr + lane + 64 * q] : 0u;
-#pragma unroll
-        for (int q = 0; q < kResvSlots; ++q) {
-            const int k = lane + 64 * q;
-            if (k < area) cur[k] = start[win.tile_of(k, gx, inv_w)] + base[q];
-        }
-        __builtin_amdgcn_wave_barrier();
-        if (visible)
-            for (int ty = y0; ty < y1; ++ty)
-                for (int tx = x0; tx < x1; ++tx) {
-                    const int l = (ty - win.y0) * win.w + (tx - win.x0);
-                    if ((unsigned)l >= (unsigned)area) continue;
-                    const uint32_t pos = atomicAdd(&cur[l], 1u);
-                    if (pos < dcap) keys[pos] = key;
-                }
-    } else if (visible) {
-        for (int ty = y0; ty < y1; ++ty)
-            for (int tx = x0; tx < x1; ++tx) {
-                const uint32_t pos = atomicAdd(&cursor[ty * gx + tx], 1u);
-                if (pos < dcap) keys[pos] = key;
-            }
-    }
-}
+    if constexpr (sizeof...(TAIL) > 0) {
+        if (strips_route(first_of(tail...).vis_part)) return;
+        const unsigned nbx = ((unsigned)P + kBlock - 1) / kBlock;
+        for (unsigned bx = blockIdx.x; bx < nbx; bx += gridDim.x) {
+            D3GA_SCATTER_BLOCK(bx, nbx, continue)
+            __builtin_amdgcn_wave_barrier();
+        }
+    } else {
+        D3GA_SCATTER_BLOCK(blockIdx.x, gridDim.x, return)
+    }
+}
+
+#undef D3GA_SCATTER_BLOCK
 
 template <typename KeyPtr>
 __device__ __forceinline__ void bitonic_sort(KeyPtr k, int n, int tid, int nthreads) {
@@ -289,7 +307,8 @@
 template <int BLOCK, int CAP>
 __device__ __forceinline__ void sort_one_tile_bucket(uint64_t *s_key, uint32_t *s_bin, uint32_t *s_red, int tile,
                                                      const uint32_t *__restrict__ start, const uint64_t *__restrict__ keys,
-                                                     uint32_t *__restrict__ point_list, uint64_t dcap) {
+                                                     uint32_t *__restrict__ point_list, uint64_t dcap,
+                                                     const uint64_t *__restrict__ strip = nullptr ) {
     static_assert(CAP == 8 * BLOCK, "eight keys / eight counters per thread");
     constexpr int NW = BLOCK / 64;
     const uint64_t b64 = min((uint64_t)start[tile], dcap), e64 = min((uint64_t)start[tile + 1], dcap);
@@ -300,7 +319,7 @@
 #pragma unroll
     for (int k = 0; k < 8; ++k) {
         const int i = tid + k * BLOCK;
-        r[k] = i < n ? keys[b64 + i] : ~0ull;
+        r[k] = i < n ? (strip ? strip[i] : keys[b64 + i]) : ~0ull;
     }
 #pragma unroll
     for (int k = 0; k < 8; ++k) {
@@ -372,11 +391,13 @@
 template <int BLOCK, int CAP>
 __device__ __forceinline__ bool sort_huge_tile_bucket(uint64_t *s_key, uint32_t *s_bin, uint32_t *s_cur, uint32_t *s_red, int tile,
                                                       const uint32_t *__restrict__ start, const uint64_t *__restrict__ keys,
-                                                      uint32_t *__restrict__ point_list, uint64_t dcap) {
+                                                      uint32_t *__restrict__ point_list, uint64_t dcap,
+                                                      const uint64_t *__restrict__ strip = nullptr) {
     static_assert(CAP == 8 * BLOCK, "eight counters per thread");
     constexpr int NW = BLOCK / 64;
     const uint64_t b64 = min((uint64_t)start[tile], dcap), e64 = min((uint64_t)start[tile + 1], dcap);
     const int n = (int)(e64 - b64);
+    if (strip) keys = strip - b64;
     const int tid = threadIdx.x, lane = tid & 63, wave = tid >> 6;
     uint32_t lo = 0xffffffffu, hi = 0u;
     for (int i = tid; i < n; i += BLOCK) { const uint32_t d = (uint32_t)(keys[b64 + i] >> 32); lo = min(lo, d); hi = max(hi, d); }
@@ -472,6 +493,28 @@
 }
 
 template <int BLOCK, int CAP>
+__global__ __launch_bounds__(BLOCK) void tile_sort_lds_strips_kernel(const uint32_t *__restrict__ start,
+                                                                     const uint64_t *__restrict__ keys,
+                                                                     uint32_t *__restrict__ point_list, uint64_t dcap,
+                                                                     const uint32_t *__restrict__ order, int tiles,
+                                                                     const uint64_t *__restrict__ strips, uint32_t strip_cap,
+                                                                     const uint32_t *__restrict__ vis_part) {
+    __shared__ uint64_t s_key[CAP];
+    __shared__ __attribute__((aligned(8))) uint32_t s_bin[CAP + 1];
+    __shared__ uint32_t s_red[2 * (BLOCK / 64)];
+    const bool route = strips_route(vis_part);
+    for (int rank = blockIdx.x; rank < tiles; rank += gridDim.x) {
+        const int tile = (int)order[rank];
+        const uint32_t n = start[tile + 1] - start[tile];
+        if (n == 0) return;
+        if (n <= (uint32_t)CAP)
+            sort_one_tile_bucket<BLOCK, CAP>(s_key, s_bin, s_red, tile, start, keys, point_list, dcap,
+                                             route ? strips + strip_index((uint32_t)tile, 0u, strip_cap) : nullptr);
+        __syncthreads();
+    }
+}
+
+template <int BLOCK, int CAP, class... TAIL>
 __global__ __launch_bounds__(BLOCK) void tile_sort_lds_list_kernel(const uint32_t *__restrict__ start,
                                                                    const uint64_t *__restrict__ keys,
                                                                    uint32_t *__restrict__ point_list, uint64_t dcap,
@@ -481,21 +524,27 @@
                                                                    const uint32_t *__restrict__ huge_list,
                                                                    const uint32_t *__restrict__ huge_count,
                                                                    const uint32_t *__restrict__ list2,
-                                                                   const uint32_t *__restrict__ list2_count) {
+                                                                   const uint32_t *__restrict__ list2_count, TAIL... tail) {
     extern __shared__ __attribute__((aligned(16))) uint64_t s_key_dyn[];
     uint32_t *s_bin = reinterpret_cast<uint32_t *>(s_key_dyn + CAP);
     uint32_t *s_red = s_bin + CAP + 1;
     uint32_t *s_cur = s_red + 2 * (BLOCK / 64) + 2;
+    bool route = false;
+    if constexpr (sizeof...(TAIL) > 0) route = strips_route(first_of(tail...).vis_part);
+    auto strip_of = [&](int tile) __attribute__((always_inline)) -> uint64_t * {
+        if constexpr (sizeof...(TAIL) > 0) return route ? first_of(tail...).keys + strip_index((uint32_t)tile, 0u, first_of(tail...).cap) : nullptr;
+        else return nullptr;
+    };
     const uint32_t count = *list_count;
     for (uint32_t v = blockIdx.x; v < count; v += gridDim.x) {
         __syncthreads();
-        sort_one_tile_bucket<BLOCK, CAP>(s_key_dyn, s_bin, s_red, (int)list[v], start, keys, point_list, dcap);
+        sort_one_tile_bucket<BLOCK, CAP>(s_key_dyn, s_bin, s_red, (int)list[v], start, keys, point_list, dcap, strip_of((int)list[v]));
     }
     if (list2) {
         const uint32_t count2 = *list2_count;
         for (uint32_t v = gridDim.x - 1u - blockIdx.x; v < count2; v += gridDim.x) {
             __syncthreads();
-            sort_one_tile_bucket<BLOCK, CAP>(s_key_dyn, s_bin, s_red, (int)list2[v], start, keys, point_list, dcap);
+            sort_one_tile_bucket<BLOCK, CAP>(s_key_dyn, s_bin, s_red, (int)list2[v], start, keys, point_list, dcap, strip_of((int)list2[v]));
         }
     }
     if (huge_list) {
@@ -506,7 +555,12 @@
             const uint64_t b64 = min((uint64_t)start[tile], dcap), e64 = min((uint64_t)start[tile + 1], dcap);
             const int n = (int)(e64 - b64);
             __syncthreads();
-            if (!sort_huge_tile_bucket<BLOCK, CAP>(s_key_dyn, s_bin, s_cur, s_red, tile, start, keys, point_list, dcap)) {
+            if (!sort_huge_tile_bucket<BLOCK, CAP>(s_key_dyn, s_bin, s_cur, s_red, tile, start, keys, point_list, dcap, strip_of(tile))) {
+                if (uint64_t *const rw = strip_of(tile)) {
+                    bitonic_sort(rw, n, tid, BLOCK);
+                    for (int i = tid; i < n; i += BLOCK) point_list[b64 + i] = (uint32_t)rw[i];
+                    continue;
+                }
                 bitonic_sort(keys_rw + b64, n, tid, BLOCK);
                 for (int i = tid; i < n; i += BLOCK) point_list[b64 + i] = (uint32_t)keys_rw[b64 + i];
             }
@@ -530,6 +584,9 @@
                                     d3ga_stream_t stream) {
     if (!prm || !geom || !binning) return D3GA_E_NULL;
     if (prm->P < 0 || prm->W <= 0 || prm->H <= 0 || d_capacity < 0) return D3GA_E_SIZE;
+    if (prm->key_strips < 0 || (prm->key_strips > 0 && !strip_cap_valid(prm->key_strips))) return D3GA_E_SIZE;
+    const KeyStrips ks = key_strips_of(prm);
+    if (key_strips_on(prm) && !ks.keys) return D3GA_E_NULL;
     hipStream_t s = (hipStream_t)stream;
     const int views = n_views_of(prm);
     const int gx = grid_x(prm);
@@ -542,7 +599,13 @@
                        (uint32_t)kSortSmall, (uint32_t)kSortMid, (uint32_t)kSortLarge, bin.tile_order);
     D3GA_TRY(check_launch(s, prm->debug));
     if (P == 0 || d_capacity == 0) return D3GA_OK;
-    hipLaunchKernelGGL(tile_scatter_kernel, dim3((unsigned)((prm->P + kBlock - 1) / kBlock), (unsigned)views), dim3(kBlock), 0, s, prm->P,
+    const StripSrc ss = {ks.keys, ks.cap, bin.vis_part};
+    if (ks.keys)
+        hipLaunchKernelGGL(tile_scatter_kernel<StripSrc>, dim3((unsigned)std::min<int64_t>((prm->P + kBlock - 1) / kBlock, 512), (unsigned)views), dim3(kBlock), 0, s,
+                           prm->P, gx, g.rect, g.depth, bin.tile_start, resv_records(binning, tiles, d_capacity, views, is_windowed(prm)),
+                           bin.tile_cursor, bin.keys, (uint64_t)d_capacity, ss);
+    else
+    hipLaunchKernelGGL(tile_scatter_kernel<>, dim3((unsigned)((prm->P + kBlock - 1) / kBlock), (unsigned)views), dim3(kBlock), 0, s, prm->P,
                        gx, g.rect, g.depth, bin.tile_start, resv_records(binning, tiles, d_capacity, views, is_windowed(prm)),
                        bin.tile_cursor, bin.keys, (uint64_t)d_capacity);
     D3GA_TRY(check_launch(s, prm->debug));
@@ -558,6 +621,11 @@
             want = per_cu * cus;
             if (dev >= 0 && dev < 64) resident[dev].store(want, std::memory_order_relaxed);
         }
+        if (ks.keys)
+            hipLaunchKernelGGL((tile_sort_lds_strips_kernel<256, kSortSmall>), dim3(tiles < want ? tiles : want), dim3(256), 0, s, bin.tile_start,
+                               bin.keys, bin.point_list, (uint64_t)d_capacity, (const uint32_t *)bin.tile_order, tiles,
+                               (const uint64_t *)ks.keys, ks.cap, (const uint32_t *)bin.vis_part);
+        else
         hipLaunchKernelGGL((tile_sort_lds_kernel<256, kSortSmall>), dim3(tiles < want ? tiles : want), dim3(256), 0, s, bin.tile_start,
                            bin.keys, bin.point_list, (uint64_t)d_capacity, (const uint32_t *)bin.tile_order, tiles);
     }
@@ -569,6 +637,8 @@
         if (dev >= 0 && dev < 64 && !attr_set[dev].load(std::memory_order_relaxed)) {
             D3GA_HIP(hipFuncSetAttribute((const void *)tile_sort_lds_list_kernel<1024, kSortLarge>,
                                          hipFuncAttributeMaxDynamicSharedMemorySize, (int)sort_lds_bytes(kSortLarge, 1024, true)));
+            D3GA_HIP(hipFuncSetAttribute((const void *)tile_sort_lds_list_kernel<1024, kSortLarge, StripSrc>,
+                                         hipFuncAttributeMaxDynamicSharedMemorySize, (int)sort_lds_bytes(kSortLarge, 1024, true)));
             attr_set[dev].store(true, std::memory_order_relaxed);
         }
     }
@@ -576,6 +646,10 @@
     const int merge_knob = debug_knob(D3GA_KNOB_SORT_MERGE);
     const bool merged = merge_knob >= 0 ? merge_knob != 0 : d_capacity / (tiles > 0 ? tiles : 1) < 320;
 #define D3GA_LAUNCH_LIST_SORT(BLOCKV, CAPV, GRID, HUGE, LIST, CNT, KEYS_RW, HLIST, HCNT, LIST2, CNT2)                              \
+    if (ks.keys)                                                                                                                    \
+        hipLaunchKernelGGL((tile_sort_lds_list_kernel<BLOCKV, CAPV, StripSrc>), dim3(GRID), dim3(BLOCKV), sort_lds_bytes(CAPV, BLOCKV, HUGE), s, \
+                           bin.tile_start, bin.keys, bin.point_list, (uint64_t)d_capacity, LIST, CNT, KEYS_RW, HLIST, HCNT, LIST2, CNT2, ss); \
+    else                                                                                                                            \
     hipLaunchKernelGGL((tile_sort_lds_list_kernel<BLOCKV, CAPV>), dim3(GRID), dim3(BLOCKV), sort_lds_bytes(CAPV, BLOCKV, HUGE), s, \
                        bin.tile_start, bin.keys, bin.point_list, (uint64_t)d_capacity, LIST, CNT, KEYS_RW, HLIST, HCNT, LIST2, CNT2)
     const uint32_t *const nil = nullptr;
diff --git a/d3ga_amd/csrc/raster_pre.hip b/d3ga_amd/csrc/raster_pre.hip
--- a/d3ga_amd/csrc/raster_pre.hip
+++ b/d3ga_amd/csrc/raster_pre.hip
@@ -245,6 +245,36 @@
         if (lane + 64 * j < area) rec[kResvHdr + lane + 64 * j] = r.base[j];
 }
 
+__device__ __forceinline__ void tile_place_keys(const d3ga_raster_params &prm, uint32_t *s_win, const TileResv &r, uint2 rc, float depth,
+                                                int i, int gx, uint32_t *__restrict__ vis_part) {
+    if (r.win.empty() || !r.win.fits()) return;
+    const int lane = threadIdx.x & 63;
+    uint64_t *__restrict__ strips = reinterpret_cast<uint64_t *>((uint64_t)(uint32_t)prm.key_strips_lo | ((uint64_t)(uint32_t)prm.key_strips_hi << 32));
+    const uint32_t cap = (uint32_t)prm.key_strips;
+    const int area = r.win.area();
+    __builtin_amdgcn_wave_barrier();
+#pragma unroll
+    for (int j = 0; j < kResvSlots; ++j)
+        if (lane + 64 * j < area) s_win[lane + 64 * j] = r.base[j];
+    __builtin_amdgcn_wave_barrier();
+    const int x0 = rc.x & 0xffffu, y0 = rc.x >> 16, x1 = rc.y & 0xffffu, y1 = rc.y >> 16;
+    const uint64_t key = strip_key(__float_as_uint(depth), (uint32_t)i);
+    bool ovf = false;
+    if (x1 > x0 && y1 > y0)
+        for (int ty = y0; ty < y1; ++ty)
+            for (int tx = x0; tx < x1; ++tx) {
+                const int l = (ty - r.win.y0) * r.win.w + (tx - r.win.x0);
+                if ((unsigned)l >= (unsigned)area) continue;
+                const uint32_t s = atomicAdd(&s_win[l], 1u);
+                if (strip_slot_fits(s, cap)) strips[strip_index((uint32_t)(ty * gx + tx), s, cap)] = key;
+                else ovf = true;
+            }
+    if (__ballot(ovf) != 0ull && lane == 0) atomicOr(&vis_part[kStripOvfWord], 1u);
+}
+__device__ __forceinline__ uint2 pack_rect(const TileRect &t) {
+    return t.visible ? make_uint2((uint32_t)t.r0 | ((uint32_t)t.r1 << 16), (uint32_t)t.r2 | ((uint32_t)t.r3 << 16)) : make_uint2(0u, 0u);
+}
+
 template <bool WIN, bool TC = false>
 __device__ __forceinline__ PreOut preprocess_view(const d3ga_raster_params &prm, const ViewCam &cam, int i, V3 mean,
                                                     const float *sh_row, bool staged, const ShColJ &cj, bool pre, const float (&pc6)[6],
@@ -263,7 +293,7 @@
     return o;
 }
 
-template <bool WIN, bool TC = false>
+template <bool WIN, bool TC = false, bool KS = false>
 __device__ __forceinline__ void preprocess_full_wavefront(
     const d3ga_raster_params &prm, const ViewCam &cam, const float *__restrict__ means3D, const float *__restrict__ shs,
     const float *__restrict__ opacities, const float *__restrict__ cov3D_precomp, const float *__restrict__ campos, const GeomBuf &geom,
@@ -284,6 +314,8 @@
     float dx, dy, dz, invd;
     bool visible = false;
     TileResv rs;
+    uint2 krc = make_uint2(0u, 0u);
+    float kdepth = 0.f;
     ShColJ cj = {0.f, 0.f, 0.f, 0.f, 0.f, 0.f, 0.f, 0.f, 0.f, 0.f, 0.f, 0.f};
     sh_two_pass48(slab, shs + (size_t)48 * row0, lane, [&]() __attribute__((always_inline)) {
         PreOut o = preprocess_geom(prm, cam, i, pl.mean, opacities, nullptr, nullptr, cov3D_precomp, pl);
@@ -291,6 +323,7 @@
         if constexpr (TC) tile_tighten(o);
         if constexpr (WIN) o = window_clip(o, cam.ox / kTile, cam.oy / kTile, gx, gy);
         rs = tile_reserve_issue<true>(reinterpret_cast<uint32_t *>(slab), view_tile_rect(o, tile_row0), gx, tile_count, tile_count2, vis_part);
+        if constexpr (KS) { krc = pack_rect(view_tile_rect(o, tile_row0)); kdepth = o.sp.depth; }
         invd = write_geom_records_splat(geom, i, o, false, tile_row0, radii);
         sh_view_dir(pl.mean, campos, dx, dy, dz);
         sh_basis(prm.sh_degree, dx, dy, dz, B);
@@ -304,9 +337,10 @@
     preprocess_colour(prm, cam, i, pl.mean, nullptr, nullptr, pl, visible, rgb, clampmask);
     write_geom_records_colour(geom, i, rgb[0], rgb[1], rgb[2], invd, clampmask, true, cj);
     tile_reserve_store(rs, rec);
-}
-
-template <bool WANT_J, bool WIN, bool TC = false>
+    if constexpr (KS) tile_place_keys(prm, reinterpret_cast<uint32_t *>(slab), rs, krc, kdepth, i, gx, vis_part);
+}
+
+template <bool WANT_J, bool WIN, bool TC = false, bool KS = false>
 __global__ __launch_bounds__(kBlock) void preprocess_kernel(
     d3ga_raster_params prm, const float *__restrict__ means3D, const float *__restrict__ shs,
     const float *__restrict__ colors_precomp, const float *__restrict__ opacities, const float *__restrict__ scales,
@@ -327,7 +361,7 @@
     uint32_t *const rec = resv + (size_t)(blockIdx.x * (kBlock / 64) + wave) * kResvStride;
     const int row0 = blockIdx.x * kBlock + wave * 64;
     if (WANT_J && staged && cov3D_precomp && M3 == 48 && prm.P - row0 >= 64) {
-        preprocess_full_wavefront<WIN, TC>(prm, cam, means3D, shs, opacities, cov3D_precomp, campos, geom, tile_count, tile_count2, vis_part, rec,
+        preprocess_full_wavefront<WIN, TC, KS>(prm, cam, means3D, shs, opacities, cov3D_precomp, campos, geom, tile_count, tile_count2, vis_part, rec,
                                            radii, tile_row0, gx, gy, s_sh + wave * kShHalfSlab);
         return;
     }
@@ -360,6 +394,7 @@
     const TileResv rs = tile_reserve_issue(s_win, tr, gx, tile_count, tile_count2, vis_part);
     if (i < prm.P) write_geom_records(geom, i, o, !cov3D_precomp, tile_row0, radii, WANT_J, cj);
     tile_reserve_store(rs, rec);
+    if constexpr (KS) tile_place_keys(prm, s_win, rs, pack_rect(tr), o.sp.depth, i, gx, vis_part);
 }
 
 template <bool WANT_J, int KV>
@@ -755,6 +790,8 @@
     if (prm->n_views < 0) return D3GA_E_SIZE;
     if (grid_x(prm) > 65535 || (int64_t)grid_y(prm) * n_views_of(prm) > 65535) return D3GA_E_SIZE;
     if ((int64_t)prm->P * n_views_of(prm) >= (1ll << 31)) return D3GA_E_SIZE;
+    if (prm->key_strips < 0 || (prm->key_strips > 0 && !strip_cap_valid(prm->key_strips))) return D3GA_E_SIZE;
+    if (key_strips_on(prm) && !key_strips_of(prm).keys) return D3GA_E_NULL;
     return D3GA_OK;
 }
 
@@ -829,10 +866,16 @@
         else if (left == 3 || left == 5) launch_group(std::integral_constant<int, 3>());
         else launch_group(std::integral_constant<int, 2>());
     }
-    const auto kernel = tc ? (want_j ? (wnd ? preprocess_kernel<true, true, true> : preprocess_kernel<true, false, true>)
-                                      : (wnd ? preprocess_kernel<false, true, true> : preprocess_kernel<false, false, true>))
-                            : (want_j ? (wnd ? preprocess_kernel<true, true> : preprocess_kernel<true, false>)
-                                      : (wnd ? preprocess_kernel<false, true> : preprocess_kernel<false, false>));
+    const bool ks = key_strips_on(prm);
+    const auto kernel =
+        ks ? (tc ? (want_j ? (wnd ? preprocess_kernel<true, true, true, true> : preprocess_kernel<true, false, true, true>)
+                           : (wnd ? preprocess_kernel<false, true, true, true> : preprocess_kernel<false, false, true, true>))
+                 : (want_j ? (wnd ? preprocess_kernel<true, true, false, true> : preprocess_kernel<true, false, false, true>)
+                           : (wnd ? preprocess_kernel<false, true, false, true> : preprocess_kernel<false, false, false, true>)))
+           : (tc ? (want_j ? (wnd ? preprocess_kernel<true, true, true> : preprocess_kernel<true, false, true>)
+                           : (wnd ? preprocess_kernel<false, true, true> : preprocess_kernel<false, false, true>))
+                 : (want_j ? (wnd ? preprocess_kernel<true, true> : preprocess_kernel<true, false>)
+                           : (wnd ? preprocess_kernel<false, true> : preprocess_kernel<false, false>)));
     for (int v = v0; v < views; ++v) {
         const ViewCams<1> c = view_cams<1>(viewmatrix, projmatrix, campos, cs, v, 1);
         const size_t og = pv * v, oa = pa * v;
diff --git a/d3ga_amd/rasterizer.py b/d3ga_amd/rasterizer.py
--- a/d3ga_amd/rasterizer.py
+++ b/d3ga_amd/rasterizer.py
@@ -24,6 +24,7 @@
     debug: bool
     antialiasing: bool = False
     tile_cull: bool = False
+    key_strips: bool = False
 
 
 _policy = {"mode": "auto", "static": 0}
@@ -89,6 +90,49 @@
     return bool(requested) if o is None else o
 
 
+KEY_STRIP_CAP = 4096
+_key_strips = {"override": None, "cap": None}
+_strip_bufs = {}
+
+
+def set_key_strips(mode, cap=None):
+    if mode not in (None, True, False):
+        raise ValueError(mode)
+    if cap is not None and (int(cap) < 1 or int(cap) > (1 << 20) or int(cap) & (int(cap) - 1)):
+        raise ValueError(f"set_key_strips: cap must be a power of two in [1, 2^20], got {cap}")
+    _key_strips["override"] = mode
+    _key_strips["cap"] = None if cap is None else int(cap)
+
+
+def _key_strips_of(requested):
+    o = _key_strips["override"]
+    on = bool(requested) if o is None else o
+    return (_key_strips["cap"] or KEY_STRIP_CAP) if on else 0
+
+
+def _strip_buffer(tiles, cap, dev):
+    need = 8 * tiles * cap
+    bufs = _strip_bufs.setdefault(dev.index, [])
+    for b in bufs:
+        if b.numel() >= need:
+            return b
+    b = torch.empty(need, dtype=torch.uint8, device=dev)
+    bufs.append(b)
+    return b
+
+
+def last_key_route(device=None):
+    dev = torch.cuda.current_device() if device is None else torch.device(device).index
+    binning, _cap, prm, windowed = _last_route[dev]
+    tiles = ((prm.W + 15) // 16 + windowed) * ((prm.H + 15) // 16 + windowed)
+    off = 256 + 2 * ((4 * tiles + 255) // 256 * 256)
+    w = binning[off:off + 16].view(torch.int32).cpu().tolist()
+    return {"unreserved": bool(w[1]), "strip_overflow": bool(w[2]), "strips": bool(prm.key_strips) and not (w[1] or w[2])}
+
+
+_last_route = {}
+
+
 _l1_policy = {"fused_value": os.environ.get("D3GA_L1_VALUE", "fused") != "separate"}
 
 
@@ -177,9 +221,10 @@
 
 
 def _params(P, M, sh_degree, W, H, tanfovx, tanfovy, scale_modifier, antialiasing, prefiltered, debug, opacity_activation,
-            forward_only, n_views=0, per_view_geometry=False, per_view_appearance=False, per_view_background=False, tile_cull=False):
+            forward_only, n_views=0, per_view_geometry=False, per_view_appearance=False, per_view_background=False, tile_cull=False, key_strips=0, strips=None):
     key = (P, M, sh_degree, W, H, tanfovx, tanfovy, scale_modifier, antialiasing, prefiltered, debug, opacity_activation,
-           forward_only, n_views, per_view_geometry, per_view_appearance, per_view_background, tile_cull)
+           forward_only, n_views, per_view_geometry, per_view_appearance, per_view_background, tile_cull, key_strips,
+           0 if strips is None else strips.data_ptr())
     prm = _prm_cache.get(key)
     if prm is None:
         if len(_prm_cache) > 64:
@@ -189,9 +234,14 @@
             antialiasing=int(antialiasing), prefiltered=int(prefiltered), debug=int(debug),
             opacity_activation=_ACTIVATIONS[opacity_activation], forward_only=int(forward_only), n_views=n_views,
             per_view_geometry=int(per_view_geometry), per_view_appearance=int(per_view_appearance),
-            per_view_background=int(per_view_background), tile_cull=int(tile_cull))
+            per_view_background=int(per_view_background), tile_cull=int(tile_cull), key_strips=int(key_strips),
+            key_strips_lo=_i32(key[-1] & 0xFFFFFFFF), key_strips_hi=_i32(key[-1] >> 32))
         prm.cache_key = key
     return prm
+
+
+def _i32(u):
+    return u - (1 << 32) if u >= (1 << 31) else u
 
 
 def _prm_variant(prm, **fields):
@@ -401,7 +451,7 @@
 
 
 def _geometry_key(prm, cap_mode, tensors):
-    return (prm.P, prm.W, prm.H, prm.tanfovx, prm.tanfovy, prm.scale_modifier, prm.prefiltered, prm.opacity_activation, prm.antialiasing, prm.tile_cull, cap_mode) + tuple(
+    return (prm.P, prm.W, prm.H, prm.tanfovx, prm.tanfovy, prm.scale_modifier, prm.prefiltered, prm.opacity_activation, prm.antialiasing, prm.tile_cull, prm.key_strips, cap_mode) + tuple(
         _tkey(t) for t in tensors)
 
 
@@ -457,8 +507,11 @@
                 raise ValueError(f"GaussianRasterizationSettings: tanfovx / tanfovy must be positive (got {tfx}, {tfy}); only a "
                                  "camera slot (tanfovx = tanfovy = 0 with a 5-float campos: cameras.CameraSlot) reads them from the device")
         fwd_only = not any(ctx.needs_input_grad[:8])
+        strip_cap = _key_strips_of(getattr(s, "key_strips", False)) if P > 0 else 0
+        strips = _strip_buffer(((W + 15) // 16 + windowed) * ((H + 15) // 16 + windowed), strip_cap, dev) if strip_cap else None
         prm = _params(P, M, int(s.sh_degree), W, H, tfx, tfy, float(s.scale_modifier), bool(s.antialiasing), bool(s.prefiltered),
-                      bool(s.debug), opacity_activation, fwd_only, tile_cull=_tile_cull_of(getattr(s, "tile_cull", False)))
+                      bool(s.debug), opacity_activation, fwd_only, tile_cull=_tile_cull_of(getattr(s, "tile_cull", False)),
+                      key_strips=strip_cap, strips=strips)
         color = torch.empty((3, H, W), dtype=torch.float32, device=dev)
         l1_t = l1_cell = loss = None
         if l1_target is not None:
@@ -496,6 +549,7 @@
             if use_cache:
                 _geom_cache[dev.index] = {"key": key, "geom": geom, "binning": binning, "cap": cap, "radii": radii,
                                           "pins": tuple(None if t is None else t.detach() for t in geo_inputs)}
+        _last_route[dev.index] = (binning, cap, prm, int(windowed))
         ctx.prm = prm
         ctx.cap = cap
         ctx.has_means2D = means2D is not None
diff --git a/d3ga_amd/renderer.py b/d3ga_amd/renderer.py
--- a/d3ga_amd/renderer.py
+++ b/d3ga_amd/renderer.py
@@ -124,6 +124,7 @@
         debug=False,
         antialiasing=False,
         tile_cull=True,
+        key_strips=True,
     )
 
     geo = {k: pkg.get(k) for k in ("cov3D_precomp", "scales", "rotations", "opacities")}
diff --git a/include/d3ga.h b/include/d3ga.h
--- a/include/d3ga.h
+++ b/include/d3ga.h
@@ -152,6 +152,8 @@
     int32_t n_views;
     int32_t per_view_geometry;
     int32_t tile_cull;
+    int32_t key_strips;
+    int32_t key_strips_lo, key_strips_hi;
     int32_t factor_rows;
     int32_t per_view_appearance;
     int32_t per_view_background;
```

Result: no change. 2919 (-0.5%).
